# pedro-morgado/spatialaudiogen

Hardware: AMD Instinct MI355X
Metric: ambisonic seconds generated/sec (0.1 s windows, 224x448 video) (higher is better)
Workload: dtype f32 (fp32 in / out / accumulate; products on the 16-bit matrix cores with fp32-equivalent operand splits: two fp16 planes (3 products per multiply) for the ResNet trunk's 3x3 convs, whose operand ranges batch-norm bounds, three bf16 planes (6 products) elsewhere - measured against the fp64 oracle as

## Files before the change

spatialaudiogen_amd/csrc/kernels.h:

```cpp
#pragma once
#include "common.h"
#include "wave_reduce.h"
#include "igemm_tiles.h"

namespace sagen {

struct BnRef {
    const double* acc = nullptr;
    const float* gamma = nullptr;
    const float* beta = nullptr;
    double inv_count = 0.0;
    float eps = 1e-3f;
};

constexpr int H2_AMAX_SLOTS = 64, H2_AMAX_STRIDE = 32, H2_AMAX_FLOATS = H2_AMAX_SLOTS * H2_AMAX_STRIDE;

struct IgemmDesc {
    const float* x = nullptr;
    const float* w = nullptr;
    int w_split = 0;
    float* y = nullptr;
    const float* bias = nullptr;
    const float* in_scale = nullptr;
    const float* in_shift = nullptr;
    BnRef bn_in;
    double* stats = nullptr;
    float* amax_out = nullptr;
    float* splitk_ws = nullptr;
    int* sk_ticket = nullptr;
    int sk_rep = 1;
    int M = 0, N = 0, K = 0, Kpad = 0;
    int Hg = 1, Wg = 1, g_h0 = 0, g_w0 = 0;
    int Hin = 1, Win = 1, Cin = 0, ldx = 0;
    long x_bstride = 0;
    int in_sh = 1, in_sw = 1;
    int ntaps = 1, TW = 1, tap_sh = 1, tap_sw = 1, tap_h0 = 0, tap_w0 = 0;
    int log2Cin = -1;
    int dsh = 1, dsw = 1, Cout = 0;
    int Hlim = 1, Wlim = 1;
    long y_bstride = 0;
    long y_rstride = 0;
    int ldy = 0;
    int relu_out = 0;
    int splitk = 1;
    unsigned x_bytes = 0, w_bytes = 0;
    unsigned y_bytes = 0;
    int no_bounds = 0;
    int uniform_taps = 0;
    const void* xp3 = nullptr;
    unsigned xp3_bytes = 0, xp3_cstride = 0;
    int p3_np = 0;
    int xp3_fmt = 0;
    int xp3_row0 = 0, xp3_rows = 0;
    const void* xs2d = nullptr;
    unsigned xs2d_bytes = 0;
    int xs2d_np = 0;
    const void* wh2 = nullptr;
    unsigned wh2_bytes = 0;
    const float* h2_a_inv = nullptr;
    const float* h2_w_inv = nullptr;
    unsigned p3_magic_wp = 0, p3_magic_h = 0;
    const float* mm_coeffs = nullptr;
    float* mm_out = nullptr;
    int mm_row0 = 0, mm_nf = 0;
    int mm_f_lo = 1;
    void* trace = nullptr;
    int trace_block = 0;
    GroupInfo grp;
};
__device__ __forceinline__ void igemm_relocate(IgemmDesc& d, int g) {
    const GroupInfo gi = d.grp;
    d.x = grp_ptr(d.x, gi, g); d.y = grp_ptr(d.y, gi, g);
    d.in_scale = grp_ptr(d.in_scale, gi, g); d.in_shift = grp_ptr(d.in_shift, gi, g);
    d.bn_in.acc = grp_ptr(d.bn_in.acc, gi, g);
    d.stats = grp_ptr(d.stats, gi, g); d.amax_out = grp_ptr(d.amax_out, gi, g);
    d.splitk_ws = grp_ptr(d.splitk_ws, gi, g); d.sk_ticket = grp_ptr(d.sk_ticket, gi, g);
    d.xp3 = grp_ptr(d.xp3, gi, g); d.xs2d = grp_ptr(d.xs2d, gi, g);
    d.h2_a_inv = grp_ptr(d.h2_a_inv, gi, g); d.h2_w_inv = grp_ptr(d.h2_w_inv, gi, g);
    d.mm_coeffs = grp_ptr(d.mm_coeffs, gi, g); d.mm_out = grp_ptr(d.mm_out, gi, g);
}

inline void igemm_set_p3_planes(IgemmDesc& d, const void* planes, int B, int H, int W, int C) {
    d.xp3 = planes;
    d.p3_np = planes ? B * H * (W + 1) : 0;
    d.xp3_cstride = (unsigned)((size_t)d.p3_np * 96);
    d.xp3_bytes = (unsigned)((size_t)d.xp3_cstride * (C / 16));
}
inline void igemm_set_h2_planes(IgemmDesc& d, const void* planes, int B, int rows, int W, int C, const void* wh2, const float* a_inv,
                                const float* w_inv, int row0 = 0, int band = 0) {
    d.xp3 = planes; d.xp3_fmt = 1; d.xp3_row0 = row0; d.xp3_rows = band;
    d.p3_np = planes ? B * rows * (W + 1) : 0;
    d.xp3_cstride = (unsigned)((size_t)d.p3_np * 64);
    d.xp3_bytes = (unsigned)((size_t)d.xp3_cstride * (C / 16));
    d.wh2 = wh2; d.wh2_bytes = (unsigned)((size_t)d.N * d.Kpad * 4);
    d.h2_a_inv = a_inv; d.h2_w_inv = w_inv;
}
inline void igemm_set_s2d_planes(IgemmDesc& d, const void* planes, int B, int H, int W, int C) {
    d.xs2d = planes;
    d.xs2d_np = B * (H / 2) * (W / 2 + 1);
    d.xs2d_bytes = (unsigned)((size_t)4 * d.xs2d_np * 64 * (C / 16));
}

#define SAGEN_TILE_ENUM(id, ...) TILE_##id,
enum IgemmTile { SAGEN_TILES(SAGEN_TILE_ENUM) TILE_AUTO };

int igemm_launch(const IgemmDesc& d, IgemmTile tile, hipStream_t s);
int igemm_grid_m(const IgemmDesc& d, IgemmTile tile);
IgemmTile igemm_pick_tile(const IgemmDesc& d);
const char* igemm_tile_name(IgemmTile t);
unsigned igemm_tile_traits(IgemmTile t);
int igemm_tile_bm(IgemmTile t);
int igemm_tile_bn(IgemmTile t);
int igemm_tile_bk(IgemmTile t);
bool igemm_tile_split(IgemmTile t);
int igemm_auto_splitk(const IgemmDesc& d, IgemmTile tile);
int igemm3_dispatch(const IgemmDesc& d, IgemmTile tile, hipStream_t s);
int igemm3dw_dispatch(const IgemmDesc& d, IgemmTile tile, hipStream_t s);
int igemm3s2_dispatch(const IgemmDesc& d, IgemmTile tile, hipStream_t s);
int conv3p_dispatch(const IgemmDesc& d, IgemmTile tile, hipStream_t s);
int conv3g_dispatch(const IgemmDesc& d, IgemmTile tile, hipStream_t s);
int conv3h_dispatch(const IgemmDesc& d, IgemmTile tile, hipStream_t s);
int conv3s_dispatch(const IgemmDesc& d, IgemmTile tile, hipStream_t s);
bool conv3s_ok(const IgemmDesc& d);
int h2_filter_pack_launch(const float* wp, int N, int Kpad, void* w2, unsigned* scratch, float* w_inv, hipStream_t s);
struct H2Job {
    const float* wp = nullptr;
    void* w2 = nullptr;
    float* w_inv = nullptr;
    int N = 0, Kpad = 0, first_block = 0, pad_ = 0;
};
int h2_filter_pack_multi_launch(const H2Job* jobs_dev, int njobs, int nblocks, unsigned* amax, hipStream_t s);
bool conv3g_ok(const IgemmDesc& d);
constexpr int SK_TICKETS = 8192;
bool igemm_tile_p3(IgemmTile t);
bool igemm_tile_grouped(IgemmTile t);
bool igemm_tile_s2d(IgemmTile t);
bool igemm_tile_dh_split(IgemmTile t);
bool igemm_p3_eligible(const IgemmDesc& d);
bool igemm_tile_ok(const IgemmDesc& d, IgemmTile t);
constexpr int SPLITK_RB = 16;
int splitk_reduce_launch(const float* ws, int splitk, int M, int N, const float* bias, int relu,
                         float* y, int ldy, int rep, double* stats, hipStream_t s, float* amax_out = nullptr);

struct DeconvGather {
    int B = 0, Hin = 0, Win = 0, kh = 1, kw = 1, sh = 1, sw = 1, Cout = 0;
    int in_row0 = 0, R = 0;
    int y0 = 0, y1 = 0;
    int relu = 0, ldy = 0;
    const float* bias = nullptr;
    float* y = nullptr;
    float* amax_out = nullptr;
};
int deconv_gather_launch(const float* ws, int splitk, const DeconvGather& g, hipStream_t s);

int pack_conv_launch(const float* w_hwio, int ntaps, int cin_src, int cin_pad, int cout,
                     float* wp, int Npad, int Kpad, hipStream_t s, int tw_src = 0, int tw_pad = 0);
int pack_split_launch(float* wp, int N, int Kpad, hipStream_t s);
inline size_t packed_split_floats(size_t n_fp32) { return n_fp32 + (3 * n_fp32 + 1) / 2; }
enum PackKind { PACK_CONV = 0, PACK_DECONV, PACK_FLIPT, PACK_ROWS, PACK_DECONV_PHASE };
struct PackJob {
    const float* src = nullptr;
    float* dst = nullptr;
    int kind = 0, N = 0, Kpad = 0;
    int p[7] = {0, 0, 0, 0, 0, 0, 0};
    int first_block = 0;
};
inline int pack_job_blocks(int kind, long N, long Kpad) {
    return kind == PACK_CONV ? (int)(((N + 31) / 32) * ((Kpad + 31) / 32)) : (int)((N * Kpad + 1023) / 1024);
}
int pack_multi_launch(const PackJob* jobs_dev, int njobs, int nblocks, hipStream_t s, int block0 = 0);
int pack_deconv_launch(const float* w_hwoi, int kh, int kw, int cout, int cin, int sh, int sw,
                       float* wp, int Npad, int Kpad, hipStream_t s);

int bn_finalize_launch(const double* stats, long count, int C, const float* gamma,
                       const float* beta, float eps, float* scale, float* shift, hipStream_t s);
int bn_apply_relu_launch(const float* x, const float* scale, const float* shift, const BnRef& bn, const float* residual,
                         float* y, long n_pixels, int C, hipStream_t s);
int maxpool3x3s2_launch(const float* x, const float* scale, const float* shift, const BnRef& bn, float* y,
                        int B, int H, int W, int C, hipStream_t s);
int pad_nhwc3to4_launch(const float* x, float* y, int B, int H, int W, int pt, int pb, int pl, int pr,
                        hipStream_t s);
int pad_u8_nhwc3to4_launch(const unsigned char* x, float* y, int B, int H, int W, int pt, int pb, int pl, int pr, hipStream_t s);
int stempool_launch(const float* xpad, const float* wp, const float* gamma, float* pooled, double* stats, int B, hipStream_t s);
size_t stem8_plane_bytes(int B);
int stem8_prep_launch(const unsigned char* x, void* plane, int B, hipStream_t s, float* zero_ptr = nullptr, long zero_n = 0, int half = 0);
int stem8pool_h2_launch(const void* plane, const float* wp, const void* wh2, const float* w_inv, const float* gamma, float* pooled, double* stats, int B,
                        hipStream_t s);
int stem8pool_launch(const void* plane, const float* wp, const float* gamma, float* pooled, double* stats, int B, hipStream_t s);
int stem16_prep_launch(const float* x, void* planes, float* part, float* a_inv, int B, hipStream_t s, float* zero_ptr = nullptr, long zero_n = 0);
int stem16pool_launch(const void* planes, const void* wh2, const float* gamma, float* pooled, double* stats, const float* a_inv, const float* w_inv,
                      int B, hipStream_t s);
constexpr int STEM16_PARTS = 1024;
int stem8raw_launch(const void* plane, const float* wp, float* y0, double* stats, int B, hipStream_t s);
int stem8rawpool_launch(const void* plane, const float* wp, const float* gamma, float* y0, float* pooled, double* stats, int B, hipStream_t s);
int assemble_wyzx_launch(const float* audio, const float* yzx, float* out, int B, int snd_size,
                         int snd_contx, int snd_dur, hipStream_t s);
int power_map_launch(const float* ambi, long T, const float* sh, int P, float* rms, hipStream_t s);
int power_map_batched_launch(const float* ambi, int nchunks, long T, const float* sh, int P, float* rms, double* moments, hipStream_t s);
int nosep_mix_launch(const float* audio, const float* coeffs, float* out, int B, int snd_size,
                     int snd_contx, int snd_dur, int num_out, hipStream_t s);
int nosep_mix_multi_launch(const float* audio, const float* coeffs, float* out, int B, int snd_size, int snd_contx,
                           int snd_dur, int nin, int num_out, hipStream_t s);

size_t p3_bytes(int B, int H, int W, int C);
constexpr int H2S_SAT_COUNT = 7;
constexpr int H2S_FILTER_FIRST = 8;
constexpr int H2S_FIXED_FIRST = 232;
constexpr int H2S_A_INV_X = 232;
constexpr int H2S_A_INV_B = 236;
constexpr int H2S_S16_A_INV = 238;
constexpr int H2_RIG_OFF = 240;
struct P3hScale {
    float* a_inv = nullptr;
    const float* res_bound = nullptr;
    const double* res_acc = nullptr;
    double res_inv_count = 0.0;
    float* bound_out = nullptr;
    unsigned* sat_count = nullptr;
    unsigned char* relu_bits = nullptr;
    const void* res_planes = nullptr;
    const float* res_a_inv = nullptr;
};
int p3_pack_launch(const float* x, const float* scale, const float* shift, const BnRef& bn, const float* residual, int relu,
                   float* y, void* p3, int B, int H, int W, int C, hipStream_t s, int fmt = 0, const P3hScale* h2 = nullptr,
                   int s2d = 0);
size_t p3h_bytes(int B, int H, int W, int C);
size_t p3s_bytes(int B, int H, int W, int C);
int h2_pack_rows_launch(const float* x, long x_bstride, long x_rstride, int ldx, int row0, int B, int R, int W, int C, const float* amax0,
                        const float* amax1, void* planes, float* a_inv, unsigned* sat_count, hipStream_t s);
int p3_maxpool_launch(const float* x, const float* scale, const float* shift, const BnRef& bn, float* y, void* p3, int B, int H,
                      int W, int C, hipStream_t s, int fmt = 0, const P3hScale* h2 = nullptr);

int fft_tables_ensure(hipStream_t s);
int stft_launch(const float* audio, int B, int n_samples, int f0, int f1, float* mag,
                int c0, int c1, float* spec, hipStream_t s, float* zero_ptr = nullptr, int zero_n = 0);
size_t mask_istft_scratch_bytes(int B);
int mask_istft_mix_launch(const float* dmask, long dmask_bstride, int dmask_f0, const float* spec,
                          const float* coeffs, int B, int ntracks, float* out, float* scratch,
                          hipStream_t s, const float* ebuf = nullptr);
int stft_multi_launch(const float* audio, int B, int n_samples, int nin, int f0, int f1, float* mag, int c0, int c1, float* spec,
                      hipStream_t s, float* zero_ptr = nullptr, int zero_n = 0);
size_t mask_istft_hoa_scratch_bytes(int B, int nout);
int mask_istft_hoa_launch(const float* dmask, long dmask_bstride, int dmask_f0, const float* spec, const float* coeffs, int B,
                          int ntracks, int nin, int nout, float* out, float* scratch, hipStream_t s);

size_t eval_scratch_floats(int B);
int eval_init_launch(float* scratch, hipStream_t s);
int eval_metrics_launch(const float* pred, const float* gt, int B, float* ps, double* pw, float* scratch, hipStream_t s);
size_t eval_scratch_floats_c(int B, int C);
int eval_metrics_c_launch(const float* pred, const float* gt, int B, int C, float* ps, double* pw, float* scratch, hipStream_t s);
size_t evalx_scratch_floats(int B, int C);
int evalx_mel_env_launch(const float* pred, const float* gt, int B, int C, float* mel_lsd, float* env_mse, float* scratch,
                         hipStream_t s);
int evalx_emd_launch(const float* p, const float* q, int n_maps, int nodes, const double* cost, double* out, unsigned int* not_converged,
                     hipStream_t s);

int render_fir_launch(const float* x, long long n_hist, long long n, int channels, const float* taps, int outputs, int ntaps,
                      const float* rot, int n_rot, int rot_hop, long long pos0, long long zero_before, float* y, hipStream_t s);

int power_map_windows_launch(const float* ambi, int channels, int stride, long long window, int n_maps, const float* sh, int P, float* rms,
                             double* moments, hipStream_t s);
size_t overlay_blend_grid_bytes(int mh, int mw, int n_frames);
int overlay_blend_launch(const float* maps, long long map0, int mh, int mw, const double* lut, const uint8_t* frames, int n_frames,
                         long long frame0, int h, int w, int frames_per_map, uint8_t* out, void* scratch, hipStream_t s);

struct ProjArgs;
int reproject_launch(const uint8_t* src, uint8_t* dst, const double* rot, const ProjArgs& a, hipStream_t s);

struct FlowArgs;
int flow_auto_fuse();
int optical_flow_launch(const uint8_t* frames, const FlowArgs& a, float* flow, void* scratch, hipStream_t s);
int flow_encode_launch(const float* flow, int n, int h, int w, uint8_t* rgb, float* limits, void* scratch, hipStream_t s);

struct ResampleArgs;
int resample_fir_launch(const float* x, const double* taps, const double* mix, float* y, const ResampleArgs& a, const char** why, hipStream_t s);
int window_rms_launch(const float* x, int channels, int channel, long long first, long long hop, long long length, long long count,
                      double* rms, hipStream_t s);

int stft_loss_grad_launch(const float* pred, const float* gt, const float* mask, int B, float* grad, double* loss, hipStream_t s);
int adam_update_launch(float* p, const float* g, float* m, float* v, long n, float lr_t, float beta1, float beta2, float eps,
                       float gscale, hipStream_t s);

struct WgradDesc {
    const float* g = nullptr;
    const float* d = nullptr;
    float* out = nullptr;
    float* ws = nullptr;
    int B = 1, Hd = 1, Wd = 1;
    int HG = 1, WG = 1, ldg = 0, Cg = 0;
    int ldd = 0, Cd = 0;
    unsigned g_bstride = 0, g_rstride = 0, d_bstride = 0, d_rstride = 0;
    int sh = 1, sw = 1, TH = 1, TW = 1, h0 = 0, w0 = 0;
    int tsh = 1, tsw = 1;
    int splitk = 1;
    int defer_reduce = 0;
    const void* gp = nullptr;
    const void* dp = nullptr;
    const float* gp_a_inv = nullptr;
    const float* dp_a_inv = nullptr;
    unsigned gp_bytes = 0, dp_bytes = 0;
    int P = 0, fold = 1;
    unsigned g_bytes = 0, d_bytes = 0, magic_w = 0, magic_h = 0;
};
int wgrad_launch(const WgradDesc& d, hipStream_t s);
int wgrad_pick_splitk(const WgradDesc& d, size_t ws_capacity_floats);
int wgrad_reduce_launch(const WgradDesc& d, hipStream_t s);
const char* wgrad_kernel_name(const WgradDesc& d);
void wgrad_describe(const WgradDesc& d, char* buf, size_t n);
bool wgrad_reads_fp32_operands();
bool wgrad_planes_enabled();

size_t reduce_scratch_floats(int C);
int relu_bwd_launch(const float* ga, int lda, const float* gb, int ldb, const float* act, int ldact, float* dy, int lddy, long R,
                    int C, double* colsum, float* scratch, hipStream_t s, float* colsum_f32 = nullptr,
                    long band_rows = 0, long batch_rows = 0, long row0 = 0);
int bn_bwd_reduce_launch(const float* ga, const float* gb, const float* act, const float* y, const BnRef& bn, long n_pixels, int C,
                         double* acc, float* scratch, hipStream_t s, int self_mask = 0, float* mx_part = nullptr, int* mx_blocks = nullptr,
                         const unsigned char* relu_bits = nullptr);
int bn_bwd_apply_launch(const float* ga, const float* gb, const float* act, const float* y, const BnRef& bn, const double* acc,
                        long n_pixels, int C, float* dy, float* dz_out, float* dgamma, float* dbeta, hipStream_t s, int self_mask = 0);
int bn_bwd_apply_h2_launch(const float* ga, const float* gb, const float* act, const float* y, const BnRef& bn, const double* acc,
                           int B, int H, int W, int C, float* dy, float* dz_out, float* dgamma, float* dbeta, hipStream_t s, int self_mask,
                           void* planes, const float* mx_part, int mx_blocks, float* a_inv, unsigned* sat_count,
                           const unsigned char* relu_bits = nullptr);
int maxpool_bwd_launch(const float* y0, const BnRef& bn, const float* pooled, const float* ga, const float* gb, float* dz,
                       int B, int H, int W, int C, hipStream_t s);
int maxpool_bn_bwd_launch(const float* y0, const BnRef& bn, const float* pooled, const float* ga, const float* gb, float* dy0, int B,
                          int H, int W, int C, double* acc, float* scratch, float* dgamma, float* dbeta, hipStream_t s,
                          const float* pooled_raw = nullptr);
int sum_rows_launch(const float* ina, int lda, const float* inb, int ldb, int rep, long M, int C, float* out, int ldo, hipStream_t s);
int acc_to_f32_launch(const double* acc, float* dst, int n, hipStream_t s);
int bn_moving_update_launch(const BnRef& bn, float* moving_mean, float* moving_var, int C, float decay, hipStream_t s);
constexpr int BN_MOVING_MAX_JOBS = 40;
struct BnMovingJob { const double* acc = nullptr; double inv_count = 0.0; float* mm = nullptr; float* mv = nullptr; int C = 0; };
int bn_moving_update_multi_launch(const BnMovingJob* jobs, int n, float decay, hipStream_t s);
int pack_conv_flipT_launch(const float* w_hwio, int ntaps, int cin, int cout, float* wp, int Kpad, hipStream_t s);
int pack_rows_launch(const float* w, int rows, int cols, float* wp, int Kpad, hipStream_t s);
int stem_wgrad_unpack_launch(const float* tmp, float* dw, hipStream_t s);

size_t mask_istft_bwd_scratch_floats(int B, int ntracks);
int mask_istft_mix_bwd_launch(const float* dmask, long dmask_bstride, int dmask_f0, const float* spec, const float* coeffs,
                              const float* dpred, int B, int ntracks, float* d_dmask, long dd_bstride, int dd_f0, float* dcoeffs,
                              int ldc, float* scratch, hipStream_t s);

}
```

spatialaudiogen_amd/csrc/model.h:

```cpp
#pragma once
#include "kernels.h"
#include "fcm.h"
#include <algorithm>
#include <cstdlib>
#include <functional>
#include <map>
#include <string>
#include <vector>

namespace sagen {

struct VarSpec {
    std::string name;
    int ndim;
    int64_t shape[4];
    long numel() const {
        long n = 1;
        for (int i = 0; i < ndim; ++i) n *= shape[i];
        return n;
    }
};

struct Buf {
    size_t off = 0, n = 0;
};

struct Named {
    Buf buf;
    size_t extra_off = 0;
    int ndim = 0;
    int64_t shape[4] = {0, 0, 0, 0};
    int64_t pixel_stride = 0;
};

static const int AENC_F[5] = {32, 64, 128, 256, 512};
static const int AENC_K[5][2] = {{7, 16}, {3, 7}, {3, 5}, {3, 5}, {3, 5}};
static const int AENC_S[5][2] = {{4, 8}, {2, 4}, {2, 2}, {1, 1}, {1, 1}};

static inline bool is_weights(const std::string& n) { return n.size() >= 8 && n.compare(n.size() - 8, 8, "/weights") == 0; }

struct PkSpec {
    int kind = PACK_CONV;
    int N = 0, K = 0, Kpad = 0;
    int p[7] = {0, 0, 0, 0, 0, 0, 0};
    bool stem = false;
    int dec_l = -1, sh = 1, sw = 1;
    int Ns = 0, Ks = 0;
    bool h2 = false;
};
static inline PkSpec pk_spec(const VarSpec& vs) {
    PkSpec k;
    const int64_t* sp = vs.shape;
    const size_t dec = vs.name.find("/deconv");
    if (dec != std::string::npos) {
        k.kind = PACK_DECONV;
        k.dec_l = vs.name[dec + 7] - '1'; k.sh = AENC_S[k.dec_l][0]; k.sw = AENC_S[k.dec_l][1];
        const int ntw = cdiv((int)sp[1], k.sw);
        k.N = k.sh * k.sw * (int)sp[2]; k.K = cdiv((int)sp[0], k.sh) * ntw * (int)sp[3];
        for (int i = 0; i < 4; ++i) k.p[i] = (int)sp[i];
        k.p[4] = k.sh; k.p[5] = k.sw; k.p[6] = ntw;
        if (k.dec_l >= 1 && sp[3] % 16 == 0) { k.Ns = (int)(sp[0] * sp[1] * sp[2]); k.Ks = (int)sp[3]; }
        k.h2 = k.dec_l == 0;
    } else if (vs.ndim == 4) {
        int cin = (int)sp[2], cinp = cin, taps = (int)(sp[0] * sp[1]);
        k.stem = cin == 3;
        if (k.stem) { cinp = 4; taps = (int)(sp[0] * (sp[1] + 1)); k.p[4] = (int)sp[1]; k.p[5] = (int)sp[1] + 1; }
        if (cin == 1) { cin = cinp = (int)sp[1]; taps = (int)sp[0]; }
        k.N = (int)sp[3]; k.K = taps * cinp;
        k.p[0] = taps; k.p[1] = cin; k.p[2] = cinp; k.p[3] = k.N;
        const bool trunk = vs.name.find("_encoder/conv") != std::string::npos && ((sp[0] == 3 && sp[1] == 3) || (sp[0] == 1 && sp[1] == 1));
        k.h2 = k.stem || (sp[2] % 16 == 0 && (trunk || vs.name.compare(0, 18, "audio_encoder/conv") == 0));
    } else {
        k.N = (int)sp[1]; k.K = (int)sp[0];
        k.p[0] = 1; k.p[1] = k.K; k.p[2] = k.K; k.p[3] = k.N;
    }
    k.Kpad = (k.K + 15) / 16 * 16;
    return k;
}

}

using namespace sagen;

constexpr int SAGEN_MAX_GROUPS = 32;

struct ProfRec {
    std::string kernel, layer;
    double flops = 0.0;
    hipEvent_t e0 = nullptr, e1 = nullptr;
};

struct Choice {
    int tile = -1;
    int splitk = 0;
    float us = 0.f;
};

struct sagen_ctx {
    sagen_config cfg;
    std::map<std::string, Choice> plan;
    std::map<std::string, bool> materialize;
    bool tuning = false;
    bool fp32_only = false;
    bool use_p3 = true;
    int p3_from_stage = 3;
    hipEvent_t tune_e0 = nullptr, tune_e1 = nullptr;
    hipStream_t aux = nullptr;
    hipEvent_t ev_fork = nullptr, ev_join = nullptr, ev_stft = nullptr, ev_pack = nullptr;
    int pack_early_jobs = 0, pack_early_blocks = 0;
    bool late_repack = false;
    bool profiling = false;
    std::vector<ProfRec> prof;
    std::vector<hipEvent_t> event_pool;
    size_t events_used = 0;
    int B = 0;
    int snd_size = 52799, snd_contx = 48000, snd_dur = 4800;
    int enc_h[6], enc_w[6], enc_c[6];
    int Cb = 0;
    int nsep = 32;
    int nin = 1, nout = 3;
    bool has_video = false, has_flow = false, freq_mask = true;

    std::vector<VarSpec> vars;
    std::map<std::string, int> var_index;
    std::vector<const float*> var_ptr;
    bool bound = false;

    int G = 1;
    int tune_groups = 0;
    int inter_group = 0;
    size_t grp_off = 0, grp_floats = 0;
    static bool off_grouped(const sagen_ctx* c) {
        return c->use_fcm || c->sk_fused || c->fp32_only || !c->use_h2 || !c->use_p3 || !c->use_p3g || c->p3_from_stage > 2 || c->no_lean_trunk;
    }
    GroupInfo group_info() const {
        GroupInfo gi;
        if (G > 1 && ws) {
            gi.lo = reinterpret_cast<const char*>(ws + grp_off);
            gi.span = (unsigned long long)grp_floats * sizeof(float);
            gi.stride = gi.span;
            gi.G = G;
        }
        return gi;
    }
    size_t ws_floats = 0;
    float* ws = nullptr;
    std::map<std::string, Buf> bufs;
    std::map<std::string, Named> named;
    std::vector<PackJob> pack_jobs, pack_jobs_bwd;
    int pack_blocks = 0, pack_blocks_bwd = 0;
    bool train_mode = false;
    bool train_ready = false;
    bool stem_fused = true;
    bool materialize_mask = false;
    bool mask_fused_last = false;
    bool video_u8 = false;
    bool train_h2 = true;
    bool use_h2 = true;
    bool train_h2d = true;
    bool no_aud_planes = false;
    bool no_dh_split = false;
    bool sk_fused = false;
    bool train_h2w = true;
    std::map<std::string, int> h2d_slot;
    std::vector<H2Job> h2d_jobs;
    int h2d_blocks = 0;
    std::map<std::string, int> h2_slot;
    std::vector<H2Job> h2_jobs;
    int h2_blocks = 0;
    bool use_p3g = true;
    bool rawpool_last = false;
    bool train_rawpool = true;
    bool train_bands = true;
    int dec_lo[7] = {0, 0, 0, 0, 0, 0, 0}, dec_hi[7] = {0, 0, 0, 0, 0, 0, 0};
    bool use_s2d = true;
    bool no_scatter = false, no_d1_planes = false, no_lean_trunk = false;
    int dec_planes_min_batch = 16;
    bool use_fcm = false;
    std::map<std::string, int> fcm_slices;
    bool stem8h = true;
    bool stem16 = true;
    bool stem8 = true;
    size_t tws_floats = 0;
    float* tws = nullptr;
    std::map<std::string, Buf> tbufs;
    std::vector<float*> grad_ptr;
    std::vector<int> ms_bucket;
    std::vector<int> ms_count, ms_left;
    std::vector<hipEvent_t> ms_event;
    std::vector<char> ms_done;
    std::vector<int> ms_touched;
    hipEvent_t ms_tmp = nullptr;
    std::vector<float*> mov_ptr;
    Buf talloc(const std::string& name, size_t n) {
        Buf b;
        b.off = tws_floats;
        b.n = n;
        tws_floats += (n + 63) / 64 * 64;
        tbufs[name] = b;
        return b;
    }
    size_t cap(const std::string& name) const { auto it = bufs.find(name); return it != bufs.end() ? it->second.n : tbufs.at(name).n; }

    Buf alloc(const std::string& name, size_t n) {
        Buf b;
        b.off = ws_floats;
        b.n = n;
        ws_floats += (n + 63) / 64 * 64;
        bufs[name] = b;
        return b;
    }
    float* p(const std::string& name) const {
        auto it = bufs.find(name);
        if (it != bufs.end()) return ws + it->second.off;
        return tws + tbufs.at(name).off;
    }
    const float* v(const std::string& name) const { return var_ptr[var_index.at(name)]; }
    void add_var(const std::string& name, std::initializer_list<int64_t> shape) {
        VarSpec s;
        s.name = name;
        s.ndim = (int)shape.size();
        int i = 0;
        for (auto d : shape) s.shape[i++] = d;
        for (; i < 4; ++i) s.shape[i] = 1;
        var_index[name] = (int)vars.size();
        vars.push_back(s);
    }
    void expose(const std::string& name, const std::string& buf, size_t extra, std::initializer_list<int64_t> shape,
                int64_t pixel_stride) {
        Named nm;
        nm.buf = bufs.at(buf);
        nm.extra_off = extra;
        nm.ndim = (int)shape.size();
        int i = 0;
        for (auto d : shape) nm.shape[i++] = d;
        nm.pixel_stride = pixel_stride;
        named[name] = nm;
    }
};

namespace sagen {

static inline void add_resnet_vars(sagen_ctx* c, const std::string& scope) {
    auto bn = [&](const std::string& p, int ch) {
        for (const char* leaf : {"beta", "gamma", "moving_mean", "moving_variance"}) c->add_var(p + "/bn/" + leaf, {ch});
    };
    c->add_var(scope + "/conv1/conv/weights", {7, 7, 3, 64});
    bn(scope + "/conv1/conv", 64);
    int cin = 64;
    const int couts[4] = {64, 128, 256, 512};
    for (int st = 0; st < 4; ++st) {
        const int cout = couts[st];
        for (int unit = 1; unit <= 2; ++unit) {
            const std::string pfx = scope + "/conv" + std::to_string(st + 2) + "_" + std::to_string(unit);
            if (unit == 1 && cin != cout) c->add_var(pfx + "/shortcut/weights", {1, 1, cin, cout});
            c->add_var(pfx + "/conv_1/weights", {3, 3, cin, cout});
            bn(pfx + "/conv_1", cout);
            c->add_var(pfx + "/conv_2/weights", {3, 3, cout, cout});
            bn(pfx + "/conv_2", cout);
            cin = cout;
        }
    }
}

static inline bool conv3g_ok_desc(const IgemmDesc& d, int cin) {
    return cin % 16 == 0 && d.Kpad == d.K && d.in_scale == nullptr && d.bn_in.acc == nullptr && d.dsh * d.dsw == 1;
}

static inline size_t packed_floats(long N, long K) { return (size_t)N * ((K + 15) / 16 * 16); }

}


int sagen_repack_impl(sagen_ctx* c, hipStream_t s);
int sagen_repack_part(sagen_ctx* c, hipStream_t s, int part);
bool sagen_forward_forks(const sagen_ctx* c);
int sagen_upload_pack_jobs(std::vector<PackJob>& jobs, void* dev, hipStream_t s);
int sagen_forward_impl(sagen_ctx* c, const float* audio, const float* video, const float* flow, float* out, hipStream_t s);

namespace sagen {

struct Fwd {
    sagen_ctx* c;
    hipStream_t s;
    int rc = SAGEN_OK;
    std::string layer;
    std::string wsname = "splitk";
    std::string sfx;
    hipEvent_t wait_before_mfma = nullptr;
    hipEvent_t wait_packs = nullptr;
    std::function<int(const float* ws, int sk, hipStream_t s)> custom_reduce;
    const char* custom_reduce_name = "";

    hipEvent_t next_event() {
        if (c->events_used == c->event_pool.size()) {
            hipEvent_t e = nullptr;
            if (hipEventCreate(&e) != hipSuccess) return nullptr;
            c->event_pool.push_back(e);
        }
        return c->event_pool[c->events_used++];
    }
    template <class F>
    void timed(const char* kernel, double flops, F&& launch) {
        if (rc) return;
        if (!c->profiling) { rc = launch(); return; }
        ProfRec r;
        r.kernel = kernel; r.layer = layer; r.flops = flops;
        r.e0 = next_event(); r.e1 = next_event();
        if (!r.e0 || !r.e1) { rc = fail(SAGEN_ERR_HIP, "hipEventCreate failed"); return; }
        hipError_t he = hipEventRecord(r.e0, s);
        rc = launch();
        if (he == hipSuccess) he = hipEventRecord(r.e1, s);
        if (he != hipSuccess && !rc) rc = fail(SAGEN_ERR_HIP, "hipEventRecord: %s", hipGetErrorString(he));
        c->prof.push_back(r);
    }

    bool dense_out(const IgemmDesc& d) const {
        return d.dsh * d.dsw == 1 && d.g_h0 == 0 && d.g_w0 == 0 && d.y_rstride == (long)d.Wg * d.ldy &&
               (d.M <= d.Hg * d.Wg || d.y_bstride == (long)d.Hg * d.Wg * d.ldy);
    }
    size_t ws_capacity() const { return c->bufs.at(wsname).n; }
    hipError_t memset_groups(void* p, size_t bytes) {
        for (int g = 0; g < c->G; ++g) {
            const hipError_t e = hipMemsetAsync(reinterpret_cast<char*>(p) + (size_t)g * c->grp_floats * sizeof(float), 0, bytes, s);
            if (e != hipSuccess) return e;
        }
        return hipSuccess;
    }

    int run_choice(const IgemmDesc& d, int rep, IgemmTile tile, int sk) {
        if (rc) return 0;
        if (sk > 1 || rep > 1 || custom_reduce) {
            IgemmDesc e = d;
            e.splitk = sk;
            e.splitk_ws = c->ws + c->bufs.at(wsname).off;
            e.amax_out = nullptr;
            if (custom_reduce) {
                e.bias = nullptr; e.relu_out = 0; e.stats = nullptr;
                if (igemm_tile_p3(tile)) e.y = e.splitk_ws;
                timed(igemm_tile_name(tile), 2.0 * d.M * d.N * d.K, [&] { return igemm_launch(e, tile, s); });
                timed(custom_reduce_name, 0.0, [&] { return custom_reduce(e.splitk_ws, sk, s); });
                return 0;
            }
            const long tiles = (long)cdiv(d.M, igemm_tile_bm(tile)) * cdiv(d.N, igemm_tile_bn(tile));
            if (c->sk_fused && sk > 1 && !d.stats && !d.amax_out && d.N % 4 == 0 && d.ldy % 4 == 0 && ((uintptr_t)d.y % 16) == 0 && (!d.bias || ((uintptr_t)d.bias % 16) == 0) &&
                tiles <= SK_TICKETS && c->bufs.count(wsname + ":tk")) {
                e.sk_ticket = reinterpret_cast<int*>(c->ws + c->bufs.at(wsname + ":tk").off);
                e.sk_rep = rep;
                e.stats = nullptr;
                timed(igemm_tile_name(tile), 2.0 * d.M * d.N * d.K, [&] { return igemm_launch(e, tile, s); });
                return 0;
            }
            e.bias = nullptr; e.relu_out = 0; e.stats = nullptr;
            timed(igemm_tile_name(tile), 2.0 * d.M * d.N * d.K, [&] { return igemm_launch(e, tile, s); });
            timed("splitk_reduce_kernel", 0.0, [&] {
                return splitk_reduce_launch(e.splitk_ws, sk, d.M, d.N, d.bias, d.relu_out, d.y, d.ldy, rep, d.stats, s, d.amax_out); });
            return 0;
        }
        timed(igemm_tile_name(tile), 2.0 * d.M * d.N * d.K, [&] { return igemm_launch(d, tile, s); });
        return 0;
    }

    Choice heuristic(const IgemmDesc& d, int rep, bool allow_split) const {
        Choice ch;
        const IgemmTile tile = igemm_pick_tile(d);
        ch.tile = (int)tile;
        const bool can_split = allow_split && dense_out(d) && !d.stats && !igemm_tile_p3(tile);
        ch.splitk = can_split ? igemm_auto_splitk(d, tile) : 1;
        while (ch.splitk > 1 && (size_t)ch.splitk * d.M * d.N > ws_capacity()) --ch.splitk;
        return ch;
    }

    float time_once(const IgemmDesc& d, int rep, IgemmTile tile, int sk) {
        const Buf& fl = c->bufs.at("dmask_or_scratch_flush");
        (void)hipMemsetAsync(c->ws + fl.off, 0, std::min<size_t>(fl.n * sizeof(float), (size_t)48 << 20), s);
        (void)hipEventRecord(c->tune_e0, s);
        run_choice(d, rep, tile, sk);
        (void)hipEventRecord(c->tune_e1, s);
        if (hipEventSynchronize(c->tune_e1) != hipSuccess) { rc = fail(SAGEN_ERR_HIP, "autotune: event sync failed"); return 1e30f; }
        float ms = 0.f;
        (void)hipEventElapsedTime(&ms, c->tune_e0, c->tune_e1);
        return ms * 1e3f;
    }

    Choice tune(const IgemmDesc& d, int rep, bool allow_split) {
        struct FewerGroups {
            GroupInfo& g; int saved;
            explicit FewerGroups(int n) : g(cur_group()), saved(g.G) { if (n > 0 && g.G > n) g.G = n; }
            ~FewerGroups() { g.G = saved; }
        } fewer(c->tune_groups);
        Choice top[3];
        for (auto& t : top) { t = heuristic(d, rep, allow_split); t.us = 1e30f; }
        const bool dense = dense_out(d);
        static const int SKS[] = {1, 2, 3, 4, 5, 6, 8, 10, 12, 16, 24, 32, 48, 64};
        for (int t = 0; t < (int)TILE_AUTO && !rc; ++t) {
            const IgemmTile tile = (IgemmTile)t;
            const int bm = igemm_tile_bm(tile), bn = igemm_tile_bn(tile);
            if (!igemm_tile_ok(d, tile)) continue;
            static const bool p3pp = getenv("SAGEN_P3PP") != nullptr;
            if (!p3pp && !c->train_mode && (igemm_tile_traits(tile) & TF_TWO_TEAM)) continue;
            static const bool p3hr = getenv("SAGEN_P3HR") != nullptr;
            if (!p3hr && c->G == 1 && (igemm_tile_traits(tile) & TF_RING3)) continue;
            const int nk = d.Kpad / igemm_tile_bk(tile);
            if (bn > 32 && bn >= 2 * d.N) continue;
            if (bm > 32 && bm >= 4 * d.M) continue;
            for (int sk : SKS) {
                if (sk > 1 && (!allow_split || !dense)) break;
                if (sk > 1 && igemm_tile_p3(tile)) {
                    if (!igemm_tile_dh_split(tile) || sk > 3 || c->no_dh_split) break;
                    if (sk != 3) continue;
                }
                if (sk > 1 && ((nk / sk < 4 && !igemm_tile_p3(tile)) || (size_t)sk * d.M * d.N > ws_capacity())) break;
                if (sk == 1 && (rep > 1 || custom_reduce) && (size_t)d.M * d.N > ws_capacity()) continue;
                const long blocks = (long)cdiv(d.M, bm) * cdiv(d.N, bn) * sk;
                if (sk > 1 && blocks > 8192) break;
                float t_best = 1e30f;
                for (int it = 0; it < 5 && !rc; ++it) {
                    const float us = time_once(d, rep, tile, sk);
                    if (it > 0) t_best = std::min(t_best, us);
                }
                Choice ch; ch.tile = t; ch.splitk = sk; ch.us = t_best;
                for (int k = 0; k < 3; ++k)
                    if (ch.us < top[k].us) { std::swap(ch, top[k]); }
            }
        }
        if (rc || top[1].us > 1e29f) return top[0];
        std::vector<float> runs[3];
        const int nc = top[2].us > 1e29f ? 2 : 3;
        for (int it = 0; it < 8 && !rc; ++it)
            for (int k = 0; k < nc; ++k) runs[k].push_back(time_once(d, rep, (IgemmTile)top[k].tile, top[k].splitk));
        int best = 0;
        for (int k = 0; k < nc; ++k) {
            std::sort(runs[k].begin(), runs[k].end());
            top[k].us = runs[k][runs[k].size() / 2];
            if (top[k].us < top[best].us) best = k;
        }
        return top[best];
    }

    int contract(const IgemmDesc& d_in, int rep = 1, bool allow_split = true) {
        if (rc) return 0;
        IgemmDesc d = d_in;
        d.w_split = c->fp32_only ? 0 : 1;
        if (rep > 1 && !dense_out(d)) { rc = fail(SAGEN_ERR_UNSUPPORTED, "replicated store needs a dense plain epilogue"); return 0; }
        Choice ch;
        auto it = c->plan.find(layer);
        if (c->tuning) {
            const bool was_prof = c->profiling;
            c->profiling = false;
            ch = tune(d, rep, allow_split);
            c->profiling = was_prof;
            c->plan[layer] = ch;
            if (d.stats && !rc && memset_groups(d.stats, (size_t)2 * d.N * sizeof(double)) != hipSuccess)
                rc = fail(SAGEN_ERR_HIP, "autotune: memset failed");
        } else if (it != c->plan.end()) {
            ch = it->second;
            if (!igemm_tile_ok(d, (IgemmTile)ch.tile)) ch = heuristic(d, rep, allow_split);
            const bool dh3 = ch.splitk == 3 && igemm_tile_dh_split((IgemmTile)ch.tile);
            if (ch.splitk > 1 && (!allow_split || !dense_out(d) || (igemm_tile_p3((IgemmTile)ch.tile) && !dh3) || d.Kpad / igemm_tile_bk((IgemmTile)ch.tile) / ch.splitk < 1)) ch.splitk = 1;
        } else {
            ch = heuristic(d, rep, allow_split);
        }
        if ((ch.splitk > 1 || rep > 1 || custom_reduce) && (size_t)std::max(ch.splitk, 1) * d.M * d.N > ws_capacity()) {
            rc = fail(SAGEN_ERR_WORKSPACE, "split-K scratch too small for %s", layer.c_str());
            return 0;
        }
        return run_choice(d, rep, (IgemmTile)ch.tile, std::max(ch.splitk, 1));
    }
    void gemm(const IgemmDesc& d, int rep = 1, bool allow_split = true) { contract(d, rep, allow_split); }

    IgemmDesc conv_desc(const float* x, int Hin, int Win, int Cin, int ldx, const float* wp, int kh, int kw, int sh, int sw,
                        bool same, int Cout, float* y, int ldy, int& Hout, int& Wout) {
        IgemmDesc d;
        int pt = 0, pl = 0;
        if (same) {
            Hout = cdiv(Hin, sh); Wout = cdiv(Win, sw);
            pt = std::max((Hout - 1) * sh + kh - Hin, 0) / 2;
            pl = std::max((Wout - 1) * sw + kw - Win, 0) / 2;
        } else {
            Hout = (Hin - kh) / sh + 1; Wout = (Win - kw) / sw + 1;
        }
        d.x = x; d.w = wp; d.y = y;
        d.M = c->B * Hout * Wout; d.N = Cout; d.K = kh * kw * Cin; d.Kpad = (d.K + 15) / 16 * 16;
        d.Hg = Hout; d.Wg = Wout;
        d.Hin = Hin; d.Win = Win; d.Cin = Cin; d.ldx = ldx; d.x_bstride = (long)Hin * Win * ldx;
        d.in_sh = sh; d.in_sw = sw;
        d.ntaps = kh * kw; d.TW = kw; d.tap_sh = 1; d.tap_sw = 1; d.tap_h0 = -pt; d.tap_w0 = -pl;
        d.log2Cin = ilog2_exact(Cin);
        d.Cout = Cout; d.Hlim = Hout; d.Wlim = Wout;
        d.ldy = ldy; d.y_rstride = (long)Wout * ldy; d.y_bstride = (long)Hout * Wout * ldy;
        return d;
    }

    void fc(const float* x, int M, int K, int ldx, const std::string& name, int N, bool relu, float* y, int ldy, int rep = 1, float* amax_out = nullptr) {
        layer = name;
        IgemmDesc d;
        d.x = x; d.w = c->p("pk:" + name + "/weights"); d.y = y; d.bias = c->v(name + "/biases");
        d.M = M; d.N = N; d.K = K; d.Kpad = (K + 15) / 16 * 16;
        d.Hg = 1; d.Wg = 1; d.Hin = 1; d.Win = 1; d.Cin = K; d.ldx = ldx; d.x_bstride = ldx;
        d.ntaps = 1; d.Cout = N; d.Hlim = 1; d.Wlim = 1; d.ldy = ldy; d.y_rstride = ldy; d.y_bstride = ldy;
        d.relu_out = relu;
        d.amax_out = amax_out;
        gemm(d, rep);
    }

    void deconv(const float* x, int Hin, int Win, int Cin, int l, float* y, int ldy, bool relu, int a0, int a1, int Ylim,
                long y_bstride, long y_row0, const float* mm_coeffs = nullptr, float* mm_out = nullptr, int mm_nf = 0,
                const std::function<void(IgemmDesc&)>& tweak = nullptr) {
        const std::string name = "separation/deconv" + std::to_string(l + 1);
        layer = name;
        const int kh = AENC_K[l][0], kw = AENC_K[l][1], sh = AENC_S[l][0], sw = AENC_S[l][1];
        const int Cout = l == 0 ? c->nsep * c->nin : AENC_F[l - 1];
        const int Hout = Hin * sh + kh - sh, Wout = Win * sw + kw - sw;
        const int nth = cdiv(kh, sh), ntw = cdiv(kw, sw);
        IgemmDesc d;
        d.x = x; d.w = c->p("pk:" + name + "/weights"); d.bias = c->v(name + "/biases");
        d.Hg = (a1 > a0 ? a1 - a0 : cdiv(Hout, sh)); d.g_h0 = a0; d.Wg = cdiv(Wout, sw);
        d.M = c->B * d.Hg * d.Wg; d.N = sh * sw * Cout; d.K = nth * ntw * Cin; d.Kpad = (d.K + 15) / 16 * 16;
        d.Hin = Hin; d.Win = Win; d.Cin = Cin; d.ldx = Cin; d.x_bstride = (long)Hin * Win * Cin;
        d.ntaps = nth * ntw; d.TW = ntw; d.tap_sh = -1; d.tap_sw = -1; d.log2Cin = ilog2_exact(Cin);
        d.dsh = sh; d.dsw = sw; d.Cout = Cout;
        d.Hlim = Ylim > 0 ? Ylim : Hout; d.Wlim = Wout;
        d.ldy = ldy; d.y_rstride = (long)Wout * ldy;
        d.y_bstride = y_bstride > 0 ? y_bstride : (long)Hout * Wout * ldy;
        d.y = y - y_row0 * d.y_rstride;
        d.relu_out = relu;
        if (mm_out) { d.mm_coeffs = mm_coeffs; d.mm_out = mm_out; d.mm_row0 = (int)y_row0; d.mm_nf = mm_nf; d.mm_f_lo = 1; }
        if (tweak) tweak(d);
        gemm(d);
    }

    float* cat_amax(int l, int half) { return c->p("amax") + (size_t)((l - 1) * 2 + half) * H2_AMAX_FLOATS; }
    float* cat_a_inv(int l) { return c->p("amax") + (size_t)10 * H2_AMAX_FLOATS + l; }
    void deconv_scatter(const float* x, int Hin, int Win, int Cin, int l, float* y, int ldy, bool relu, int in_row0, int R, int y0, int y1,
                        float* amax_out = nullptr, bool x_planes = false) {
        const std::string name = "separation/deconv" + std::to_string(l + 1);
        layer = name;
        DeconvGather gd;
        gd.B = c->B; gd.Hin = Hin; gd.Win = Win; gd.kh = AENC_K[l][0]; gd.kw = AENC_K[l][1]; gd.sh = AENC_S[l][0]; gd.sw = AENC_S[l][1];
        gd.Cout = l == 0 ? c->nsep : AENC_F[l - 1];
        gd.in_row0 = in_row0; gd.R = R; gd.y0 = y0; gd.y1 = y1; gd.relu = relu ? 1 : 0; gd.ldy = ldy;
        gd.bias = c->v(name + "/biases"); gd.y = y; gd.amax_out = amax_out;
        IgemmDesc d;
        d.x = x + (long)in_row0 * Win * Cin; d.w = c->p("pks:" + name + "/weights");
        d.M = c->B * R * Win; d.N = gd.kh * gd.kw * gd.Cout; d.K = Cin; d.Kpad = Cin;
        d.Hg = R; d.Wg = Win; d.Hin = Hin - in_row0; d.Win = Win; d.Cin = Cin; d.ldx = Cin; d.x_bstride = (long)Hin * Win * Cin;
        d.ntaps = 1; d.Cout = d.N; d.Hlim = R; d.Wlim = Win; d.ldy = d.N; d.y_rstride = (long)Win * d.N; d.y_bstride = (long)R * Win * d.N;
        d.y = c->ws + c->bufs.at(wsname).off;
        if (x_planes && !c->tuning) {
            auto it = c->plan.find(name);
            if (it != c->plan.end() && !igemm_tile_p3((IgemmTile)it->second.tile)) x_planes = false;
        }
        if (x_planes) {
            const int lx = l + 1;
            void* planes = c->p("catp");
            timed("h2_pack_rows_kernel", 0.0, [&] {
                return h2_pack_rows_launch(x, (long)Hin * Win * Cin, (long)Win * Cin, Cin, in_row0, c->B, R, Win, Cin, cat_amax(lx, 0), cat_amax(lx, 1), planes,
                                           cat_a_inv(lx), h2_sat_count(), s); });
            const H2Filter w = h2_filter(name, true);
            igemm_set_h2_planes(d, planes, c->B, R, Win, Cin, w.w2, cat_a_inv(lx), w.w_inv, 0, R);
        }
        custom_reduce_name = "deconv_gather_kernel";
        custom_reduce = [gd](const float* ws, int sk, hipStream_t st) { return deconv_gather_launch(ws, sk, gd, st); };
        gemm(d);
        custom_reduce = nullptr;
    }

    bool h2() const { return c->use_h2 && c->use_p3 && !c->fp32_only && (!c->train_mode || c->train_h2); }
    struct H2Filter { const void* w2; const float* w_inv; };
    bool has_h2_filter(const std::string& name) const { return c->h2_slot.count(name) != 0; }
    H2Filter h2_filter(const std::string& name, bool scatter = false) const {
        return {c->p((scatter ? "pkhs:" : "pkh:") + name + "/weights"), c->p("h2s") + c->h2_slot.at((scatter ? "pks:" : "") + name)};
    }
    unsigned* h2_sat_count() const { return reinterpret_cast<unsigned*>(c->p("h2s") + H2S_SAT_COUNT); }
    int p3_fmt() const { return h2() ? 1 : 0; }
    float* h2_a_inv() { return c->p("h2s") + (sfx.empty() ? 0 : 1); }
    float* h2_a_inv_x(int parity) { return c->p("h2s") + H2S_A_INV_X + 2 * (parity & 1) + (sfx.empty() ? 0 : 1); }
    float* h2_a_inv_b() { return c->p("h2s") + H2S_A_INV_B + (sfx.empty() ? 0 : 1); }
    float* h2_xbound(int parity) { return c->p("h2s") + 2 + 2 * (parity & 1) + (sfx.empty() ? 0 : 1); }
    P3hScale h2_scale(float* bound_out = nullptr, const float* res_bound = nullptr, const double* res_acc = nullptr, double res_inv_count = 0.0) {
        P3hScale h;
        h.a_inv = h2_a_inv(); h.bound_out = bound_out; h.res_bound = res_bound; h.res_acc = res_acc; h.res_inv_count = res_inv_count;
        h.sat_count = h2_sat_count();
        return h;
    }

    double* bn_acc(int layer_index) { return reinterpret_cast<double*>(c->p("bnacc" + sfx)) + (size_t)layer_index * 2 * 512; }
    BnRef bn_ref(int layer_index, const std::string& bn_name, long count) {
        BnRef r;
        r.acc = bn_acc(layer_index);
        r.gamma = c->v(bn_name + "/bn/gamma");
        r.beta = c->v(bn_name + "/bn/beta");
        r.inv_count = 1.0 / (double)count;
        r.eps = 1e-3f;
        return r;
    }

    void conv_bn(const float* x, int Hin, int Win, int Cin, const std::string& name, int k, int stride, int Cout,
                 const BnRef& bn_in, float* y, int& Hout, int& Wout, int bn_index, const std::string& plan_key = "",
                 const void* planes = nullptr, const float* planes_a_inv = nullptr, const void* s2d_planes = nullptr) {
        if (rc) return;
        IgemmDesc d = conv_desc(x, Hin, Win, Cin, Cin, c->p("pk:" + name + "/weights"), k, k, stride, stride, true, Cout, y,
                                Cout, Hout, Wout);
        if (planes || s2d_planes) {
            if (h2() && (stride == 1 || c->use_p3g) && k == 3 && has_h2_filter(name)) {
                const H2Filter w = h2_filter(name);
                igemm_set_h2_planes(d, planes, c->B, Hin, Win, Cin, w.w2, planes_a_inv ? planes_a_inv : h2_a_inv(), w.w_inv);
                if (s2d_planes) igemm_set_s2d_planes(d, s2d_planes, c->B, Hin, Win, Cin);
            } else {
                igemm_set_p3_planes(d, planes, c->B, Hin, Win, Cin);
            }
        }
        d.bn_in = bn_in;
        d.stats = bn_acc(bn_index);
        layer = plan_key.empty() ? name : plan_key;
        contract(d);
    }

    void projection(const std::string& pfx, int st, const float* x, bool x_fp32, int H, int W, int cin, int cout, const void* planes,
                    const float* planes_a_inv, bool stats, int& Ho, int& Wo) {
        IgemmDesc d = conv_desc(x_fp32 ? x : nullptr, H, W, cin, cin, c->p("pk:" + pfx + "/shortcut/weights"), 1, 1, 2, 2, true, cout,
                                c->p("rsc" + sfx), cout, Ho, Wo);
        if (planes && planes_a_inv) {
            const H2Filter w = h2_filter(pfx + "/shortcut");
            igemm_set_h2_planes(d, planes, c->B, H, W, cin, w.w2, planes_a_inv, w.w_inv);
        } else if (planes) {
            igemm_set_p3_planes(d, planes, c->B, H, W, cin);
        }
        if (stats) d.stats = bn_acc(20 + st);
        layer = pfx + "/shortcut";
        gemm(d, 1, false);
    }

    const float* resnet(const float* img, const std::string& scope) {
        const int B = c->B;
        int li = 0;
        const bool tune_general = c->tuning && c->G == 1;
        const bool fast8 = c->video_u8 && scope == "video_encoder" && c->stem8 && !tune_general && !c->fp32_only && !c->train_mode;
        const bool fast8h = fast8 && c->stem8h && h2() && has_h2_filter(scope + "/conv1/conv");
        const bool fast16 = !fast8 && !(c->video_u8 && scope == "video_encoder") && c->stem16 && !tune_general && !c->fp32_only && !c->train_mode && h2() &&
                            c->use_p3 && c->p3_from_stage <= 2 && c->bufs.count("s16:part" + sfx) != 0 && has_h2_filter(scope + "/conv1/conv");
        if (!fast8 && !fast16 && !rc && hipMemsetAsync(c->p("bnacc" + sfx), 0, c->bufs.at("bnacc" + sfx).n * sizeof(float), s) != hipSuccess)
            rc = fail(SAGEN_ERR_HIP, "hipMemsetAsync(bn accumulators) failed");
        layer = scope + "/pad";
        const bool pool_planes = c->use_p3 && c->p3_from_stage <= 2;
        const bool no_lean = c->no_lean_trunk;
        const bool lean = !no_lean && h2() && pool_planes && c->use_p3g && c->bufs.count("p3b" + sfx) != 0 && !c->train_mode;
        float* const s16_a_inv = c->p("h2s") + H2S_S16_A_INV + (sfx.empty() ? 0 : 1);
        if (fast16)
            timed("stem16_amax_kernel+stem16_prep_kernel", 0.0, [&] { return stem16_prep_launch(img, c->p("xpad" + sfx), c->p("s16:part" + sfx), s16_a_inv, B, s,
                                                                                               c->p("bnacc" + sfx), (long)c->bufs.at("bnacc" + sfx).n); });
        else if (fast8)
            timed("stem8_prep_kernel", 0.0, [&] { return stem8_prep_launch(reinterpret_cast<const unsigned char*>(img), c->p("xpad" + sfx), B, s,
                                                                          c->p("bnacc" + sfx), (long)c->bufs.at("bnacc" + sfx).n, fast8h ? 1 : 0); });
        else if (c->video_u8 && scope == "video_encoder")
            timed("pad_u8_nhwc3to4_kernel", 0.0, [&] { return pad_u8_nhwc3to4_launch(reinterpret_cast<const unsigned char*>(img), c->p("xpad" + sfx), B, 224, 448, 2, 3, 2, 4, s); });
        else
            timed("pad_nhwc3to4_kernel", 0.0, [&] { return pad_nhwc3to4_launch(img, c->p("xpad" + sfx), B, 224, 448, 2, 3, 2, 4, s); });
        int H = 0, W = 0;
        if (!rc && wait_before_mfma) {
            if (hipStreamWaitEvent(s, wait_before_mfma, 0) != hipSuccess) rc = fail(SAGEN_ERR_HIP, "hipStreamWaitEvent failed");
            wait_before_mfma = nullptr;
        }
        {
            const std::string name = scope + "/conv1/conv";
            const bool fused = c->stem_fused && !c->tuning && !c->fp32_only && !(c->use_p3 && c->p3_from_stage <= 2);
            if (fast8 || fast16) {
                H = 112; W = 224;
                layer = name + "+pool";
                if (fast16)
                    timed("stem8pool_kernel<f16>", 2.0 * B * H * W * 64 * 224, [&] {
                        return stem16pool_launch(c->p("xpad" + sfx), h2_filter(name).w2, c->v(name + "/bn/gamma"), c->p("rx0" + sfx), bn_acc(li),
                                                 s16_a_inv, h2_filter(name).w_inv, B, s); });
                else if (fast8h)
                    timed("stem8pool_kernel<h2>", 2.0 * B * H * W * 64 * 224, [&] {
                        return stem8pool_h2_launch(c->p("xpad" + sfx), c->p("pk:" + name + "/weights"), h2_filter(name).w2, h2_filter(name).w_inv,
                                                   c->v(name + "/bn/gamma"), c->p("rx0" + sfx), bn_acc(li), B, s); });
                else
                timed("stem8pool_kernel", 2.0 * B * H * W * 64 * 224, [&] {
                    return stem8pool_launch(c->p("xpad" + sfx), c->p("pk:" + name + "/weights"), c->v(name + "/bn/gamma"), c->p("rx0" + sfx), bn_acc(li), B, s); });
                const BnRef bnf = bn_ref(li, name, (long)B * H * W);
                layer = name + "/bn-relu";
                P3hScale hs0 = h2_scale(h2_xbound(0));
                if (lean) hs0.a_inv = h2_a_inv_x(0);
                if (pool_planes)
                    timed("p3_pack_kernel", 0.0, [&] { return p3_pack_launch(c->p("rx0" + sfx), nullptr, nullptr, bnf, nullptr, 1, lean ? nullptr : c->p("rx0" + sfx), c->p("p3" + sfx), B, 56, 112, 64, s, p3_fmt(), &hs0); });
                else
                    timed("bn_apply_relu_kernel", 0.0, [&] { return bn_apply_relu_launch(c->p("rx0" + sfx), nullptr, nullptr, bnf, nullptr, c->p("rx0" + sfx), (long)B * 56 * 112, 64, s); });
            } else if (fused) {
                H = 112; W = 224;
                layer = name + "+pool";
                timed("stempool_kernel", 2.0 * B * H * W * 64 * 224, [&] {
                    return stempool_launch(c->p("xpad" + sfx), c->p("pk:" + name + "/weights"), c->v(name + "/bn/gamma"), c->p("rx0" + sfx), bn_acc(li), B, s); });
                const BnRef bnf = bn_ref(li, name, (long)B * H * W);
                layer = name + "/bn-relu";
                timed("bn_apply_relu_kernel", 0.0, [&] { return bn_apply_relu_launch(c->p("rx0" + sfx), nullptr, nullptr, bnf, nullptr, c->p("rx0" + sfx), (long)B * 56 * 112, 64, s); });
            } else {
            IgemmDesc d = conv_desc(c->p("xpad" + sfx), 229, 454, 4, 4, c->p("pk:" + name + "/weights"), 7, 8, 2, 2, false, 64,
                                    c->p("y0" + sfx), 64, H, W);
            d.stats = bn_acc(li);
            layer = name;
            contract(d);
            const BnRef bn = bn_ref(li, name, (long)B * H * W);
            if (c->use_p3 && c->p3_from_stage <= 2)
            {
                P3hScale hs0 = h2_scale(h2_xbound(0));
                if (lean) hs0.a_inv = h2_a_inv_x(0);
                timed("p3_maxpool_kernel", 0.0, [&] { return p3_maxpool_launch(c->p("y0" + sfx), nullptr, nullptr, bn, lean ? nullptr : c->p("rx0" + sfx), c->p("p3" + sfx), B, H, W, 64, s, p3_fmt(), &hs0); });
            }
            else
                timed("maxpool3x3s2_kernel", 0.0, [&] { return maxpool3x3s2_launch(c->p("y0" + sfx), nullptr, nullptr, bn, c->p("rx0" + sfx), B, H, W, 64, s); });
            }
            ++li;
            H = (H + 1) / 2; W = (W + 1) / 2;
        }
        float* xin = c->p("rx0" + sfx);
        float* xout = c->p("rx1" + sfx);
        int cin = 64;
        const int couts[4] = {64, 128, 256, 512};
        bool x_in_planes = pool_planes;
        int xb_par = 0;
        bool x_in_s2d = false, x_in_rows = true;
        bool x_fp32_valid = !lean;
        for (int st = 0; st < 4; ++st) {
            const int cout = couts[st];
            for (int unit = 1; unit <= 2; ++unit) {
                const std::string pfx = scope + "/conv" + std::to_string(st + 2) + "_" + std::to_string(unit);
                const bool first = unit == 1 && cin != cout;
                const int stride = first ? 2 : 1;
                int Ho = 0, Wo = 0;
                const float* shortcut = xin;
                const bool p3_here = c->use_p3 && st + 2 >= c->p3_from_stage;
                void* planes = p3_here ? (void*)c->p((lean ? "p3b" : "p3") + sfx) : nullptr;
                void* const xplanes = p3_here ? (void*)c->p("p3" + sfx) : nullptr;
                const float* const x_ai = lean ? h2_a_inv_x(xb_par) : nullptr;
                const void* in_planes = (p3_here && x_in_planes && x_in_rows) ? xplanes : nullptr;
                const void* const in_s2d = (first && p3_here && x_in_planes && x_in_s2d) ? (void*)c->p("p3b" + sfx) : nullptr;
                auto shortcut_s2d = [&] {
                    IgemmDesc d = conv_desc(nullptr, H / 2, W / 2, cin, cin, c->p("pk:" + pfx + "/shortcut/weights"), 1, 1, 1, 1, true,
                                            cout, c->p("rsc" + sfx), cout, Ho, Wo);
                    const H2Filter w = h2_filter(pfx + "/shortcut");
                    igemm_set_h2_planes(d, in_s2d, B, H / 2, W / 2, cin, w.w2, x_ai, w.w_inv);
                    d.stats = bn_acc(20 + st);
                    layer = pfx + "/shortcut#s2d";
                    gemm(d, 1, false);
                };
                if (first && in_s2d && !in_planes) {
                    shortcut_s2d();
                    shortcut = c->p("rsc" + sfx);
                } else if (first) {
                    const bool proj_h2 = h2() && has_h2_filter(pfx + "/shortcut");
                    projection(pfx, st, xin, x_fp32_valid, H, W, cin, cout, in_planes, proj_h2 ? (x_ai ? x_ai : h2_a_inv()) : nullptr, h2() && p3_here, Ho, Wo);
                    if (in_s2d && !rc) {
                        if (memset_groups(bn_acc(20 + st), (size_t)2 * cout * sizeof(double)) != hipSuccess) rc = fail(SAGEN_ERR_HIP, "autotune: memset failed");
                        shortcut_s2d();
                    }
                    shortcut = c->p("rsc" + sfx);
                }
                conv_bn(x_fp32_valid ? xin : nullptr, H, W, cin, pfx + "/conv_1", 3, stride, cout, BnRef(), c->p("ry1" + sfx), Ho, Wo, li, "", in_planes, x_ai, in_s2d);
                const BnRef bn1 = bn_ref(li, pfx + "/conv_1", (long)B * Ho * Wo);
                ++li;
                int H2, W2;
                if (p3_here) {
                    layer = pfx + "/bn1-relu";
                    P3hScale hs1 = h2_scale();
                    if (lean) hs1.a_inv = h2_a_inv_b();
                    timed("p3_pack_kernel", 0.0, [&] { return p3_pack_launch(c->p("ry1" + sfx), nullptr, nullptr, bn1, nullptr, 1, nullptr, planes, B, Ho, Wo, cout, s, p3_fmt(), &hs1); });
                    conv_bn(nullptr, Ho, Wo, cout, pfx + "/conv_2", 3, 1, cout, BnRef(), c->p("ry2" + sfx), H2, W2, li, "", planes, lean ? h2_a_inv_b() : nullptr);
                    const BnRef bn2 = bn_ref(li, pfx + "/conv_2", (long)B * Ho * Wo);
                    layer = pfx + "/merge";
                    const bool to_next_stage = unit == 2 && c->use_p3g && st < 3;
                    const bool next_p3 = unit == 1 || to_next_stage;
                    P3hScale hs2 = first ? h2_scale(h2_xbound(xb_par ^ 1), nullptr, bn_acc(20 + st), 1.0 / ((double)B * Ho * Wo))
                                         : h2_scale(h2_xbound(xb_par ^ 1), h2_xbound(xb_par));
                    const bool res_planes = lean && !first;
                    const bool y_fp32 = lean ? !next_p3 : !to_next_stage;
                    if (lean) {
                        hs2.a_inv = h2_a_inv_x(xb_par ^ 1);
                        if (res_planes) { hs2.res_planes = xplanes; hs2.res_a_inv = h2_a_inv_x(xb_par); }
                    }
                    xb_par ^= 1;
                    bool s2d_out = false, rows_out = true;
                    const std::string next_c1 = scope + "/conv" + std::to_string(st + 3) + "_1/conv_1";
                    if (lean && to_next_stage && c->use_s2d && !(Ho & 1) && !(Wo & 1) && c->h2_slot.count(next_c1) != 0 &&
                        c->h2_slot.count(scope + "/conv" + std::to_string(st + 3) + "_1/shortcut") != 0) {
                        auto it = c->plan.find(next_c1);
                        s2d_out = c->tuning || (it != c->plan.end() && igemm_tile_s2d((IgemmTile)it->second.tile));
                        rows_out = c->tuning || !s2d_out;
                    }
                    if (s2d_out)
                        timed("p3_pack_kernel", 0.0, [&] { return p3_pack_launch(c->p("ry2" + sfx), nullptr, nullptr, bn2, res_planes ? nullptr : shortcut, 1, nullptr, c->p("p3b" + sfx), B, Ho, Wo, cout, s, p3_fmt(), &hs2, 1); });
                    if (rows_out)
                        timed("p3_pack_kernel", 0.0, [&] { return p3_pack_launch(c->p("ry2" + sfx), nullptr, nullptr, bn2, res_planes ? nullptr : shortcut, 1, y_fp32 ? xout : nullptr, next_p3 ? xplanes : nullptr, B, Ho, Wo, cout, s, p3_fmt(), &hs2); });
                    x_in_s2d = s2d_out; x_in_rows = rows_out;
                    x_in_planes = next_p3;
                    x_fp32_valid = y_fp32;
                    ++li;
                    std::swap(xin, xout);
                    H = Ho; W = Wo; cin = cout;
                    continue;
                }
                const std::string l2 = pfx + "/conv_2";
                auto run_prologue = [&] { conv_bn(c->p("ry1" + sfx), Ho, Wo, cout, l2, 3, 1, cout, bn1, c->p("ry2" + sfx), H2, W2, li); };
                auto run_materialized = [&](const std::string& key) {
                    layer = pfx + "/bn1-relu";
                    timed("bn_apply_relu_kernel", 0.0, [&] { return bn_apply_relu_launch(c->p("ry1" + sfx), nullptr, nullptr, bn1, nullptr, c->p("ry1n" + sfx), (long)B * Ho * Wo, cout, s); });
                    conv_bn(c->p("ry1n" + sfx), Ho, Wo, cout, l2, 3, 1, cout, BnRef(), c->p("ry2" + sfx), H2, W2, li, key);
                };
                if (c->tuning && !rc) {
                    run_prologue();
                    const float t_pro = c->plan[l2].us;
                    (void)hipEventRecord(c->tune_e0, s);
                    (void)bn_apply_relu_launch(c->p("ry1" + sfx), nullptr, nullptr, bn1, nullptr, c->p("ry1n" + sfx), (long)B * Ho * Wo, cout, s);
                    (void)hipEventRecord(c->tune_e1, s);
                    (void)hipEventSynchronize(c->tune_e1);
                    float ms = 0.f;
                    (void)hipEventElapsedTime(&ms, c->tune_e0, c->tune_e1);
                    if (!rc && hipMemsetAsync(bn_acc(li), 0, (size_t)2 * cout * sizeof(double), s) != hipSuccess) rc = fail(SAGEN_ERR_HIP, "memset failed");
                    run_materialized(l2 + "#mat");
                    const float t_mat = c->plan[l2 + "#mat"].us + ms * 1e3f;
                    c->materialize[l2] = t_mat < t_pro;
                    if (!c->materialize[l2] && !rc) {
                        if (hipMemsetAsync(bn_acc(li), 0, (size_t)2 * cout * sizeof(double), s) != hipSuccess) rc = fail(SAGEN_ERR_HIP, "memset failed");
                        c->tuning = false; run_prologue(); c->tuning = true;
                    }
                } else if (c->materialize.count(l2) && c->materialize[l2]) {
                    run_materialized(l2 + "#mat");
                } else {
                    run_prologue();
                }
                const BnRef bn2 = bn_ref(li, pfx + "/conv_2", (long)B * Ho * Wo);
                layer = pfx + "/merge";
                const bool planes_out = unit == 2 && st < 3 && c->use_p3g && c->use_p3 && st + 3 >= c->p3_from_stage;
                if (planes_out)
                    timed("p3_pack_kernel", 0.0, [&] { return p3_pack_launch(c->p("ry2" + sfx), nullptr, nullptr, bn2, shortcut, 1, nullptr, c->p("p3" + sfx), B, Ho, Wo, cout, s); });
                else
                    timed("bn_apply_relu_kernel", 0.0, [&] { return bn_apply_relu_launch(c->p("ry2" + sfx), nullptr, nullptr, bn2, shortcut, xout, (long)B * Ho * Wo, cout, s); });
                x_in_planes = planes_out;
                x_fp32_valid = !planes_out;
                ++li;
                std::swap(xin, xout);
                H = Ho; W = Wo; cin = cout;
            }
        }
        return xin;
    }

    bool h2w() const { return c->train_mode && c->train_h2w && c->train_h2d && h2() && c->p3_from_stage <= 2 && wgrad_planes_enabled() && c->tbufs.count("t:h2a" + sfx) != 0; }
    void* pl_buf(const char* what, int k) { return c->p(std::string("t:pl:") + what + ":" + std::to_string(k) + sfx); }
    float* pl_a_inv(int slot) { return c->p("t:h2a" + sfx) + slot; }
    const float* resnet_train(const float* img, const std::string& scope) {
        const int B = c->B;
        const bool keep = h2w();
        int li = 0;
        if (!rc && hipMemsetAsync(c->p("bnacc" + sfx), 0, c->bufs.at("bnacc" + sfx).n * sizeof(float), s) != hipSuccess)
            rc = fail(SAGEN_ERR_HIP, "hipMemsetAsync(bn accumulators) failed");
        layer = scope + "/pad";
        if (c->video_u8 && scope == "video_encoder")
            timed("pad_u8_nhwc3to4_kernel", 0.0, [&] { return pad_u8_nhwc3to4_launch(reinterpret_cast<const unsigned char*>(img), c->p("xpad" + sfx), B, 224, 448, 2, 3, 2, 4, s); });
        else
            timed("pad_nhwc3to4_kernel", 0.0, [&] { return pad_nhwc3to4_launch(img, c->p("xpad" + sfx), B, 224, 448, 2, 3, 2, 4, s); });
        int H = 0, W = 0;
        const bool fast8 = c->video_u8 && scope == "video_encoder" && c->stem8 && !c->tuning && !c->fp32_only && c->tbufs.count("t:s8plane" + sfx) != 0;
        if (fast8) {
            layer = scope + "/plane";
            timed("stem8_prep_kernel", 0.0, [&] { return stem8_prep_launch(reinterpret_cast<const unsigned char*>(img), c->p("t:s8plane" + sfx), B, s); });
        }
        if (!rc && wait_before_mfma) {
            if (hipStreamWaitEvent(s, wait_before_mfma, 0) != hipSuccess) rc = fail(SAGEN_ERR_HIP, "hipStreamWaitEvent failed");
            wait_before_mfma = nullptr;
        }
        {
            const std::string name = scope + "/conv1/conv";
            const bool rawpool = fast8 && keep && c->train_rawpool && c->bufs.count("rx0" + sfx) != 0;
            if (scope == "video_encoder") c->rawpool_last = rawpool;
            if (rawpool) {
                H = 112; W = 224;
                layer = name;
                timed("stem8pool_kernel<raw+pool>", 2.0 * B * H * W * 64 * 224, [&] {
                    return stem8rawpool_launch(c->p("t:s8plane" + sfx), c->p("pk:" + name + "/weights"), c->v(name + "/bn/gamma"), c->p("y0" + sfx), c->p("rx0" + sfx),
                                               bn_acc(li), B, s); });
            } else if (fast8) {
                H = 112; W = 224;
                layer = name;
                timed("stem8pool_kernel<raw>", 2.0 * B * H * W * 64 * 224, [&] {
                    return stem8raw_launch(c->p("t:s8plane" + sfx), c->p("pk:" + name + "/weights"), c->p("y0" + sfx), bn_acc(li), B, s); });
            } else {
                IgemmDesc d = conv_desc(c->p("xpad" + sfx), 229, 454, 4, 4, c->p("pk:" + name + "/weights"), 7, 8, 2, 2, false, 64,
                                        c->p("y0" + sfx), 64, H, W);
                d.stats = bn_acc(li);
                layer = name;
                contract(d);
            }
            const BnRef bn = bn_ref(li, name, (long)B * H * W);
            if (rawpool) {
                P3hScale hs0 = h2_scale(h2_xbound(0));
                hs0.a_inv = pl_a_inv(8);
                layer = name + "/bn-relu";
                timed("p3_pack_kernel", 0.0, [&] { return p3_pack_launch(c->p("rx0" + sfx), nullptr, nullptr, bn, nullptr, 1, c->p("t:x0" + sfx), pl_buf("x", 0), B, 56, 112, 64, s, 1, &hs0); });
            } else if (keep) {
                P3hScale hs0 = h2_scale(h2_xbound(0));
                hs0.a_inv = pl_a_inv(8);
                timed("p3_maxpool_kernel", 0.0, [&] { return p3_maxpool_launch(c->p("y0" + sfx), nullptr, nullptr, bn, c->p("t:x0" + sfx), pl_buf("x", 0), B, H, W, 64, s, 1, &hs0); });
            } else {
                timed("maxpool3x3s2_kernel", 0.0, [&] { return maxpool3x3s2_launch(c->p("y0" + sfx), nullptr, nullptr, bn, c->p("t:x0" + sfx), B, H, W, 64, s); });
            }
            ++li;
            H = (H + 1) / 2; W = (W + 1) / 2;
        }
        if (!rc && wait_packs) {
            if (hipStreamWaitEvent(s, wait_packs, 0) != hipSuccess) rc = fail(SAGEN_ERR_HIP, "hipStreamWaitEvent failed");
            wait_packs = nullptr;
        }
        const float* xin = c->p("t:x0" + sfx);
        int cin = 64;
        int xb_par = 0;
        const int couts[4] = {64, 128, 256, 512};
        for (int st = 0; st < 4; ++st) {
            const int cout = couts[st];
            for (int unit = 1; unit <= 2; ++unit) {
                const std::string pfx = scope + "/conv" + std::to_string(st + 2) + "_" + std::to_string(unit);
                const std::string k = std::to_string(2 * st + unit - 1) + sfx;
                const bool first = unit == 1 && cin != cout;
                const int stride = first ? 2 : 1;
                int Ho = 0, Wo = 0, H2, W2;
                const float* shortcut = xin;
                const int kidx = 2 * st + unit - 1;
                const bool p3_here = c->use_p3 && st + 2 >= c->p3_from_stage && (st + 2 >= 3 || keep);
                void* planes = p3_here ? (keep ? pl_buf("a1", kidx) : (void*)c->p("p3" + sfx)) : nullptr;
                const float* planes_ai = keep && p3_here ? pl_a_inv(kidx) : nullptr;
                void* xplanes = p3_here ? (keep ? pl_buf("x", kidx) : (void*)c->p("p3" + sfx)) : nullptr;
                const float* xplanes_ai = keep && p3_here ? pl_a_inv(8 + kidx) : nullptr;
                const bool to_next_stage = keep && unit == 2 && st < 3 && c->use_p3g;
                void* nplanes = p3_here && (unit == 1 || to_next_stage) ? (keep ? pl_buf("x", kidx + 1) : (void*)c->p("p3" + sfx)) : nullptr;
                const bool x_planes = p3_here && (stride == 1 ? (unit == 2 || (keep && st == 0)) : (keep && c->use_p3g));
                if (first) {
                    projection(pfx, st, xin, true, H, W, cin, cout, x_planes && has_h2_filter(pfx + "/shortcut") ? xplanes : nullptr, xplanes_ai,
                               h2() && p3_here, Ho, Wo);
                    shortcut = c->p("rsc" + sfx);
                }
                float* y1 = c->p("t:y1:" + k); float* a1 = c->p("t:a1:" + k); float* y2 = c->p("t:y2:" + k); float* xout = c->p("t:out:" + k);
                conv_bn(xin, H, W, cin, pfx + "/conv_1", 3, stride, cout, BnRef(), y1, Ho, Wo, li, "",
                        x_planes ? xplanes : nullptr, x_planes ? xplanes_ai : nullptr);
                const BnRef bn1 = bn_ref(li, pfx + "/conv_1", (long)B * Ho * Wo);
                ++li;
                layer = pfx + "/bn1-relu";
                P3hScale hs1 = h2_scale();
                if (planes_ai) hs1.a_inv = const_cast<float*>(planes_ai);
                static const bool a1_wanted = getenv("SAGEN_BN_READ_ACT") != nullptr || getenv("SAGEN_TRAIN_KEEP_A1") != nullptr;
                float* a1w = (keep && p3_here && !a1_wanted && !wgrad_reads_fp32_operands()) ? nullptr : a1;
                if (p3_here) timed("p3_pack_kernel", 0.0, [&] { return p3_pack_launch(y1, nullptr, nullptr, bn1, nullptr, 1, a1w, planes, B, Ho, Wo, cout, s, p3_fmt(), &hs1); });
                else timed("bn_apply_relu_kernel", 0.0, [&] { return bn_apply_relu_launch(y1, nullptr, nullptr, bn1, nullptr, a1, (long)B * Ho * Wo, cout, s); });
                conv_bn(p3_here ? a1w : a1, Ho, Wo, cout, pfx + "/conv_2", 3, 1, cout, BnRef(), y2, H2, W2, li, p3_here ? "" : pfx + "/conv_2#mat", planes, planes_ai);
                const BnRef bn2 = bn_ref(li, pfx + "/conv_2", (long)B * Ho * Wo);
                ++li;
                layer = pfx + "/merge";
                P3hScale hs2 = first ? h2_scale(h2_xbound(xb_par ^ 1), nullptr, bn_acc(20 + st), 1.0 / ((double)B * Ho * Wo))
                                     : h2_scale(h2_xbound(xb_par ^ 1), h2_xbound(xb_par));
                if (keep && p3_here) {
                    hs2.a_inv = pl_a_inv(8 + kidx + 1);
                    hs2.relu_bits = reinterpret_cast<unsigned char*>(c->p("t:mb:" + k));
                }
                if (p3_here) xb_par ^= 1;
                if (p3_here) timed("p3_pack_kernel", 0.0, [&] { return p3_pack_launch(y2, nullptr, nullptr, bn2, shortcut, 1, xout, nplanes, B, Ho, Wo, cout, s, p3_fmt(), &hs2); });
                else timed("bn_apply_relu_kernel", 0.0, [&] { return bn_apply_relu_launch(y2, nullptr, nullptr, bn2, shortcut, xout, (long)B * Ho * Wo, cout, s); });
                xin = xout;
                H = Ho; W = Wo; cin = cout;
            }
        }
        return xin;
    }
};

}
```

spatialaudiogen_amd/csrc/model.hip:

```cpp
#include "model.h"

void sagen_destroy_impl(sagen_ctx* c);
int sagen_groups_impl(const sagen_ctx* c) { return c->G; }
int sagen_create_impl(sagen_ctx** out, const sagen_config* cfg, int groups) {
    if (!out || !cfg) return fail(SAGEN_ERR_NULL, "sagen_create: null argument");
    if (groups < 1 || groups > SAGEN_MAX_GROUPS) return fail(SAGEN_ERR_SHAPE, "sagen_create_grouped: groups=%d (1..%d)", groups, SAGEN_MAX_GROUPS);
    if (groups > 1 && cfg->separation != SAGEN_SEP_FREQ_MASK)
        return fail(SAGEN_ERR_UNSUPPORTED, "sagen_create_grouped: the grouped launch covers the FREQ_MASK path only");
    if (cfg->batch <= 0) return fail(SAGEN_ERR_SHAPE, "sagen_create: batch=%d", cfg->batch);
    if (!(cfg->encoders & SAGEN_ENC_AUDIO))
        return fail(SAGEN_ERR_UNSUPPORTED, "the audio encoder is mandatory (reference model.py:207)");
    if (cfg->audio_rate != 48000 || cfg->video_rate != 10 || cfg->context != 1.0f || cfg->sample_duration != 0.1f ||
        cfg->fft_window != 0.025f)
        return fail(SAGEN_ERR_UNSUPPORTED,
                    "HIP path implements audio_rate=48000 video_rate=10 context=1.0 sample_duration=0.1 "
                    "fft_window=0.025 (the geometry of every BASELINE config)");
    if (cfg->ambi_order != 1 && cfg->ambi_order != 2)
        return fail(SAGEN_ERR_UNSUPPORTED, "ambi_order=%d (supported: 1, 2; order 3 would need audio_encoder/conv1 with cin = 9, "
                    "which the contraction kernels do not take)", cfg->ambi_order);
    if (cfg->separation != SAGEN_SEP_NONE && cfg->separation != SAGEN_SEP_FREQ_MASK)
        return fail(SAGEN_ERR_UNSUPPORTED, "unknown separation mode %d", cfg->separation);
    if (cfg->separation == SAGEN_SEP_NONE && cfg->num_sep_tracks > 1)
        return fail(SAGEN_ERR_UNSUPPORTED, "separation 'none' decodes the mono track only: num_sep_tracks must be 1 (got %d); the reference's fc3 "
                    "would be [.., 3*(num_sep_tracks+1)] (model.py:254) against a single separated track (model.py:274-280)", cfg->num_sep_tracks);
    if (cfg->separation == SAGEN_SEP_FREQ_MASK && cfg->num_sep_tracks != 16 && cfg->num_sep_tracks != 32 &&
        cfg->num_sep_tracks != 64)
        return fail(SAGEN_ERR_UNSUPPORTED, "num_sep_tracks=%d (supported 16/32/64)", cfg->num_sep_tracks);
    if (cfg->n_loc_units < 0 || cfg->n_loc_units > 4) return fail(SAGEN_ERR_SHAPE, "n_loc_units=%d", cfg->n_loc_units);
    for (int i = 0; i < cfg->n_loc_units; ++i)
        if (cfg->loc_units[i] <= 0 || cfg->loc_units[i] % 4) return fail(SAGEN_ERR_UNSUPPORTED, "loc_units[%d]=%d must be a positive multiple of 4", i, cfg->loc_units[i]);

    sagen_ctx* c = new sagen_ctx();
    c->G = groups;

    c->fp32_only = getenv("SAGEN_FP32_ONLY") != nullptr;
    c->use_p3 = !c->fp32_only && getenv("SAGEN_NO_P3") == nullptr;
    if (const char* e = getenv("SAGEN_P3_FROM_STAGE")) c->p3_from_stage = atoi(e);
    c->stem_fused = getenv("SAGEN_NO_STEMPOOL") == nullptr && (getenv("SAGEN_ONE_STREAM") == nullptr || getenv("SAGEN_STEMPOOL") != nullptr);
    c->stem8 = getenv("SAGEN_NO_STEM8") == nullptr;
    c->stem16 = getenv("SAGEN_NO_STEM16") == nullptr;
    c->stem8h = getenv("SAGEN_NO_STEM8_H2") == nullptr;
    c->use_h2 = getenv("SAGEN_NO_H2") == nullptr;
    c->train_h2 = getenv("SAGEN_TRAIN_NO_H2") == nullptr;
    c->train_h2d = getenv("SAGEN_TRAIN_NO_H2D") == nullptr;
    c->train_h2w = getenv("SAGEN_TRAIN_NO_H2W") == nullptr;
    c->sk_fused = getenv("SAGEN_SK_FUSED") != nullptr;
    c->no_dh_split = getenv("SAGEN_NO_DH_SPLIT") != nullptr;
    c->no_aud_planes = getenv("SAGEN_NO_AUDIO_PLANES") != nullptr;
    if (const char* e = getenv("SAGEN_TUNE_GROUPS")) c->tune_groups = atoi(e);
    c->no_scatter = getenv("SAGEN_NO_DECONV_SCATTER") != nullptr;
    c->train_bands = getenv("SAGEN_TRAIN_NO_BANDS") == nullptr;
    c->train_rawpool = getenv("SAGEN_TRAIN_NO_RAWPOOL") == nullptr;
    c->no_d1_planes = getenv("SAGEN_NO_DECONV1_PLANES") != nullptr;
    c->no_lean_trunk = getenv("SAGEN_NO_LEAN_TRUNK") != nullptr;
    c->use_s2d = getenv("SAGEN_NO_S2D") == nullptr;
    if (getenv("SAGEN_NO_DECODER_PLANES") != nullptr) c->dec_planes_min_batch = 1 << 30;
    if (getenv("SAGEN_P3_FROM_STAGE") == nullptr) c->p3_from_stage = (c->use_h2 && c->use_p3) ? 2 : 3;
    c->use_p3g = c->use_p3 && (getenv("SAGEN_P3G") != nullptr || (c->use_h2 && getenv("SAGEN_NO_P3G") == nullptr));
    c->cfg = *cfg;
    c->B = cfg->batch;
    c->has_video = cfg->encoders & SAGEN_ENC_VIDEO;
    c->has_flow = cfg->encoders & SAGEN_ENC_FLOW;
    c->freq_mask = cfg->separation == SAGEN_SEP_FREQ_MASK;
    c->nsep = c->freq_mask ? cfg->num_sep_tracks : 1;
    c->nin = cfg->ambi_order * cfg->ambi_order;
    c->nout = (cfg->ambi_order + 1) * (cfg->ambi_order + 1) - cfg->ambi_order * cfg->ambi_order;
    const int B = c->B;

    c->enc_h[0] = 127; c->enc_w[0] = 1024; c->enc_c[0] = c->nin;
    for (int l = 0; l < 5; ++l) {
        c->enc_h[l + 1] = (c->enc_h[l] - AENC_K[l][0]) / AENC_S[l][0] + 1;
        c->enc_w[l + 1] = (c->enc_w[l] - AENC_K[l][1]) / AENC_S[l][1] + 1;
        c->enc_c[l + 1] = AENC_F[l];
    }
    c->Cb = 1024 + (c->has_video ? 512 : 0) + (c->has_flow ? 512 : 0);

    {
        int cin = c->nin;
        for (int l = 0; l < 5; ++l) {
            const std::string n = "audio_encoder/conv" + std::to_string(l + 1);
            c->add_var(n + "/weights", {AENC_K[l][0], AENC_K[l][1], cin, AENC_F[l]});
            c->add_var(n + "/biases", {AENC_F[l]});
            cin = AENC_F[l];
        }
        if (c->has_video) add_resnet_vars(c, "video_encoder");
        if (c->has_flow) add_resnet_vars(c, "flow_encoder");
        c->add_var("bottleneck/audio-fc/weights", {c->enc_w[5] * c->enc_c[5], 1024});
        c->add_var("bottleneck/audio-fc/biases", {1024});
        for (const char* e : {"video", "flow"}) {
            if ((std::string(e) == "video" && !c->has_video) || (std::string(e) == "flow" && !c->has_flow)) continue;
            c->add_var(std::string("bottleneck/") + e + "-fc-red/weights", {512, 128});
            c->add_var(std::string("bottleneck/") + e + "-fc-red/biases", {128});
            c->add_var(std::string("bottleneck/") + e + "-fc/weights", {7 * 14 * 128, 512});
            c->add_var(std::string("bottleneck/") + e + "-fc/biases", {512});
        }
        int fin = c->Cb;
        for (int i = 0; i < cfg->n_loc_units; ++i) {
            const std::string n = "localization/fc" + std::to_string(i + 1);
            c->add_var(n + "/weights", {fin, cfg->loc_units[i]});
            c->add_var(n + "/biases", {cfg->loc_units[i]});
            fin = cfg->loc_units[i];
        }
        const int nlast = c->nout * c->nin * (c->nsep + 1);
        const std::string n = "localization/fc" + std::to_string(cfg->n_loc_units + 1);
        c->add_var(n + "/weights", {fin, nlast});
        c->add_var(n + "/biases", {nlast});
        if (c->freq_mask) {
            c->add_var("separation/fc-feats/weights", {c->Cb, 512});
            c->add_var("separation/fc-feats/biases", {512});
            const int nfs[5] = {c->nsep * c->nin, 32, 64, 128, 256};
            int dcin = 1024;
            for (int l = 4; l >= 0; --l) {
                const std::string dn = "separation/deconv" + std::to_string(l + 1);
                c->add_var(dn + "/weights", {AENC_K[l][0], AENC_K[l][1], nfs[l], dcin});
                c->add_var(dn + "/biases", {nfs[l]});
                dcin = nfs[l] + (l > 0 ? AENC_F[l - 1] : 0);
            }
        }
    }
    c->var_ptr.assign(c->vars.size(), nullptr);

    size_t h2_pack_blocks = 0;
    for (const auto& vs : c->vars) {
        if (!is_weights(vs.name)) continue;
        const PkSpec k = pk_spec(vs);
        const std::string lname = vs.name.substr(0, vs.name.size() - 8);
        const size_t n = (size_t)k.N * k.Kpad;
        c->alloc("pk:" + vs.name, packed_split_floats(n));
        if (k.Ns) {
            const size_t ns = (size_t)k.Ns * k.Ks;
            c->alloc("pks:" + vs.name, packed_split_floats(ns));
            c->alloc("pkhs:" + vs.name, ns);
            h2_pack_blocks += ns / 1024 + 1;
            c->h2_slot["pks:" + lname] = -1;
        }
        if (k.h2) {
            c->alloc("pkh:" + vs.name, n);
            h2_pack_blocks += n / 1024 + 1;
            c->h2_slot[lname] = -1;
        }
    }
    {
        int slot = H2S_FILTER_FIRST;
        for (auto& kv : c->h2_slot) kv.second = slot++;
        static_assert(H2S_A_INV_X + 4 <= H2S_A_INV_B && H2S_A_INV_B + 2 <= H2S_S16_A_INV && H2S_S16_A_INV + 2 <= H2_RIG_OFF &&
                      2 + H2_RIG_OFF + 4 <= 256, "h2s: the fixed slots overlap");
        if (slot > H2S_FIXED_FIRST) return fail(SAGEN_ERR_UNSUPPORTED, "too many fp16x2 layers for the scale table");
    }
    c->alloc("h2:jobs", (c->h2_slot.size() + 1) * sizeof(H2Job) / sizeof(float) + 64);
    c->alloc("h2:amax", c->h2_slot.size() + h2_pack_blocks + 64);
    c->alloc("pk:jobs", (c->vars.size() + 1) * sizeof(PackJob) / sizeof(float) + 64);
    c->grp_off = c->ws_floats;
    c->alloc("h2s", 256);
    c->alloc("mag", (size_t)B * 127 * 1024 * c->nin);
    c->alloc("spec", (size_t)B * c->nin * 28 * 513 * 2);
    for (int l = 1; l <= 5; ++l)
        c->alloc("cat" + std::to_string(l), (size_t)B * c->enc_h[l] * c->enc_w[l] * 2 * c->enc_c[l]);
    c->alloc("bott", (size_t)B * 3 * c->Cb);
    for (int i = 0; i < cfg->n_loc_units; ++i) c->alloc("loc" + std::to_string(i + 1), (size_t)B * 3 * cfg->loc_units[i]);
    c->alloc("coeffs", (size_t)B * 3 * c->nout * c->nin * (c->nsep + 1));
    {
        struct L { std::string name; int rows, K, N; };
        std::vector<L> ls;
        ls.push_back({"bottleneck/audio-fc", 3 * B, c->enc_w[5] * c->enc_c[5], 1024});
        if (c->has_video) ls.push_back({"bottleneck/video-fc", B, 7 * 14 * 128, 512});
        if (c->has_flow) ls.push_back({"bottleneck/flow-fc", B, 7 * 14 * 128, 512});
        int fin = c->Cb;
        for (int i = 0; i < cfg->n_loc_units; ++i) { ls.push_back({"localization/fc" + std::to_string(i + 1), 3 * B, fin, cfg->loc_units[i]}); fin = cfg->loc_units[i]; }
        ls.push_back({"localization/fc" + std::to_string(cfg->n_loc_units + 1), 3 * B, fin, c->nout * c->nin * (c->nsep + 1)});
        if (c->freq_mask) ls.push_back({"separation/fc-feats", 3 * B, c->Cb, 512});
        bool ok = getenv("SAGEN_FCM") != nullptr && !c->sk_fused && 3 * B <= FCM_MAX_M;
        for (const L& l : ls) ok = ok && fcm_pick_slices(l.K, (long)l.K * l.N) > 0;
        c->use_fcm = ok;
        if (ok)
            for (const L& l : ls) {
                int ns = fcm_pick_slices(l.K, (long)l.K * l.N);
                if (l.name == "separation/fc-feats") ns = c->fcm_slices.at("localization/fc1");
                c->fcm_slices[l.name] = ns;
                c->alloc("fcm:" + l.name, (size_t)ns * l.rows * l.N);
            }
    }
    c->alloc("splitk", std::max<size_t>((size_t)16 << 20, (size_t)B * 56 * 112 * 64 * 2));
    if (c->freq_mask) {
        c->alloc("cat1p", (p3h_bytes(B, 7, c->enc_w[1], 2 * c->enc_c[1]) + 3) / 4 + 64);
        {
            size_t mx = 0;
            for (int l = 2; l <= 5; ++l) mx = std::max(mx, p3h_bytes(B, c->enc_h[l], c->enc_w[l], 2 * c->enc_c[l]));
            c->alloc("catp", (mx + 3) / 4 + 64);
        }
        {
            size_t mx = 0;
            for (int l = 1; l <= 4; ++l) mx = std::max(mx, p3h_bytes(B, c->enc_h[l], c->enc_w[l], c->enc_c[l]));
            c->alloc("aencp", (mx + 3) / 4 + 64);
        }
        c->alloc("amax", 10 * H2_AMAX_FLOATS + 64);
        c->alloc("dmask", (size_t)B * 23 * 1024 * c->nsep * c->nin);
        c->alloc("frames", (c->nin == 1 ? mask_istft_scratch_bytes(B) : mask_istft_hoa_scratch_bytes(B, c->nout)) / sizeof(float));
    }
    c->alloc("splitk_aux", (size_t)8 << 20);
    c->alloc("splitk:tk", SK_TICKETS);
    c->alloc("splitk_aux:tk", SK_TICKETS);
    for (int set = 0; set < 2; ++set) {
        const std::string x = set ? "_b" : "";
        if (set == 0 ? !(c->has_video || c->has_flow) : !(c->has_video && c->has_flow)) continue;
        c->alloc("xpad" + x, (size_t)B * 229 * 456 * 4);
        c->alloc("s16:part" + x, STEM16_PARTS + 64);
        c->alloc("y0" + x, (size_t)B * 112 * 224 * 64);
        const size_t stage = (size_t)B * 56 * 112 * 64;
        for (const char* nm : {"rx0", "rx1", "ry1", "ry2", "rsc", "ry1n"}) c->alloc(nm + x, stage);
        c->alloc("p3" + x, (p3_bytes(B, 56, 112, 64) + 3) / 4 + 64);
        c->alloc("p3b" + x, (std::max(p3h_bytes(B, 56, 112, 64), p3s_bytes(B, 56, 112, 64)) + 3) / 4 + 64);
        c->alloc("bnacc" + x, (size_t)24 * 2 * 512 * 2);
        c->alloc("fcred" + x, (size_t)B * 98 * 128);
        const std::string enc = (set == 1 || !c->has_video) ? "flow_encoder" : "video_encoder";
        c->expose(enc + "/conv5_2", "rx0" + x, 0, {B, 7, 14, 512}, 512);
    }
    c->bufs["dmask_or_scratch_flush"] = c->freq_mask ? c->bufs.at("dmask") : c->bufs.at("splitk_aux");
    c->expose("mag", "mag", 0, {B, 127, 1024, c->nin}, c->nin);
    c->expose("stft", "spec", 0, {B, c->nin * 28, 513, 2}, 2);
    for (int l = 1; l <= 5; ++l) {
        const int ce = c->enc_c[l];
        c->expose("audio_encoder/conv" + std::to_string(l), "cat" + std::to_string(l), l == 5 ? 0 : ce,
                  {B, c->enc_h[l], c->enc_w[l], ce}, 2 * ce);
    }
    c->expose("bottleneck", "bott", 0, {B, 3, c->Cb}, c->Cb);
    c->expose("localization/coeffs", "coeffs", 0, {B, 3, c->nout * c->nin, c->nsep + 1}, c->nsep + 1);
    if (c->freq_mask) c->expose("separation/deconv1", "dmask", 0, {B, 23, 1024, c->nsep * c->nin}, c->nsep * c->nin);
    int prio_lo = 0, prio_hi = 0;
    (void)hipDeviceGetStreamPriorityRange(&prio_lo, &prio_hi);
    const char* aux_prio = getenv("SAGEN_AUX_PRIO");
    const int prio = aux_prio && aux_prio[0] == 'l' ? prio_lo : (aux_prio && aux_prio[0] == 'h' ? prio_hi : 0);
    if ((aux_prio ? hipStreamCreateWithPriority(&c->aux, hipStreamNonBlocking, prio) : hipStreamCreateWithFlags(&c->aux, hipStreamNonBlocking)) != hipSuccess ||
        hipEventCreateWithFlags(&c->ev_fork, hipEventDisableTiming) != hipSuccess ||
        hipEventCreateWithFlags(&c->ev_stft, hipEventDisableTiming) != hipSuccess ||
        hipEventCreateWithFlags(&c->ev_pack, hipEventDisableTiming) != hipSuccess ||
        hipEventCreateWithFlags(&c->ev_join, hipEventDisableTiming) != hipSuccess) {
        (void)hipGetLastError();
        c->aux = nullptr;
    }
    c->grp_floats = c->ws_floats - c->grp_off;
    c->ws_floats = c->grp_off + (size_t)c->G * c->grp_floats;
    if (c->G > 1 && sagen_ctx::off_grouped(c)) {
        sagen_destroy_impl(c);
        return fail(SAGEN_ERR_UNSUPPORTED, "sagen_create_grouped: the grouped launch runs the default kernels only (an environment switch selected others)");
    }
    *out = c;
    return SAGEN_OK;
}

int sagen_bind_impl(sagen_ctx* c, const sagen_tensor* tensors, int n, void* workspace, size_t workspace_bytes,
                    hipStream_t s) {
    if (!c || !tensors || !workspace) return fail(SAGEN_ERR_NULL, "sagen_bind_weights: null argument");
    if (workspace_bytes < c->ws_floats * sizeof(float))
        return fail(SAGEN_ERR_WORKSPACE, "workspace has %zu bytes, need %zu", workspace_bytes, c->ws_floats * sizeof(float));
    if (((uintptr_t)workspace) % 256) return fail(SAGEN_ERR_WORKSPACE, "workspace must be 256-byte aligned");
    c->ws = (float*)workspace;
    std::vector<const float*> ptr(c->vars.size(), nullptr);
    for (int i = 0; i < n; ++i) {
        const sagen_tensor& t = tensors[i];
        if (!t.name || !t.data) return fail(SAGEN_ERR_NULL, "tensor %d has a null name or data pointer", i);
        auto it = c->var_index.find(t.name);
        if (it == c->var_index.end()) continue;
        const VarSpec& vs = c->vars[it->second];
        bool ok = t.ndim == vs.ndim;
        for (int k = 0; ok && k < vs.ndim; ++k) ok = t.shape[k] == vs.shape[k];
        if (!ok) return fail(SAGEN_ERR_WEIGHTS, "variable %s has the wrong shape", t.name);
        if (((uintptr_t)t.data) % 16) return fail(SAGEN_ERR_WEIGHTS, "variable %s is not 16-byte aligned", t.name);
        ptr[it->second] = t.data;
    }
    for (size_t i = 0; i < c->vars.size(); ++i) {
        const std::string& nm = c->vars[i].name;
        const bool moving = nm.find("/moving_") != std::string::npos;
        if (!ptr[i] && !moving) return fail(SAGEN_ERR_WEIGHTS, "variable %s was not provided", nm.c_str());
    }
    c->var_ptr = ptr;
    c->pack_jobs.clear();
    c->h2_jobs.clear();
    for (int g = 0; g < c->G; ++g) {
        const size_t go = (size_t)g * c->grp_floats;
        SAGEN_HIP_CHECK(hipMemsetAsync(c->p("h2s") + go, 0, 256 * sizeof(float), s));
        SAGEN_HIP_CHECK(hipMemsetAsync(c->p("splitk:tk") + go, 0, SK_TICKETS * sizeof(int), s));
        SAGEN_HIP_CHECK(hipMemsetAsync(c->p("splitk_aux:tk") + go, 0, SK_TICKETS * sizeof(int), s));
    }
    int rc = fft_tables_ensure(s);
    if (rc) return rc;
    rc = sagen_repack_impl(c, s);
    if (rc) return rc;
    for (int g = 1; g < c->G; ++g)
        SAGEN_HIP_CHECK(hipMemcpyAsync(c->p("h2s") + (size_t)g * c->grp_floats + H2S_FILTER_FIRST, c->p("h2s") + H2S_FILTER_FIRST,
                                       (H2S_FIXED_FIRST - H2S_FILTER_FIRST) * sizeof(float), hipMemcpyDeviceToDevice, s));
    c->bound = true;
    return SAGEN_OK;
}

static PackJob forward_pack_job(const sagen_ctx* c, const VarSpec& vs, const PkSpec& k, bool scatter = false) {
    PackJob j;
    j.src = c->v(vs.name);
    j.dst = c->p((scatter ? "pks:" : "pk:") + vs.name);
    if (scatter) {
        j.kind = PACK_ROWS; j.N = k.Ns; j.Kpad = k.Ks;
        j.p[0] = k.Ns; j.p[1] = k.Ks;
    } else {
        j.kind = k.kind; j.N = k.N; j.Kpad = k.Kpad;
        std::copy(k.p, k.p + 7, j.p);
    }
    return j;
}

int sagen_upload_pack_jobs(std::vector<PackJob>& jobs, void* dev, hipStream_t s) {
    int nb = 0;
    for (auto& j : jobs) { j.first_block = nb; nb += pack_job_blocks(j.kind, j.N, j.Kpad); }
    if (!jobs.empty() && hipMemcpyAsync(dev, jobs.data(), jobs.size() * sizeof(PackJob), hipMemcpyHostToDevice, s) != hipSuccess) return -1;
    return nb;
}

int sagen_repack_part(sagen_ctx* c, hipStream_t s, int part) {
    if (c->pack_jobs.empty()) {
        for (int pass = 0; pass < 2; ++pass) {
            for (const auto& vs : c->vars) {
                if (!is_weights(vs.name)) continue;
                const PkSpec k = pk_spec(vs);
                if (k.stem == (pass == 0)) c->pack_jobs.push_back(forward_pack_job(c, vs, k));
                if (pass == 1 && k.Ns) c->pack_jobs.push_back(forward_pack_job(c, vs, k, true));
            }
            if (pass == 0) c->pack_early_jobs = (int)c->pack_jobs.size();
        }
        if (c->pack_jobs.size() * sizeof(PackJob) > c->bufs.at("pk:jobs").n * sizeof(float)) return fail(SAGEN_ERR_WORKSPACE, "pack job table too small");
        c->pack_blocks = sagen_upload_pack_jobs(c->pack_jobs, c->p("pk:jobs"), s);
        if (c->pack_blocks < 0) return fail(SAGEN_ERR_HIP, "pack job upload failed");
        c->pack_early_blocks = c->pack_early_jobs < (int)c->pack_jobs.size() ? c->pack_jobs[c->pack_early_jobs].first_block : c->pack_blocks;
    }
    const PackJob* jobs = reinterpret_cast<const PackJob*>(c->p("pk:jobs"));
    const int ne = c->pack_early_jobs, be = c->pack_early_blocks, n = (int)c->pack_jobs.size();
    int rc = SAGEN_OK;
    if (part == 1) return ne > 0 ? pack_multi_launch(jobs, ne, be, s) : SAGEN_OK;
    if (part == 2) rc = n > ne ? pack_multi_launch(jobs + ne, n - ne, c->pack_blocks - be, s, be) : SAGEN_OK;
    else rc = pack_multi_launch(jobs, n, c->pack_blocks, s);
    if (rc || c->fp32_only || !c->use_p3) return rc;
    if (c->h2_jobs.empty()) {
        c->h2_jobs.assign(c->h2_slot.size(), H2Job());
        for (const auto& vs : c->vars) {
            if (!is_weights(vs.name)) continue;
            const PkSpec k = pk_spec(vs);
            auto job = [&](const std::string& key, const char* from, const char* to, int N, int Kpad) {
                const int slot = c->h2_slot.at(key);
                H2Job& j = c->h2_jobs[slot - H2S_FILTER_FIRST];
                j.N = N; j.Kpad = Kpad;
                j.wp = c->p(from + vs.name); j.w2 = c->p(to + vs.name); j.w_inv = c->p("h2s") + slot;
            };
            const std::string lname = vs.name.substr(0, vs.name.size() - 8);
            if (k.h2) job(lname, "pk:", "pkh:", k.N, k.Kpad);
            if (k.Ns) job("pks:" + lname, "pks:", "pkhs:", k.Ns, k.Ks);
        }
        int nb = 0;
        for (H2Job& j : c->h2_jobs) { j.first_block = nb; nb += (int)(((long)j.N * j.Kpad + 1023) / 1024); }
        c->h2_blocks = nb;
        if (c->h2_jobs.size() * sizeof(H2Job) > c->bufs.at("h2:jobs").n * sizeof(float)) return fail(SAGEN_ERR_WORKSPACE, "fp16x2 job table too small");
        if (!c->h2_jobs.empty() && hipMemcpyAsync(c->p("h2:jobs"), c->h2_jobs.data(), c->h2_jobs.size() * sizeof(H2Job), hipMemcpyHostToDevice, s) != hipSuccess)
            return fail(SAGEN_ERR_HIP, "fp16x2 job upload failed");
    }
    return h2_filter_pack_multi_launch(reinterpret_cast<const H2Job*>(c->p("h2:jobs")), (int)c->h2_jobs.size(), c->h2_blocks,
                                       reinterpret_cast<unsigned*>(c->p("h2:amax")), s);
}
int sagen_repack_impl(sagen_ctx* c, hipStream_t s) { return sagen_repack_part(c, s, 0); }
bool sagen_forward_forks(const sagen_ctx* c) {
    static const bool one_stream = getenv("SAGEN_ONE_STREAM") != nullptr;
    return c->aux && !c->tuning && !one_stream && (c->has_video || c->has_flow);
}


int sagen_forward_impl(sagen_ctx* c, const float* audio, const float* video, const float* flow, float* out, hipStream_t s) {
    if (!c || !audio || !out) return fail(SAGEN_ERR_NULL, "sagen_forward: null argument");
    if (!c->bound) return fail(SAGEN_ERR_WEIGHTS, "sagen_forward: weights are not bound");
    if (c->has_video && !video) return fail(SAGEN_ERR_NULL, "sagen_forward: video encoder enabled but video is NULL");
    if (c->has_flow && !flow) return fail(SAGEN_ERR_NULL, "sagen_forward: flow encoder enabled but flow is NULL");
    const int B = c->B;
    c->events_used = 0;
    c->prof.clear();
    struct GroupScope {
        GroupInfo saved;
        explicit GroupScope(const GroupInfo& gi) : saved(cur_group()) { cur_group() = gi; }
        ~GroupScope() { cur_group() = saved; }
    } group_scope(c->group_info());
    if (c->G > 1) {
        if (c->train_mode) return fail(SAGEN_ERR_UNSUPPORTED, "the training step has no grouped launch");
        if (!c->freq_mask || sagen_ctx::off_grouped(c) ||
            (c->has_video && !c->video_u8 && !c->stem16) || (c->has_video && c->video_u8 && !c->stem8) || (c->has_flow && !c->stem16))
            return fail(SAGEN_ERR_UNSUPPORTED, "grouped forward: an option moved the path off the kernels that take a group dimension "
                        "(fp16x2 / planes_from_stage / plane_gather / u8_fast_stem / f16_fast_stem must keep their defaults)");
    }

    const bool forked = sagen_forward_forks(c);
    Fwd f{c, s};
    Fwd g{c, forked ? c->aux : s};
    auto bail = [&](int rc) {
        if (forked) {
            if (hipEventRecord(c->ev_join, c->aux) == hipSuccess) (void)hipStreamWaitEvent(s, c->ev_join, 0);
            else (void)hipStreamSynchronize(c->aux);
        }
        return rc;
    };
    if (forked) {
        g.wsname = "splitk_aux";
        SAGEN_HIP_CHECK(hipEventRecord(c->ev_fork, s));
        SAGEN_HIP_CHECK(hipStreamWaitEvent(c->aux, c->ev_fork, 0));
    }

    const bool no_d1p = c->no_d1_planes;
    bool d1_planes = !no_d1p && !c->sk_fused && c->freq_mask && !c->train_mode && !c->materialize_mask && !c->fp32_only && c->nsep == 32 && c->nin == 1 && f.h2() &&
                     c->bufs.count("cat1p") != 0 && c->h2_slot.count("separation/deconv1") != 0 && getenv("SAGEN_NO_MASKFUSE") == nullptr;
    if (d1_planes && !c->tuning) {
        auto it = c->plan.find("separation/deconv1");
        if (it != c->plan.end() && !igemm_tile_p3((IgemmTile)it->second.tile)) d1_planes = false;
    }
    const bool no_decp = c->dec_planes_min_batch > (1 << 29);
    static const bool train_no_decp = getenv("SAGEN_TRAIN_NO_DEC_PLANES") != nullptr;
    const bool dec_planes = !no_decp && c->B >= c->dec_planes_min_batch && !c->sk_fused && c->freq_mask && !(c->train_mode && (train_no_decp || !c->train_bands)) &&
                            !c->fp32_only && f.h2() && c->bufs.count("catp") != 0 && !c->no_scatter;
    const bool want_amax = d1_planes || dec_planes;

    g.layer = "stft";
    if (c->nin == 1)
        g.timed("stft_kernel", 0.0, [&] { return stft_launch(audio, B, c->snd_size, 46, 173, c->p("mag"), 89, 117, c->p("spec"), g.s,
                                                             want_amax ? c->p("amax") : nullptr, 10 * H2_AMAX_FLOATS + 64); });
    else
        g.timed("stft_multi_kernel", 0.0, [&] { return stft_multi_launch(audio, B, c->snd_size, c->nin, 46, 173, c->p("mag"), 89, 117, c->p("spec"), g.s,
                                                                         want_amax ? c->p("amax") : nullptr, 10 * H2_AMAX_FLOATS + 64); });
    if (forked) {
        SAGEN_HIP_CHECK(hipEventRecord(c->ev_stft, c->aux));
        f.wait_before_mfma = c->ev_stft;
    }
    if (c->late_repack) {
        c->late_repack = false;
        if (!forked) return bail(fail(SAGEN_ERR_UNSUPPORTED, "late repack without a second stream"));
        const int rc = sagen_repack_part(c, c->aux, 2);
        if (rc) return bail(rc);
        SAGEN_HIP_CHECK(hipEventRecord(c->ev_pack, c->aux));
        f.wait_packs = c->ev_pack;
    }

    for (int l = 0; l < 5 && !g.rc; ++l) {
        const std::string name = "audio_encoder/conv" + std::to_string(l + 1);
        const int ce = c->enc_c[l + 1];
        float* y = c->p("cat" + std::to_string(l + 1)) + (l == 4 ? 0 : ce);
        int Ho, Wo;
        IgemmDesc d;
        if (l == 0 && c->nin > 1) {
            d = g.conv_desc(c->p("mag"), 127, 1024, c->nin, c->nin, c->p("pk:" + name + "/weights"), 7, 16, 4, 8, false, ce, y, 2 * ce, Ho, Wo);
        } else if (l == 0) {
            d = g.conv_desc(c->p("mag"), 127, 1024, 16, 1, c->p("pk:" + name + "/weights"), 7, 1, 4, 8, false, ce, y, 2 * ce, Ho, Wo);
            Wo = c->enc_w[1];
            d.M = B * Ho * Wo; d.Wg = Wo; d.Wlim = Wo;
            d.y_rstride = (long)Wo * 2 * ce; d.y_bstride = (long)Ho * Wo * 2 * ce;
        } else {
            const int cp = c->enc_c[l];
            const float* x = c->p("cat" + std::to_string(l)) + (l == 5 ? 0 : cp);
            d = g.conv_desc(x, c->enc_h[l], c->enc_w[l], cp, 2 * cp, c->p("pk:" + name + "/weights"), AENC_K[l][0], AENC_K[l][1],
                            AENC_S[l][0], AENC_S[l][1], false, ce, y, 2 * ce, Ho, Wo);
        }
        d.bias = c->v(name + "/biases");
        d.relu_out = 1;
        if (want_amax) d.amax_out = g.cat_amax(l + 1, 1);
        g.layer = name;
        bool aud_planes = l >= 1 && want_amax && !c->no_aud_planes && f.h2() && c->bufs.count("aencp") != 0 && g.has_h2_filter(name) &&
                          conv3g_ok_desc(d, c->enc_c[l]);
        if (aud_planes && !c->tuning) {
            auto it = c->plan.find(name);
            if (it != c->plan.end() ? !igemm_tile_p3((IgemmTile)it->second.tile)
                                    : B < 128)
                aud_planes = false;
        }
        if (aud_planes) {
            const int cp = c->enc_c[l], Hl = c->enc_h[l], Wl = c->enc_w[l];
            float* const a_inv = c->p("amax") + (size_t)10 * H2_AMAX_FLOATS + 8 + l;
            g.layer = name + "/planes";
            g.timed("h2_pack_rows_kernel", 0.0, [&] {
                return h2_pack_rows_launch(c->p("cat" + std::to_string(l)) + cp, (long)Hl * Wl * 2 * cp, (long)Wl * 2 * cp, 2 * cp, 0, B, Hl, Wl, cp,
                                           g.cat_amax(l, 1), nullptr, c->p("aencp"), a_inv, g.h2_sat_count(), g.s); });
            g.layer = name;
            const Fwd::H2Filter w = g.h2_filter(name);
            igemm_set_h2_planes(d, c->p("aencp"), B, Hl, Wl, cp, w.w2, a_inv, w.w_inv);
        }
        g.gemm(d);
    }

    float* bott = c->p("bott");
    const bool fcm = c->use_fcm && !c->train_mode && !c->tuning;
    auto fcm_layer = [&](Fwd& w, const std::string& label, int M, int K, const std::vector<FcmSeg>& segs, const std::vector<std::string>& names, const std::vector<int>& Ns) {
        FcmDesc fd;
        fd.M = M; fd.K = K; fd.nseg = (int)segs.size(); fd.njobs = (int)names.size(); fd.nslices = c->fcm_slices.at(names[0]);
        for (size_t q = 0; q < segs.size(); ++q) fd.seg[q] = segs[q];
        double fl = 0.0;
        for (size_t j = 0; j < names.size(); ++j) {
            fd.job[j].w = c->v(names[j] + "/weights"); fd.job[j].N = Ns[j]; fd.job[j].out = c->p("fcm:" + names[j]);
            fl += 2.0 * M * K * Ns[j];
        }
        w.layer = label;
        w.timed(M <= 32 ? "fcm_kernel<1>" : (M <= 64 ? "fcm_kernel<2>" : "fcm_kernel<3>"), fl, [&] { return fcm_launch(fd, w.s); });
    };
    auto fcm_finish = [&](Fwd& w, const std::string& name, int rows, int N, bool relu, float* y, int ldy, int rep, float* amax_out = nullptr) {
        w.layer = name;
        w.timed("splitk_reduce_kernel", 0.0, [&] {
            return splitk_reduce_launch(c->p("fcm:" + name), c->fcm_slices.at(name), rows, N, c->v(name + "/biases"), relu ? 1 : 0, y, ldy, rep, nullptr, w.s, amax_out); });
    };
    if (fcm) {
        std::vector<FcmSeg> segs(6);
        for (int wq = 0; wq < 6; ++wq) {
            segs[wq].p = c->p("cat5") + (size_t)wq * 1024; segs[wq].k0 = wq * 512; segs[wq].k1 = (wq + 1) * 512; segs[wq].ld = 6 * 1024;
        }
        fcm_layer(g, "bottleneck/audio-fc", B * 3, 6 * 512, segs, {"bottleneck/audio-fc"}, {1024});
        fcm_finish(g, "bottleneck/audio-fc", B * 3, 1024, true, bott, c->Cb, 1);
    } else {
        IgemmDesc d;
        d.x = c->p("cat5"); d.w = c->p("pk:bottleneck/audio-fc/weights"); d.y = bott; d.bias = c->v("bottleneck/audio-fc/biases");
        d.M = B * 3; d.N = 1024; d.K = 6 * 512; d.Kpad = d.K;
        d.Hg = 3; d.Wg = 1; d.Hin = 3; d.Win = 6; d.Cin = 512; d.ldx = 1024; d.x_bstride = 3L * 6 * 1024;
        d.ntaps = 6; d.TW = 6; d.log2Cin = 9;
        d.Cout = 1024; d.Hlim = 3; d.Wlim = 1; d.ldy = c->Cb; d.y_rstride = c->Cb; d.y_bstride = 3L * c->Cb;
        d.relu_out = 1;
        g.layer = "bottleneck/audio-fc";
        g.gemm(d);
    }
    int choff = 1024;
    for (int e = 0; e < 2; ++e) {
        const bool on = e == 0 ? c->has_video : c->has_flow;
        if (!on) continue;
        const std::string enc = e == 0 ? "video" : "flow";
        Fwd& w = (e == 1 && c->has_video) ? g : f;
        w.sfx = (e == 1 && c->has_video) ? "_b" : "";
        const float* feat = c->train_mode ? w.resnet_train(e == 0 ? video : flow, enc + "_encoder")
                                          : w.resnet(e == 0 ? video : flow, enc + "_encoder");
        w.fc(feat, B * 98, 512, 512, "bottleneck/" + enc + "-fc-red", 128, true, c->p("fcred" + w.sfx), 128);
        if (fcm) {
            FcmSeg sg;
            sg.p = c->p("fcred" + w.sfx); sg.k0 = 0; sg.k1 = 98 * 128; sg.ld = 98 * 128;
            fcm_layer(w, "bottleneck/" + enc + "-fc", B, 98 * 128, {sg}, {"bottleneck/" + enc + "-fc"}, {512});
            fcm_finish(w, "bottleneck/" + enc + "-fc", B, 512, true, bott + choff, c->Cb, 3);
        } else {
            w.fc(c->p("fcred" + w.sfx), B, 98 * 128, 98 * 128, "bottleneck/" + enc + "-fc", 512, true, bott + choff, c->Cb, 3);
        }
        choff += 512;
    }
    if (f.rc || g.rc) return bail(f.rc ? f.rc : g.rc);
    if (forked) {
        SAGEN_HIP_CHECK(hipEventRecord(c->ev_join, c->aux));
        SAGEN_HIP_CHECK(hipStreamWaitEvent(s, c->ev_join, 0));
    }

    static const bool no_fork2 = getenv("SAGEN_NO_FORK2") != nullptr;
    const bool fork2 = forked && c->freq_mask && !no_fork2;
    const int nlast_fcm = c->nout * c->nin * (c->nsep + 1);
    if (fcm) {
        const int M3 = B * 3, nl = c->cfg.n_loc_units;
        auto plain = [&](const float* x, int K) { FcmSeg sg; sg.p = x; sg.k0 = 0; sg.k1 = K; sg.ld = K; return sg; };
        std::vector<std::string> names{"localization/fc1"};
        std::vector<int> Ns{nl > 0 ? c->cfg.loc_units[0] : nlast_fcm};
        if (c->freq_mask) { names.push_back("separation/fc-feats"); Ns.push_back(512); }
        fcm_layer(f, c->freq_mask ? "localization/fc1+separation/fc-feats" : "localization/fc1", M3, c->Cb, {plain(bott, c->Cb)}, names, Ns);
        if (c->freq_mask) fcm_finish(f, "separation/fc-feats", M3, 512, true, c->p("cat5") + 512, 1024, 6, want_amax ? f.cat_amax(5, 0) : nullptr);
        if (fork2) {
            SAGEN_HIP_CHECK(hipEventRecord(c->ev_fork, s));
            SAGEN_HIP_CHECK(hipStreamWaitEvent(c->aux, c->ev_fork, 0));
        }
        Fwd& w = fork2 ? g : f;
        int K = Ns[0];
        for (int i = 1; i <= nl; ++i) {
            const std::string prev = "localization/fc" + std::to_string(i), cur = "localization/fc" + std::to_string(i + 1);
            const int N = i < nl ? c->cfg.loc_units[i] : nlast_fcm;
            float* y = c->p("loc" + std::to_string(i));
            fcm_finish(w, prev, M3, K, true, y, K, 1);
            fcm_layer(w, cur, M3, K, {plain(y, K)}, {cur}, {N});
            K = N;
        }
        fcm_finish(w, "localization/fc" + std::to_string(nl + 1), M3, nlast_fcm, false, c->p("coeffs"), nlast_fcm, 1);
        if (f.rc || g.rc) return bail(f.rc ? f.rc : g.rc);
    } else {
    if (fork2) {
        SAGEN_HIP_CHECK(hipEventRecord(c->ev_fork, s));
        SAGEN_HIP_CHECK(hipStreamWaitEvent(c->aux, c->ev_fork, 0));
    }
    {
        Fwd& w = fork2 ? g : f;
        const float* x = bott;
        int K = c->Cb;
        for (int i = 0; i < c->cfg.n_loc_units; ++i) {
            float* y = c->p("loc" + std::to_string(i + 1));
            w.fc(x, B * 3, K, K, "localization/fc" + std::to_string(i + 1), c->cfg.loc_units[i], true, y, c->cfg.loc_units[i]);
            x = y; K = c->cfg.loc_units[i];
        }
        const int nlast = c->nout * c->nin * (c->nsep + 1);
        w.fc(x, B * 3, K, K, "localization/fc" + std::to_string(c->cfg.n_loc_units + 1), nlast, false, c->p("coeffs"), nlast);
        if (f.rc || g.rc) return bail(f.rc ? f.rc : g.rc);
    }
    }

    if (!c->freq_mask) {
        f.layer = "decoder";
        if (c->nin == 1)
            f.timed("nosep_mix_kernel", 0.0, [&] { return nosep_mix_launch(audio, c->p("coeffs"), out, B, c->snd_size, c->snd_contx, c->snd_dur, 3, s); });
        else
            f.timed("nosep_mix_multi_kernel", 0.0, [&] {
                return nosep_mix_multi_launch(audio, c->p("coeffs"), out, B, c->snd_size, c->snd_contx, c->snd_dur, c->nin, c->nout, s); });
        return f.rc;
    }

    if (!fcm)
        f.fc(bott, B * 3, c->Cb, c->Cb, "separation/fc-feats", 512, true, c->p("cat5") + 512, 1024, 6,
             want_amax ? f.cat_amax(5, 0) : nullptr);
    const bool no_scatter = c->no_scatter;
    const bool lean = (!c->train_mode || c->train_bands) && !c->fp32_only && !no_scatter;
    int need_lo[7], need_hi[7];
    for (int l = 1; l <= 5; ++l) { need_lo[l] = 0; need_hi[l] = c->enc_h[l]; }
    if (lean) {
        need_lo[1] = 10; need_hi[1] = 17;
        for (int l = 1; l <= 4; ++l) {
            const int sh = AENC_S[l][0], kh = AENC_K[l][0];
            need_lo[l + 1] = std::max((need_lo[l] - (kh - 1) + sh - 1) / sh, 0);
            need_hi[l + 1] = std::min((need_hi[l] - 1) / sh + 1, c->enc_h[l + 1]);
        }
    }
    for (int l = 1; l <= 5; ++l) { c->dec_lo[l] = need_lo[l]; c->dec_hi[l] = need_hi[l]; }
    for (int l = 4; l >= 1; --l) {
        const int Cin = 2 * c->enc_c[l + 1];
        float* const am = want_amax ? f.cat_amax(l, 0) : nullptr;
        if (lean && c->bufs.count("pks:separation/deconv" + std::to_string(l + 1) + "/weights")) {
            f.deconv_scatter(c->p("cat" + std::to_string(l + 1)), c->enc_h[l + 1], c->enc_w[l + 1], Cin, l, c->p("cat" + std::to_string(l)),
                             2 * c->enc_c[l], true, need_lo[l + 1], need_hi[l + 1] - need_lo[l + 1], need_lo[l], need_hi[l], am, dec_planes);
            continue;
        }
        f.deconv(c->p("cat" + std::to_string(l + 1)), c->enc_h[l + 1], c->enc_w[l + 1], Cin, l, c->p("cat" + std::to_string(l)),
                 2 * c->enc_c[l], true, 0, 0, 0, 0, 0, nullptr, nullptr, 0, [am](IgemmDesc& d) { d.amax_out = am; });
    }
    static const bool no_maskfuse = getenv("SAGEN_NO_MASKFUSE") != nullptr;
    const bool fused_tail = !no_maskfuse && !c->train_mode && !c->materialize_mask && !c->fp32_only && c->nsep == 32 && c->nin == 1;
    c->mask_fused_last = fused_tail;
    if (fork2 && fused_tail) {
        SAGEN_HIP_CHECK(hipEventRecord(c->ev_join, c->aux));
        SAGEN_HIP_CHECK(hipStreamWaitEvent(s, c->ev_join, 0));
    }
    float* const ebuf = fused_tail ? c->p("dmask") : nullptr;
    std::function<void(IgemmDesc&)> d1_tweak = nullptr;
    if (d1_planes && fused_tail) {
        const int W1 = c->enc_w[1], C1 = 2 * c->enc_c[1];
        f.layer = "separation/cat1-planes";
        f.timed("h2_pack_rows_kernel", 0.0, [&] {
            return h2_pack_rows_launch(c->p("cat1"), (long)c->enc_h[1] * W1 * C1, (long)W1 * C1, C1, 10, B, 7, W1, C1, f.cat_amax(1, 0), f.cat_amax(1, 1), c->p("cat1p"),
                                       f.cat_a_inv(1), f.h2_sat_count(), s); });
        const Fwd::H2Filter w = f.h2_filter("separation/deconv1");
        const void* planes = c->p("cat1p");
        const float* a_inv = f.cat_a_inv(1);
        d1_tweak = [=](IgemmDesc& d) { igemm_set_h2_planes(d, planes, B, 7, W1, C1, w.w2, a_inv, w.w_inv, 10, 7); };
    }
    const int nmask = c->nsep * c->nin;
    f.deconv(c->p("cat1"), 31, 127, 64, 0, c->p("dmask"), nmask, false, 11, 17, 67, 23L * 1024 * nmask, 44, c->p("coeffs"), ebuf, 23, d1_tweak);
    if (fork2 && !fused_tail) {
        SAGEN_HIP_CHECK(hipEventRecord(c->ev_join, c->aux));
        SAGEN_HIP_CHECK(hipStreamWaitEvent(s, c->ev_join, 0));
    }
    f.layer = "separation/mask-istft-mix";
    if (c->nin > 1) {
        f.timed("mask_istft_hoa_kernel+ola_mix_hoa_kernel", 0.0, [&] {
            return mask_istft_hoa_launch(c->p("dmask"), 23L * 1024 * nmask, 1, c->p("spec"), c->p("coeffs"), B, c->nsep, c->nin, c->nout, out,
                                         c->p("frames"), s); });
        return f.rc;
    }
    f.timed("mask_istft_kernel+ola_mix_kernel", 0.0, [&] {
        return mask_istft_mix_launch(c->p("dmask"), 23L * 1024 * c->nsep, 1, c->p("spec"), c->p("coeffs"), B, c->nsep, out,
                                     c->p("frames"), s, ebuf); });
    return f.rc;
}
int sagen_forward_u8_impl(sagen_ctx* c, const float* audio, const uint8_t* video_u8, const float* flow, float* out, hipStream_t s) {
    if (!c) return fail(SAGEN_ERR_NULL, "sagen_forward_u8: null ctx");
    if (!c->has_video) return fail(SAGEN_ERR_UNSUPPORTED, "sagen_forward_u8: the video encoder is not enabled");
    c->video_u8 = true;
    const int rc = sagen_forward_impl(c, audio, reinterpret_cast<const float*>(video_u8), flow, out, s);
    c->video_u8 = false;
    return rc;
}
void sagen_destroy_impl(sagen_ctx* c) {
    if (!c) return;
    for (hipEvent_t e : c->event_pool) (void)hipEventDestroy(e);
    if (c->tune_e0) { (void)hipEventDestroy(c->tune_e0); (void)hipEventDestroy(c->tune_e1); }
    if (c->ev_fork) (void)hipEventDestroy(c->ev_fork);
    if (c->ev_join) (void)hipEventDestroy(c->ev_join);
    if (c->ev_stft) (void)hipEventDestroy(c->ev_stft);
    if (c->ev_pack) (void)hipEventDestroy(c->ev_pack);
    if (c->aux) (void)hipStreamDestroy(c->aux);
    delete c;
}


int sagen_autotune_impl(sagen_ctx* c, const float* audio, const float* video, const float* flow, float* out, hipStream_t s) {
    if (!c) return fail(SAGEN_ERR_NULL, "sagen_autotune: null ctx");
    if (getenv("SAGEN_NO_AUTOTUNE")) return SAGEN_OK;
    if (!c->tune_e0) {
        SAGEN_HIP_CHECK(hipEventCreate(&c->tune_e0));
        SAGEN_HIP_CHECK(hipEventCreate(&c->tune_e1));
    }
    c->plan.clear();
    c->materialize.clear();
    c->tuning = true;
    const int rc = sagen_forward_impl(c, audio, video, flow, out, s);
    c->tuning = false;
    if (rc) { c->plan.clear(); return rc; }
    SAGEN_HIP_CHECK(hipStreamSynchronize(s));
    return SAGEN_OK;
}

int sagen_plan_set_impl(sagen_ctx* c, const char* layer, int tile, int splitk) {
    const std::string name(layer);
    const std::string sfx = "#materialize";
    if (name.size() > sfx.size() && name.compare(name.size() - sfx.size(), sfx.size(), sfx) == 0) {
        c->materialize[name.substr(0, name.size() - sfx.size())] = splitk != 0;
        return SAGEN_OK;
    }
    if (tile < 0 || tile >= (int)TILE_AUTO || splitk < 1 || splitk > 64) return fail(SAGEN_ERR_SHAPE, "sagen_plan_set: tile=%d splitk=%d", tile, splitk);
    Choice ch;
    ch.tile = tile; ch.splitk = splitk;
    c->plan[layer] = ch;
    return SAGEN_OK;
}

int sagen_plan_describe_impl(sagen_ctx* c, char* buf, size_t buflen) {
    std::string out;
    for (const auto& kv : c->plan) {
        char line[512];
        snprintf(line, sizeof line, "%s\t%s\t%d\t%.2f\n", kv.first.c_str(), igemm_tile_name((IgemmTile)kv.second.tile),
                 kv.second.splitk, kv.second.us);
        out += line;
    }
    int n = (int)c->plan.size();
    for (const auto& kv : c->materialize) {
        out += kv.first + "#materialize\t-\t" + (kv.second ? "1" : "0") + "\t0\n";
        ++n;
    }
    if (out.size() + 1 > buflen) return fail(SAGEN_ERR_WORKSPACE, "plan description needs %zu bytes", out.size() + 1);
    memcpy(buf, out.c_str(), out.size() + 1);
    return n;
}

int sagen_profile_enable_impl(sagen_ctx* c, int on) {
    c->profiling = on != 0;
    c->prof.clear();
    c->events_used = 0;
    return SAGEN_OK;
}

int sagen_profile_report_impl(sagen_ctx* c, char* buf, size_t buflen) {
    std::string out;
    for (const ProfRec& r : c->prof) {
        float ms = 0.f;
        hipError_t e = hipEventSynchronize(r.e1);
        if (e == hipSuccess) e = hipEventElapsedTime(&ms, r.e0, r.e1);
        if (e != hipSuccess) return fail(SAGEN_ERR_HIP, "profile: %s", hipGetErrorString(e));
        char line[512];
        snprintf(line, sizeof line, "%s\t%s\t%.3f\t%.6g\n", r.kernel.c_str(), r.layer.c_str(), ms * 1e3, r.flops);
        out += line;
    }
    if (out.size() + 1 > buflen) return fail(SAGEN_ERR_WORKSPACE, "profile report needs %zu bytes", out.size() + 1);
    memcpy(buf, out.c_str(), out.size() + 1);
    return (int)c->prof.size();
}
size_t sagen_workspace_bytes_impl(const sagen_ctx* c) { return c->ws_floats * sizeof(float); }
int sagen_num_variables_impl(const sagen_ctx* c) { return (int)c->vars.size(); }
int sagen_variable_spec_impl(const sagen_ctx* c, int i, const char** name, int32_t* ndim, int64_t shape[4]) {
    if (i < 0 || i >= (int)c->vars.size()) return fail(SAGEN_ERR_SHAPE, "variable index %d out of range", i);
    *name = c->vars[i].name.c_str();
    *ndim = c->vars[i].ndim;
    for (int k = 0; k < 4; ++k) shape[k] = c->vars[i].shape[k];
    return SAGEN_OK;
}
int sagen_set_option_impl(sagen_ctx* c, const char* name, int value) {
    const std::string n = name;
    if (n == "materialize_mask") { c->materialize_mask = value != 0; return SAGEN_OK; }
    if (n == "intermediate_group") {
        if (value < 0 || value >= c->G) return fail(SAGEN_ERR_SHAPE, "intermediate_group=%d of %d groups", value, c->G);
        c->inter_group = value;
        return SAGEN_OK;
    }
    if (n == "u8_fast_stem") { c->stem8 = value != 0; return SAGEN_OK; }
    if (n == "f16_fast_stem") { c->stem16 = value != 0; return SAGEN_OK; }
    if (n == "u8_stem_h2") { c->stem8h = value != 0; return SAGEN_OK; }
    if (n == "train_bands") { c->train_bands = value != 0; return SAGEN_OK; }
    if (n == "train_rawpool") { c->train_rawpool = value != 0; return SAGEN_OK; }
    if (n == "fp16x2") { c->use_h2 = value != 0; return SAGEN_OK; }
    if (n == "planes_from_stage") { if (value < 2 || value > 6) return fail(SAGEN_ERR_SHAPE, "planes_from_stage in 2..6"); c->p3_from_stage = value; return SAGEN_OK; }
    if (n == "decoder_planes") { c->dec_planes_min_batch = value ? 1 : (1 << 30); return SAGEN_OK; }
    if (n == "plane_gather") { c->use_p3g = c->use_p3 && value != 0; return SAGEN_OK; }
    if (n == "plane_s2d") { c->use_s2d = value != 0; return SAGEN_OK; }
    return fail(SAGEN_ERR_UNSUPPORTED, "sagen_set_option: unknown option %s", name);
}

int sagen_counter_impl(sagen_ctx* c, const char* name, uint64_t* value, hipStream_t s) {
    if (!c->ws) return fail(SAGEN_ERR_WORKSPACE, "no workspace bound");
    if (std::string(name) != "fp16x2_saturations") return fail(SAGEN_ERR_UNSUPPORTED, "sagen_counter: unknown counter %s", name);
    unsigned v[SAGEN_MAX_GROUPS] = {0};
    for (int g = 0; g < c->G; ++g)
        SAGEN_HIP_CHECK(hipMemcpyAsync(&v[g], c->p("h2s") + (size_t)g * c->grp_floats + H2S_SAT_COUNT, sizeof(unsigned), hipMemcpyDeviceToHost, s));
    SAGEN_HIP_CHECK(hipStreamSynchronize(s));
    uint64_t tot = 0;
    for (int g = 0; g < c->G; ++g) tot += v[g];
    *value = tot;
    return SAGEN_OK;
}

int sagen_get_intermediate_impl(const sagen_ctx* c, const char* name, const float** data, int32_t* ndim, int64_t shape[4],
                                int64_t* pixel_stride) {
    if (!c->ws) return fail(SAGEN_ERR_WORKSPACE, "no workspace bound");
    auto it = c->named.find(name);
    if (it == c->named.end()) return fail(SAGEN_ERR_SHAPE, "unknown intermediate %s", name);
    const Named& nm = it->second;
    if (c->mask_fused_last && std::string(name) == "separation/deconv1")
        return fail(SAGEN_ERR_UNSUPPORTED, "separation/deconv1: the last forward fused the mask into the deconvolution's epilogue - "
                    "sagen_set_option(ctx, \"materialize_mask\", 1) keeps the logits");
    *data = c->ws + nm.buf.off + nm.extra_off + (size_t)c->inter_group * c->grp_floats;
    *ndim = nm.ndim;
    for (int k = 0; k < 4; ++k) shape[k] = nm.shape[k];
    *pixel_stride = nm.pixel_stride;
    return SAGEN_OK;
}
```

spatialaudiogen_amd/csrc/stem8.hip:

```cpp
#include "igemm3_common.h"
#include "h2_planes.h"

namespace sagen {

constexpr int S8_PH = 8, S8_PW = 7;
constexpr int S8_RH = 2 * S8_PH + 1;
constexpr int S8_RW = 2 * S8_PW + 1;
constexpr int S8_M = S8_RH * S8_RW;
__device__ __forceinline__ int s8_slot(int m) { return m ^ ((m >> 1) & 1); }
constexpr int S8_UH = 229, S8_UW = 456;
constexpr int S8_NH = 32;
constexpr int S8_W_BYTES = 14 * 3 * S8_NH * 32;
constexpr int S8_CT_BYTES = 256 * S8_NH * 4;
constexpr int S8_THREADS = 512;
constexpr int S8_LDS = S8_W_BYTES + S8_CT_BYTES + 2 * 8 * S8_NH * 4 + S8_NH * 4;
typedef _Float16 f16x8s __attribute__((ext_vector_type(8)));

size_t stem8_plane_bytes(int B) { return (size_t)B * S8_UH * S8_UW * 8; }

template <bool HALF>
__global__ __launch_bounds__(256) void stem8_prep_kernel(const unsigned char* __restrict__ x_, u32x2* __restrict__ plane_, int B,
                                                         float* __restrict__ zero_ptr_, long zero_n, const GroupInfo gi) {
    const unsigned char* __restrict__ x = x_ + (size_t)blockIdx.z * ((size_t)B * 224 * 448 * 3);
    u32x2* __restrict__ plane = SAGEN_GRP(plane_);
    float* __restrict__ zero_ptr = SAGEN_GRP(zero_ptr_);
    const long total = (long)B * S8_UH * S8_UW;
    for (long i = (long)blockIdx.x * 256 + threadIdx.x; i < zero_n; i += (long)gridDim.x * 256) zero_ptr[i] = 0.f;
    auto conv = [](unsigned u) -> unsigned {
        return HALF ? (unsigned)__builtin_bit_cast(unsigned short, (_Float16)(float)((int)u - 128))
                    : __builtin_bit_cast(unsigned, (float)((int)u - 128)) >> 16;
    };
    constexpr int QW = S8_UW / 4;
    static_assert(S8_UW % 4 == 0, "plane rows are whole quads");
    const long nquad = (long)B * S8_UH * QW;
    const unsigned border = HALF ? 0xB800u : 0xBF00u;
    for (long iq = (long)blockIdx.x * 256 + threadIdx.x; iq < nquad; iq += (long)gridDim.x * 256) {
        long p = iq;
        const int q = (int)(p % QW); p /= QW;
        const int h = (int)(p % S8_UH) - 2;
        const int b = (int)(p / S8_UH);
        const int w0 = 4 * q - 2;
        u32x2 o[4];
        if ((unsigned)h < 224u && w0 >= 0 && w0 + 3 < 448) {
            const long ob = (((long)b * 224 + h) * 448 + w0) * 3;
            constexpr unsigned sh = 2;
            const unsigned* src = reinterpret_cast<const unsigned*>(x + (ob - sh));
            const unsigned d[4] = {src[0], src[1], src[2], src[3]};
            unsigned by[12];
#pragma unroll
            for (int k = 0; k < 12; ++k) by[k] = (d[(sh + k) >> 2] >> (8 * ((sh + k) & 3))) & 0xffu;
#pragma unroll
            for (int k = 0; k < 4; ++k) o[k] = u32x2{conv(by[3 * k]) | (conv(by[3 * k + 1]) << 16), conv(by[3 * k + 2])};
        } else {
#pragma unroll
            for (int k = 0; k < 4; ++k) {
                const int w = w0 + k;
                unsigned c0 = border, c1 = border, c2 = border;
                if ((unsigned)h < 224u && (unsigned)w < 448u) {
                    const unsigned char* src = x + (((long)b * 224 + h) * 448 + w) * 3;
                    c0 = conv(src[0]); c1 = conv(src[1]); c2 = conv(src[2]);
                }
                o[k] = u32x2{c0 | (c1 << 16), c2};
            }
        }
        u32x4* dst = reinterpret_cast<u32x4*>(plane + iq * 4);
        dst[0] = u32x4{o[0][0], o[0][1], o[1][0], o[1][1]};
        dst[1] = u32x4{o[2][0], o[2][1], o[3][0], o[3][1]};
    }
    (void)total;
}

template <int OUT, int MODE = 0>
__global__ __launch_bounds__(S8_THREADS, 2) void stem8pool_kernel(const char* __restrict__ plane_, const float* __restrict__ wf32,
                                                                  const char* __restrict__ wplanes, const float* __restrict__ gamma,
                                                                  float* __restrict__ pooled_, double* __restrict__ stats_, int B,
                                                                  long plane_stride, const float* __restrict__ a_inv_, const float* __restrict__ w_inv_,
                                                                  float* __restrict__ raw2_, const GroupInfo gi) {
    const char* __restrict__ plane = SAGEN_GRP(plane_);
    float* __restrict__ pooled = SAGEN_GRP(pooled_);
    double* __restrict__ stats = SAGEN_GRP(stats_);
    const float* __restrict__ a_inv = SAGEN_GRP(a_inv_);
    const float* __restrict__ w_inv = SAGEN_GRP(w_inv_);
    float* __restrict__ raw2 = SAGEN_GRP(raw2_);
    constexpr bool F16 = MODE != 0;
    constexpr int NPLA = MODE == 1 ? 2 : 1, NPLW = MODE == 0 ? 3 : 2;
    constexpr int W_BYTES = 14 * NPLW * S8_NH * 32;
    extern __shared__ __attribute__((aligned(16))) char smem[];
    char* const wl = smem;
    char* const pa = smem + S8_W_BYTES;
    float* const ct = reinterpret_cast<float*>(smem + S8_W_BYTES);
    float* const red = reinterpret_cast<float*>(smem + S8_W_BYTES + S8_CT_BYTES);
    float* const cb = reinterpret_cast<float*>(smem + S8_W_BYTES + S8_CT_BYTES + 2 * 8 * S8_NH * 4);
    const int tid = threadIdx.x;
    const int lane = tid & 63;
    const int wave = __builtin_amdgcn_readfirstlane(tid >> 6);
    const int li = lane & 31, g = lane >> 5;
    const int nh = blockIdx.x & 1;
    const int wg = blockIdx.x >> 1, nwg = gridDim.x >> 1;

    for (int i = tid; i < W_BYTES / 16; i += S8_THREADS) {
        const int row = i >> 1, hf = i & 1;
        const int kp = row >> 5, n = row & 31;
        reinterpret_cast<f32x4*>(wl)[i] = *reinterpret_cast<const f32x4*>(wplanes + ((long)(kp * 64 + nh * 32 + n) * 32 + 16 * (hf ^ ((n >> 3) & 1))));
    }
    if (tid < S8_NH) {
        double s = 0.0;
        if (MODE != 1)
            for (int k = 0; k < 224; ++k) s += (double)wf32[(nh * S8_NH + tid) * 224 + k];
        cb[tid] = (float)(s * (0.5 / 255.0));
    }
    const float osc = MODE == 1 ? a_inv[0] * w_inv[0] : (MODE == 2 ? w_inv[0] * (1.f / 255.f) : 1.f / 255.f);
    const int pch4 = tid & 7;
    bool use_min[4];
#pragma unroll
    for (int k = 0; k < 4; ++k) use_min[k] = OUT == 1 ? false : gamma[nh * S8_NH + 4 * pch4 + k] < 0.f;
    constexpr bool SGN = OUT == 0;
    float sgn4[4];
#pragma unroll
    for (int k = 0; k < 4; ++k) sgn4[k] = (SGN && use_min[k]) ? -1.f : 1.f;
    const float sgn_l = (SGN && gamma[nh * S8_NH + li] < 0.f) ? -1.f : 1.f;
    int poff[9];
    {
        const int p = tid >> 3;
        const int pr_l = p / S8_PW, pc_l = p - pr_l * S8_PW;
#pragma unroll
        for (int dr = 0; dr < 3; ++dr)
#pragma unroll
            for (int dc = 0; dc < 3; ++dc) poff[dr * 3 + dc] = s8_slot((2 * pr_l + dr) * S8_RW + 2 * pc_l + dc) * S8_NH + 4 * pch4;
    }
    unsigned own = 0;
#pragma unroll
    for (int e = 0; e < 16; ++e) {
        const int m = wave * 32 + (e & 3) + 8 * (e >> 2) + 4 * g;
        const int r = m / S8_RW, c = m - r * S8_RW;
        if (m < S8_M && r < 2 * S8_PH && c < 2 * S8_PW) own |= 1u << e;
    }
    float ssum = 0.f, ssq = 0.f;
    __syncthreads();
    const float cbl = cb[li] * sgn_l;
    const float osc_l = osc * sgn_l;

    const int npatch = B * 7 * 16;
    constexpr int PROWS = 2 * (S8_RH - 1) + 7, PCH = (2 * (S8_RW - 1) + 8) / 2;
    constexpr int NCHUNK = PROWS * PCH;
    constexpr int PATCH_BYTES = NCHUNK * 16;
    static_assert(NCHUNK <= 2 * S8_THREADS && NPLA * PATCH_BYTES <= S8_CT_BYTES, "patch staging");
    const int ck0 = tid, ck1 = tid + S8_THREADS;
    const int cr0 = ck0 / PCH, cc0 = ck0 - cr0 * PCH, cr1 = ck1 / PCH, cc1 = ck1 - cr1 * PCH;
    auto patch_src = [&](int patch, int crow, int ccol) {
        const int b = patch / 112, rem = patch - b * 112;
        const int pr = rem >> 4, pc = rem & 15;
        const int row = min(2 * 16 * pr + crow, S8_UH - 1);
        return plane + (((long)b * S8_UH + row) * S8_UW + 2 * 14 * pc) * 8 + ccol * 16;
    };
    f32x4 ld0[NPLA], ld1[NPLA];
#pragma unroll
    for (int p = 0; p < NPLA; ++p) {
        ld0[p] = f32x4{0.f, 0.f, 0.f, 0.f}; ld1[p] = ld0[p];
        if (wg < npatch) {
            ld0[p] = *reinterpret_cast<const f32x4*>(patch_src(wg, cr0, cc0) + p * plane_stride);
            if (ck1 < NCHUNK) ld1[p] = *reinterpret_cast<const f32x4*>(patch_src(wg, cr1, cc1) + p * plane_stride);
        }
    }
    int aoff;
    {
        const int m = wave * 32 + li;
        int r = m / S8_RW, c = m - r * S8_RW;
        if (m >= S8_M) { r = 0; c = 0; }
        aoff = ((2 * r) * (2 * PCH) + 2 * c + 2 * g) * 8;
    }
    for (int patch = wg; patch < npatch; patch += nwg) {
        const int b = patch / 112, rem = patch - b * 112;
        const int pr = rem >> 4, pc = rem & 15;
        const int R0 = 16 * pr, C0 = 14 * pc;
#pragma unroll
        for (int p = 0; p < NPLA; ++p) {
            reinterpret_cast<f32x4*>(pa + p * PATCH_BYTES)[ck0] = ld0[p];
            if (ck1 < NCHUNK) reinterpret_cast<f32x4*>(pa + p * PATCH_BYTES)[ck1] = ld1[p];
        }
        __syncthreads();
        const int next_patch = patch + nwg;
        if (next_patch < npatch) {
#pragma unroll
            for (int p = 0; p < NPLA; ++p) {
                ld0[p] = *reinterpret_cast<const f32x4*>(patch_src(next_patch, cr0, cc0) + p * plane_stride);
                if (ck1 < NCHUNK) ld1[p] = *reinterpret_cast<const f32x4*>(patch_src(next_patch, cr1, cc1) + p * plane_stride);
            }
        }
        f32x16 acc[2];
#pragma unroll
        for (int j = 0; j < 2; ++j)
#pragma unroll
            for (int e = 0; e < 16; ++e) acc[j][e] = 0.f;
#pragma unroll
        for (int ks = 0; ks < 14; ++ks) {
            bf16x8 fa[NPLA], fb[NPLW];
#pragma unroll
            for (int p = 0; p < NPLA; ++p) fa[p] = *reinterpret_cast<const bf16x8*>(pa + p * PATCH_BYTES + aoff + ((ks >> 1) * (2 * PCH) + (ks & 1) * 4) * 8);
#pragma unroll
            for (int pl = 0; pl < NPLW; ++pl) fb[pl] = *reinterpret_cast<const bf16x8*>(wl + ((ks * NPLW + pl) * S8_NH + li) * 32 + 16 * (g ^ ((li >> 3) & 1)));
            const int a = ks & 1;
            if constexpr (MODE == 2) {
                acc[a] = __builtin_amdgcn_mfma_f32_32x32x16_f16(__builtin_bit_cast(f16x8s, fa[0]), __builtin_bit_cast(f16x8s, fb[1]), acc[a], 0, 0, 0);
                acc[a ^ 1] = __builtin_amdgcn_mfma_f32_32x32x16_f16(__builtin_bit_cast(f16x8s, fa[0]), __builtin_bit_cast(f16x8s, fb[0]), acc[a ^ 1], 0, 0, 0);
            } else if constexpr (F16) {
                acc[a] = __builtin_amdgcn_mfma_f32_32x32x16_f16(__builtin_bit_cast(f16x8s, fa[NPLA - 1]), __builtin_bit_cast(f16x8s, fb[0]), acc[a], 0, 0, 0);
                acc[a ^ 1] = __builtin_amdgcn_mfma_f32_32x32x16_f16(__builtin_bit_cast(f16x8s, fa[0]), __builtin_bit_cast(f16x8s, fb[NPLW - 1]), acc[a ^ 1], 0, 0, 0);
                acc[a] = __builtin_amdgcn_mfma_f32_32x32x16_f16(__builtin_bit_cast(f16x8s, fa[0]), __builtin_bit_cast(f16x8s, fb[0]), acc[a], 0, 0, 0);
            } else {
                acc[a] = __builtin_amdgcn_mfma_f32_32x32x16_bf16(fa[0], fb[NPLW - 1], acc[a], 0, 0, 0);
                acc[a ^ 1] = __builtin_amdgcn_mfma_f32_32x32x16_bf16(fa[0], fb[1], acc[a ^ 1], 0, 0, 0);
                acc[a] = __builtin_amdgcn_mfma_f32_32x32x16_bf16(fa[0], fb[0], acc[a], 0, 0, 0);
            }
        }
        __syncthreads();
#pragma unroll
        for (int e = 0; e < 16; ++e) {
            const float v = fmaf(acc[0][e] + acc[1][e], osc_l, cbl);
            ct[s8_slot(wave * 32 + (e & 3) + 8 * (e >> 2) + 4 * g) * S8_NH + li] = v;
            const float vo = ((own >> e) & 1u) ? v : 0.f;
            ssum += vo;
            ssq = fmaf(vo, vo, ssq);
        }
        __syncthreads();
        if (OUT >= 1) {
            float* const raw = OUT == 2 ? raw2 : pooled;
            for (int it = tid; it < 2 * S8_PH * 2 * S8_PW * 8; it += S8_THREADS) {
                const int p = it >> 3, q4 = it & 7;
                const int r = p / (2 * S8_PW), cc = p - r * (2 * S8_PW);
                *reinterpret_cast<float4*>(raw + (((long)b * 112 + R0 + r) * 224 + C0 + cc) * 64 + nh * S8_NH + 4 * q4) =
                    *reinterpret_cast<const float4*>(ct + s8_slot(r * S8_RW + cc) * S8_NH + 4 * q4);
            }
        }
        if (OUT != 1 && tid < S8_PH * S8_PW * 8) {
            const int p = tid >> 3;
            const int pr_l = p / S8_PW, pc_l = p - pr_l * S8_PW;
            float4 v[9];
            if (pr < 6 && pc < 15) {
#pragma unroll
                for (int k = 0; k < 9; ++k) v[k] = *reinterpret_cast<const float4*>(ct + poff[k]);
            } else {
#pragma unroll
                for (int dr = 0; dr < 3; ++dr)
#pragma unroll
                    for (int dc = 0; dc < 3; ++dc) {
                        const int rr = (R0 + 2 * pr_l + dr >= 112) ? 2 * pr_l : 2 * pr_l + dr;
                        const int cc = (C0 + 2 * pc_l + dc >= 224) ? 2 * pc_l : 2 * pc_l + dc;
                        v[dr * 3 + dc] = *reinterpret_cast<const float4*>(ct + s8_slot(rr * S8_RW + cc) * S8_NH + 4 * pch4);
                    }
            }
            float4 ext = v[0];
            if constexpr (SGN) {
#pragma unroll
                for (int k = 1; k < 9; ++k) {
                    ext.x = fmaxf(ext.x, v[k].x); ext.y = fmaxf(ext.y, v[k].y); ext.z = fmaxf(ext.z, v[k].z); ext.w = fmaxf(ext.w, v[k].w);
                }
                ext.x *= sgn4[0]; ext.y *= sgn4[1]; ext.z *= sgn4[2]; ext.w *= sgn4[3];
            } else {
#pragma unroll
                for (int k = 1; k < 9; ++k) {
                    ext.x = use_min[0] ? fminf(ext.x, v[k].x) : fmaxf(ext.x, v[k].x); ext.y = use_min[1] ? fminf(ext.y, v[k].y) : fmaxf(ext.y, v[k].y);
                    ext.z = use_min[2] ? fminf(ext.z, v[k].z) : fmaxf(ext.z, v[k].z); ext.w = use_min[3] ? fminf(ext.w, v[k].w) : fmaxf(ext.w, v[k].w);
                }
            }
            *reinterpret_cast<float4*>(pooled + (((long)b * 56 + 8 * pr + pr_l) * 112 + 7 * pc + pc_l) * 64 + nh * S8_NH + 4 * pch4) = ext;
        }
        __syncthreads();
    }
    ssum *= sgn_l;
    ssum = wave_xor_add<32>(ssum);
    ssq = wave_xor_add<32>(ssq);
    if (g == 0) {
        red[(0 * 8 + wave) * S8_NH + li] = ssum;
        red[(1 * 8 + wave) * S8_NH + li] = ssq;
    }
    __syncthreads();
    if (tid < 2 * S8_NH) {
        const int which = tid >> 5, ch = tid & 31;
        float s = 0.f;
#pragma unroll
        for (int k = 0; k < 8; ++k) s += red[(which * 8 + k) * S8_NH + ch];
        atomicAdd(&stats[which * 64 + nh * S8_NH + ch], (double)s);
    }
}

int stem8_prep_launch(const unsigned char* x, void* plane, int B, hipStream_t s, float* zero_ptr, long zero_n, int half) {
    if (!x || !plane) return fail(SAGEN_ERR_NULL, "stem8_prep: null argument");
    if (((uintptr_t)x % 4) || ((uintptr_t)plane % 16)) return fail(SAGEN_ERR_UNSUPPORTED, "stem8_prep: the frames must be 4-byte aligned, the plane 16-byte aligned");
    const long total = (long)B * S8_UH * S8_UW / 4;
    const int grid = (int)std::min<long>(cdiv(total, 256), 256L * 16);
    const GroupInfo gi = cur_group();
    if (half) hipLaunchKernelGGL(stem8_prep_kernel<true>, dim3(grid, 1, gi.G), dim3(256), 0, s, x, reinterpret_cast<u32x2*>(plane), B, zero_ptr, zero_ptr ? zero_n : 0L, gi);
    else hipLaunchKernelGGL(stem8_prep_kernel<false>, dim3(grid, 1, gi.G), dim3(256), 0, s, x, reinterpret_cast<u32x2*>(plane), B, zero_ptr, zero_ptr ? zero_n : 0L, gi);
    SAGEN_LAUNCH_CHECK();
    return SAGEN_OK;
}

int stem8pool_launch(const void* plane, const float* wp, const float* gamma, float* pooled, double* stats, int B, hipStream_t s) {
    if (!plane || !wp || !gamma || !pooled || !stats) return fail(SAGEN_ERR_NULL, "stem8pool: null argument");
    static bool attr_set = false;
    if (!attr_set) {
        SAGEN_HIP_CHECK(hipFuncSetAttribute(reinterpret_cast<const void*>(stem8pool_kernel<0>), hipFuncAttributeMaxDynamicSharedMemorySize, S8_LDS));
        attr_set = true;
    }
    const char* planes = reinterpret_cast<const char*>(wp + 64 * 224);
    const int npatch = B * 7 * 16;
    hipLaunchKernelGGL(stem8pool_kernel<0>, dim3(2 * std::min(npatch, 256), 1, cur_group().G), dim3(S8_THREADS), S8_LDS, s, reinterpret_cast<const char*>(plane), wp, planes, gamma,
                       pooled, stats, B, 0L, (const float*)nullptr, (const float*)nullptr, (float*)nullptr, cur_group());
    SAGEN_LAUNCH_CHECK();
    return SAGEN_OK;
}

int stem8pool_h2_launch(const void* plane, const float* wp, const void* wh2, const float* w_inv, const float* gamma, float* pooled, double* stats, int B,
                        hipStream_t s) {
    if (!plane || !wp || !wh2 || !w_inv || !gamma || !pooled || !stats) return fail(SAGEN_ERR_NULL, "stem8pool_h2: null argument");
    static bool attr_set = false;
    if (!attr_set) {
        SAGEN_HIP_CHECK(hipFuncSetAttribute(reinterpret_cast<const void*>(stem8pool_kernel<0, 2>), hipFuncAttributeMaxDynamicSharedMemorySize, S8_LDS));
        attr_set = true;
    }
    const int npatch = B * 7 * 16;
    hipLaunchKernelGGL((stem8pool_kernel<0, 2>), dim3(2 * std::min(npatch, 256), 1, cur_group().G), dim3(S8_THREADS), S8_LDS, s, reinterpret_cast<const char*>(plane), wp,
                       reinterpret_cast<const char*>(wh2), gamma, pooled, stats, B, 0L, (const float*)nullptr, w_inv, (float*)nullptr, cur_group());
    SAGEN_LAUNCH_CHECK();
    return SAGEN_OK;
}

int stem8raw_launch(const void* plane, const float* wp, float* y0, double* stats, int B, hipStream_t s) {
    if (!plane || !wp || !y0 || !stats) return fail(SAGEN_ERR_NULL, "stem8raw: null argument");
    static bool attr_set = false;
    if (!attr_set) {
        SAGEN_HIP_CHECK(hipFuncSetAttribute(reinterpret_cast<const void*>(stem8pool_kernel<1>), hipFuncAttributeMaxDynamicSharedMemorySize, S8_LDS));
        attr_set = true;
    }
    const char* planes = reinterpret_cast<const char*>(wp + 64 * 224);
    const int npatch = B * 7 * 16;
    hipLaunchKernelGGL(stem8pool_kernel<1>, dim3(2 * std::min(npatch, 256), 1, cur_group().G), dim3(S8_THREADS), S8_LDS, s, reinterpret_cast<const char*>(plane), wp, planes,
                       (const float*)nullptr, y0, stats, B, 0L, (const float*)nullptr, (const float*)nullptr, (float*)nullptr, cur_group());
    SAGEN_LAUNCH_CHECK();
    return SAGEN_OK;
}

int stem8rawpool_launch(const void* plane, const float* wp, const float* gamma, float* y0, float* pooled, double* stats, int B, hipStream_t s) {
    if (!plane || !wp || !gamma || !y0 || !pooled || !stats) return fail(SAGEN_ERR_NULL, "stem8rawpool: null argument");
    static bool attr_set = false;
    if (!attr_set) {
        SAGEN_HIP_CHECK(hipFuncSetAttribute(reinterpret_cast<const void*>(stem8pool_kernel<2>), hipFuncAttributeMaxDynamicSharedMemorySize, S8_LDS));
        attr_set = true;
    }
    const char* planes = reinterpret_cast<const char*>(wp + 64 * 224);
    const int npatch = B * 7 * 16;
    hipLaunchKernelGGL(stem8pool_kernel<2>, dim3(2 * std::min(npatch, 256), 1, cur_group().G), dim3(S8_THREADS), S8_LDS, s, reinterpret_cast<const char*>(plane), wp, planes,
                       gamma, pooled, stats, B, 0L, (const float*)nullptr, (const float*)nullptr, y0, cur_group());
    SAGEN_LAUNCH_CHECK();
    return SAGEN_OK;
}

constexpr int S16_PARTS = 1024;
__global__ __launch_bounds__(256) void stem16_amax_kernel(const float* __restrict__ x_, long n4, float* __restrict__ part_, float* __restrict__ zero_ptr_, long zero_n, const GroupInfo gi) {
    const float* __restrict__ x = x_ + (size_t)blockIdx.z * (size_t)n4 * 4;
    float* __restrict__ part = SAGEN_GRP(part_);
    float* __restrict__ zero_ptr = SAGEN_GRP(zero_ptr_);
    for (long i = (long)blockIdx.x * 256 + threadIdx.x; i < zero_n; i += (long)gridDim.x * 256) zero_ptr[i] = 0.f;
    float m = 0.f;
    for (long i = (long)blockIdx.x * 256 + threadIdx.x; i < n4; i += (long)gridDim.x * 256) {
        const float4 v = reinterpret_cast<const float4*>(x)[i];
        m = fmaxf(m, fmaxf(fmaxf(fabsf(v.x), fabsf(v.y)), fmaxf(fabsf(v.z), fabsf(v.w))));
    }
    m = wave_max_f(m);
    __shared__ float s_m[4];
    if ((threadIdx.x & 63) == 0) s_m[threadIdx.x >> 6] = m;
    __syncthreads();
    if (threadIdx.x == 0) part[blockIdx.x] = fmaxf(fmaxf(s_m[0], s_m[1]), fmaxf(s_m[2], s_m[3]));
}
__global__ __launch_bounds__(256) void stem16_prep_kernel(const float* __restrict__ x_, u32x2* __restrict__ hi_, u32x2* __restrict__ lo_, int B,
                                                          const float* __restrict__ part_, float* __restrict__ a_inv_, const GroupInfo gi) {
    const float* __restrict__ x = x_ + (size_t)blockIdx.z * ((size_t)B * 224 * 448 * 3);
    u32x2* __restrict__ hi = SAGEN_GRP(hi_);
    u32x2* __restrict__ lo = SAGEN_GRP(lo_);
    const float* __restrict__ part = SAGEN_GRP(part_);
    float* __restrict__ a_inv = SAGEN_GRP(a_inv_);
    float m = 0.f;
    for (int i = threadIdx.x & 63; i < S16_PARTS; i += 64) m = fmaxf(m, part[i]);
    m = wave_max_f(m);
    const float sa = h2_scale_of_bound(m);
    if (blockIdx.x == 0 && threadIdx.x == 0) a_inv[0] = 1.f / sa;
    const long total = (long)B * S8_UH * S8_UW;
    for (long i = (long)blockIdx.x * 256 + threadIdx.x; i < total; i += (long)gridDim.x * 256) {
        long p = i;
        const int w = (int)(p % S8_UW) - 2; p /= S8_UW;
        const int h = (int)(p % S8_UH) - 2;
        const int b = (int)(p / S8_UH);
        unsigned short hh[3] = {0, 0, 0}, ll[3] = {0, 0, 0};
        if ((unsigned)h < 224u && (unsigned)w < 448u) {
            const float* src = x + (((long)b * 224 + h) * 448 + w) * 3;
#pragma unroll
            for (int c = 0; c < 3; ++c) {
                const float v = src[c] * sa;
                const _Float16 a = __builtin_isfinite(v) ? (_Float16)v : __builtin_bit_cast(_Float16, (unsigned short)0x7e00);
                const _Float16 r = __builtin_isfinite(v) ? (_Float16)(v - (float)a) : (_Float16)0.f;
                hh[c] = __builtin_bit_cast(unsigned short, a); ll[c] = __builtin_bit_cast(unsigned short, r);
            }
        }
        hi[i] = u32x2{(unsigned)hh[0] | ((unsigned)hh[1] << 16), (unsigned)hh[2]};
        lo[i] = u32x2{(unsigned)ll[0] | ((unsigned)ll[1] << 16), (unsigned)ll[2]};
    }
}

int stem16_prep_launch(const float* x, void* planes, float* part, float* a_inv, int B, hipStream_t s, float* zero_ptr, long zero_n) {
    if (!x || !planes || !part || !a_inv) return fail(SAGEN_ERR_NULL, "stem16_prep: null argument");
    const long n = (long)B * 224 * 448 * 3;
    if (n % 4 || ((uintptr_t)x % 16)) return fail(SAGEN_ERR_UNSUPPORTED, "stem16_prep: the frames must be 16-byte aligned");
    const GroupInfo gi = cur_group();
    hipLaunchKernelGGL(stem16_amax_kernel, dim3(S16_PARTS, 1, gi.G), dim3(256), 0, s, x, n / 4, part, zero_ptr, zero_ptr ? zero_n : 0L, gi);
    const long total = (long)B * S8_UH * S8_UW;
    char* p = reinterpret_cast<char*>(planes);
    hipLaunchKernelGGL(stem16_prep_kernel, dim3((int)std::min<long>(cdiv(total, 256), 256L * 16), 1, gi.G), dim3(256), 0, s, x, reinterpret_cast<u32x2*>(p),
                       reinterpret_cast<u32x2*>(p + stem8_plane_bytes(B)), B, part, a_inv, gi);
    SAGEN_LAUNCH_CHECK();
    return SAGEN_OK;
}

int stem16pool_launch(const void* planes, const void* wh2, const float* gamma, float* pooled, double* stats, const float* a_inv, const float* w_inv,
                      int B, hipStream_t s) {
    if (!planes || !wh2 || !gamma || !pooled || !stats || !a_inv || !w_inv) return fail(SAGEN_ERR_NULL, "stem16pool: null argument");
    static bool attr_set = false;
    if (!attr_set) {
        SAGEN_HIP_CHECK(hipFuncSetAttribute(reinterpret_cast<const void*>(stem8pool_kernel<0, 1>), hipFuncAttributeMaxDynamicSharedMemorySize, S8_LDS));
        attr_set = true;
    }
    const int npatch = B * 7 * 16;
    hipLaunchKernelGGL((stem8pool_kernel<0, 1>), dim3(2 * std::min(npatch, 256), 1, cur_group().G), dim3(S8_THREADS), S8_LDS, s, reinterpret_cast<const char*>(planes),
                       (const float*)nullptr, reinterpret_cast<const char*>(wh2), gamma, pooled, stats, B, (long)stem8_plane_bytes(B), a_inv, w_inv, (float*)nullptr, cur_group());
    SAGEN_LAUNCH_CHECK();
    return SAGEN_OK;
}

}
```

Baseline: 3214.

## Hold stem filter in registers with 4-wave blocks and bank-rotated patch layout

Adds a REGS variant of the fused stem conv+pool kernel for the fp16x2 u8 path. In it the whole 14-step filter fragment set lives in VGPRs instead of LDS, blocks shrink to 4 waves that each process two M tiles, and the input patch moves to a separate LDS region with a rotated, padded layout. A software-pipelined A-fragment prefetch and double-buffered patch staging are also added. The aim is to cut LDS traffic and bank conflicts for the B operand and to overlap the patch load with MFMA work, at the cost of higher register pressure and fewer threads per block.

```diff
diff --git a/spatialaudiogen_amd/csrc/kernels.h b/spatialaudiogen_amd/csrc/kernels.h
--- a/spatialaudiogen_amd/csrc/kernels.h
+++ b/spatialaudiogen_amd/csrc/kernels.h
@@ -185,7 +185,7 @@
 size_t stem8_plane_bytes(int B);
 int stem8_prep_launch(const unsigned char* x, void* plane, int B, hipStream_t s, float* zero_ptr = nullptr, long zero_n = 0, int half = 0);
 int stem8pool_h2_launch(const void* plane, const float* wp, const void* wh2, const float* w_inv, const float* gamma, float* pooled, double* stats, int B,
-                        hipStream_t s);
+                        hipStream_t s, int regs = 1);
 int stem8pool_launch(const void* plane, const float* wp, const float* gamma, float* pooled, double* stats, int B, hipStream_t s);
 int stem16_prep_launch(const float* x, void* planes, float* part, float* a_inv, int B, hipStream_t s, float* zero_ptr = nullptr, long zero_n = 0);
 int stem16pool_launch(const void* planes, const void* wh2, const float* gamma, float* pooled, double* stats, const float* a_inv, const float* w_inv,
diff --git a/spatialaudiogen_amd/csrc/model.h b/spatialaudiogen_amd/csrc/model.h
--- a/spatialaudiogen_amd/csrc/model.h
+++ b/spatialaudiogen_amd/csrc/model.h
@@ -178,6 +178,7 @@
     int dec_planes_min_batch = 16;
     bool use_fcm = false;
     std::map<std::string, int> fcm_slices;
+    bool stem8regs = true;
     bool stem8h = true;
     bool stem16 = true;
     bool stem8 = true;
@@ -675,7 +676,7 @@
                 else if (fast8h)
                     timed("stem8pool_kernel<h2>", 2.0 * B * H * W * 64 * 224, [&] {
                         return stem8pool_h2_launch(c->p("xpad" + sfx), c->p("pk:" + name + "/weights"), h2_filter(name).w2, h2_filter(name).w_inv,
-                                                   c->v(name + "/bn/gamma"), c->p("rx0" + sfx), bn_acc(li), B, s); });
+                                                   c->v(name + "/bn/gamma"), c->p("rx0" + sfx), bn_acc(li), B, s, c->stem8regs ? 1 : 0); });
                 else
                 timed("stem8pool_kernel", 2.0 * B * H * W * 64 * 224, [&] {
                     return stem8pool_launch(c->p("xpad" + sfx), c->p("pk:" + name + "/weights"), c->v(name + "/bn/gamma"), c->p("rx0" + sfx), bn_acc(li), B, s); });
diff --git a/spatialaudiogen_amd/csrc/model.hip b/spatialaudiogen_amd/csrc/model.hip
--- a/spatialaudiogen_amd/csrc/model.hip
+++ b/spatialaudiogen_amd/csrc/model.hip
@@ -40,6 +40,7 @@
     c->stem8 = getenv("SAGEN_NO_STEM8") == nullptr;
     c->stem16 = getenv("SAGEN_NO_STEM16") == nullptr;
     c->stem8h = getenv("SAGEN_NO_STEM8_H2") == nullptr;
+    c->stem8regs = getenv("SAGEN_NO_STEM8_REGS") == nullptr;
     c->use_h2 = getenv("SAGEN_NO_H2") == nullptr;
     c->train_h2 = getenv("SAGEN_TRAIN_NO_H2") == nullptr;
     c->train_h2d = getenv("SAGEN_TRAIN_NO_H2D") == nullptr;
@@ -781,6 +782,7 @@
     if (n == "u8_fast_stem") { c->stem8 = value != 0; return SAGEN_OK; }
     if (n == "f16_fast_stem") { c->stem16 = value != 0; return SAGEN_OK; }
     if (n == "u8_stem_h2") { c->stem8h = value != 0; return SAGEN_OK; }
+    if (n == "u8_stem_regs") { c->stem8regs = value != 0; return SAGEN_OK; }
     if (n == "train_bands") { c->train_bands = value != 0; return SAGEN_OK; }
     if (n == "train_rawpool") { c->train_rawpool = value != 0; return SAGEN_OK; }
     if (n == "fp16x2") { c->use_h2 = value != 0; return SAGEN_OK; }
diff --git a/spatialaudiogen_amd/csrc/stem8.hip b/spatialaudiogen_amd/csrc/stem8.hip
--- a/spatialaudiogen_amd/csrc/stem8.hip
+++ b/spatialaudiogen_amd/csrc/stem8.hip
@@ -1,5 +1,6 @@
 #include "igemm3_common.h"
 #include "h2_planes.h"
+#include "stem8_layout.h"
 
 namespace sagen {
 
@@ -12,8 +13,18 @@
 constexpr int S8_NH = 32;
 constexpr int S8_W_BYTES = 14 * 3 * S8_NH * 32;
 constexpr int S8_CT_BYTES = 256 * S8_NH * 4;
-constexpr int S8_THREADS = 512;
-constexpr int S8_LDS = S8_W_BYTES + S8_CT_BYTES + 2 * 8 * S8_NH * 4 + S8_NH * 4;
+static_assert(S8_RW == S8L_RW && S8_M == S8L_M, "stem8_layout.h describes this patch");
+template <int MODE, bool REGS> struct S8Cfg {
+    static_assert(!REGS || MODE == 2, "the filter fits the register file in MODE 2 only (14 x 2 fragments = 112 VGPRs)");
+    static constexpr int NPLA = MODE == 1 ? 2 : 1, NPLW = MODE == 0 ? 3 : 2;
+    static constexpr int WAVES = REGS ? 4 : 8, THREADS = 64 * WAVES, TPW = 8 / WAVES;
+    static constexpr int W_LDS = REGS ? 0 : S8_W_BYTES;
+    static constexpr int PATCH_BYTES = s8l_plane_bytes(NPLA);
+    static constexpr int PA_LDS = REGS ? NPLA * PATCH_BYTES : 0;
+    static constexpr int LDS = W_LDS + S8_CT_BYTES + PA_LDS + 2 * 8 * S8_NH * 4 + S8_NH * 4;
+    static_assert(NPLA * PATCH_BYTES <= S8_CT_BYTES, "patch staging");
+    static_assert(2 * LDS <= 160 * 1024, "two workgroups per CU");
+};
 typedef _Float16 f16x8s __attribute__((ext_vector_type(8)));
 
 size_t stem8_plane_bytes(int B) { return (size_t)B * S8_UH * S8_UW * 8; }
@@ -70,8 +81,8 @@
     (void)total;
 }
 
-template <int OUT, int MODE = 0>
-__global__ __launch_bounds__(S8_THREADS, 2) void stem8pool_kernel(const char* __restrict__ plane_, const float* __restrict__ wf32,
+template <int OUT, int MODE = 0, bool REGS = false>
+__global__ __launch_bounds__((S8Cfg<MODE, REGS>::THREADS), 2) void stem8pool_kernel(const char* __restrict__ plane_, const float* __restrict__ wf32,
                                                                   const char* __restrict__ wplanes, const float* __restrict__ gamma,
                                                                   float* __restrict__ pooled_, double* __restrict__ stats_, int B,
                                                                   long plane_stride, const float* __restrict__ a_inv_, const float* __restrict__ w_inv_,
@@ -82,15 +93,18 @@
     const float* __restrict__ a_inv = SAGEN_GRP(a_inv_);
     const float* __restrict__ w_inv = SAGEN_GRP(w_inv_);
     float* __restrict__ raw2 = SAGEN_GRP(raw2_);
+    using Cfg = S8Cfg<MODE, REGS>;
     constexpr bool F16 = MODE != 0;
-    constexpr int NPLA = MODE == 1 ? 2 : 1, NPLW = MODE == 0 ? 3 : 2;
+    constexpr int NPLA = Cfg::NPLA, NPLW = Cfg::NPLW;
     constexpr int W_BYTES = 14 * NPLW * S8_NH * 32;
+    constexpr int WAVES = Cfg::WAVES, THREADS = Cfg::THREADS, TPW = Cfg::TPW;
+    constexpr int PATCH_BYTES = Cfg::PATCH_BYTES;
     extern __shared__ __attribute__((aligned(16))) char smem[];
     char* const wl = smem;
-    char* const pa = smem + S8_W_BYTES;
-    float* const ct = reinterpret_cast<float*>(smem + S8_W_BYTES);
-    float* const red = reinterpret_cast<float*>(smem + S8_W_BYTES + S8_CT_BYTES);
-    float* const cb = reinterpret_cast<float*>(smem + S8_W_BYTES + S8_CT_BYTES + 2 * 8 * S8_NH * 4);
+    float* const ct = reinterpret_cast<float*>(smem + Cfg::W_LDS);
+    char* const pa = smem + Cfg::W_LDS + (REGS ? S8_CT_BYTES : 0);
+    float* const red = reinterpret_cast<float*>(smem + Cfg::W_LDS + S8_CT_BYTES + Cfg::PA_LDS);
+    float* const cb = red + 2 * 8 * S8_NH;
     const int tid = threadIdx.x;
     const int lane = tid & 63;
     const int wave = __builtin_amdgcn_readfirstlane(tid >> 6);
@@ -98,10 +112,19 @@
     const int nh = blockIdx.x & 1;
     const int wg = blockIdx.x >> 1, nwg = gridDim.x >> 1;
 
-    for (int i = tid; i < W_BYTES / 16; i += S8_THREADS) {
-        const int row = i >> 1, hf = i & 1;
-        const int kp = row >> 5, n = row & 31;
-        reinterpret_cast<f32x4*>(wl)[i] = *reinterpret_cast<const f32x4*>(wplanes + ((long)(kp * 64 + nh * 32 + n) * 32 + 16 * (hf ^ ((n >> 3) & 1))));
+    bf16x8 fbr[REGS ? 14 : 1][NPLW];
+    if constexpr (REGS) {
+#pragma unroll
+        for (int ks = 0; ks < 14; ++ks)
+#pragma unroll
+            for (int pl = 0; pl < NPLW; ++pl)
+                fbr[ks][pl] = *reinterpret_cast<const bf16x8*>(wplanes + ((long)((ks * NPLW + pl) * 64 + nh * S8_NH + li) * 32 + 16 * g));
+    } else {
+        for (int i = tid; i < W_BYTES / 16; i += THREADS) {
+            const int row = i >> 1, hf = i & 1;
+            const int kp = row >> 5, n = row & 31;
+            reinterpret_cast<f32x4*>(wl)[i] = *reinterpret_cast<const f32x4*>(wplanes + ((long)(kp * 64 + nh * 32 + n) * 32 + 16 * (hf ^ ((n >> 3) & 1))));
+        }
     }
     if (tid < S8_NH) {
         double s = 0.0;
@@ -110,6 +133,9 @@
         cb[tid] = (float)(s * (0.5 / 255.0));
     }
     const float osc = MODE == 1 ? a_inv[0] * w_inv[0] : (MODE == 2 ? w_inv[0] * (1.f / 255.f) : 1.f / 255.f);
+    constexpr int NPOOL = S8_PH * S8_PW * 8, PTH = THREADS >= NPOOL ? NPOOL : NPOOL / 2, PI = NPOOL / PTH;
+    constexpr int PROUND = (PTH / 8 / S8_PW) * 2 * S8_RW;
+    static_assert(PTH <= THREADS && PTH % (8 * S8_PW) == 0 && PROUND % 4 == 0, "a round of the pool is whole pooled rows");
     const int pch4 = tid & 7;
     bool use_min[4];
 #pragma unroll
@@ -128,12 +154,16 @@
 #pragma unroll
             for (int dc = 0; dc < 3; ++dc) poff[dr * 3 + dc] = s8_slot((2 * pr_l + dr) * S8_RW + 2 * pc_l + dc) * S8_NH + 4 * pch4;
     }
-    unsigned own = 0;
-#pragma unroll
-    for (int e = 0; e < 16; ++e) {
-        const int m = wave * 32 + (e & 3) + 8 * (e >> 2) + 4 * g;
-        const int r = m / S8_RW, c = m - r * S8_RW;
-        if (m < S8_M && r < 2 * S8_PH && c < 2 * S8_PW) own |= 1u << e;
+    unsigned own[TPW];
+#pragma unroll
+    for (int t = 0; t < TPW; ++t) {
+        own[t] = 0;
+#pragma unroll
+        for (int e = 0; e < 16; ++e) {
+            const int m = (wave * TPW + t) * 32 + (e & 3) + 8 * (e >> 2) + 4 * g;
+            const int r = m / S8_RW, c = m - r * S8_RW;
+            if (m < S8_M && r < 2 * S8_PH && c < 2 * S8_PW) own[t] |= 1u << e;
+        }
     }
     float ssum = 0.f, ssq = 0.f;
     __syncthreads();
@@ -141,129 +171,167 @@
     const float osc_l = osc * sgn_l;
 
     const int npatch = B * 7 * 16;
-    constexpr int PROWS = 2 * (S8_RH - 1) + 7, PCH = (2 * (S8_RW - 1) + 8) / 2;
+    constexpr int PROWS = S8L_PROWS, PCH = S8L_PCH;
+    static_assert(PROWS == 2 * (S8_RH - 1) + 7 && PCH == (2 * (S8_RW - 1) + 8) / 2, "patch geometry");
     constexpr int NCHUNK = PROWS * PCH;
-    constexpr int PATCH_BYTES = NCHUNK * 16;
-    static_assert(NCHUNK <= 2 * S8_THREADS && NPLA * PATCH_BYTES <= S8_CT_BYTES, "patch staging");
-    const int ck0 = tid, ck1 = tid + S8_THREADS;
-    const int cr0 = ck0 / PCH, cc0 = ck0 - cr0 * PCH, cr1 = ck1 / PCH, cc1 = ck1 - cr1 * PCH;
-    auto patch_src = [&](int patch, int crow, int ccol) {
+    constexpr int NS = (NCHUNK + THREADS - 1) / THREADS;
+    static_assert((NS - 1) * THREADS < NCHUNK, "patch staging");
+    const bool last_chunk = tid + (NS - 1) * THREADS < NCHUNK;
+    auto opaque_tid = [&]() { int t = tid; asm volatile("" : "+v"(t)); return t; };
+    auto patch_src = [&](int patch, int crow_, int ccol_) {
         const int b = patch / 112, rem = patch - b * 112;
         const int pr = rem >> 4, pc = rem & 15;
-        const int row = min(2 * 16 * pr + crow, S8_UH - 1);
-        return plane + (((long)b * S8_UH + row) * S8_UW + 2 * 14 * pc) * 8 + ccol * 16;
+        const int row = min(2 * 16 * pr + crow_, S8_UH - 1);
+        return plane + (((long)b * S8_UH + row) * S8_UW + 2 * 14 * pc) * 8 + ccol_ * 16;
     };
-    f32x4 ld0[NPLA], ld1[NPLA];
-#pragma unroll
-    for (int p = 0; p < NPLA; ++p) {
-        ld0[p] = f32x4{0.f, 0.f, 0.f, 0.f}; ld1[p] = ld0[p];
-        if (wg < npatch) {
-            ld0[p] = *reinterpret_cast<const f32x4*>(patch_src(wg, cr0, cc0) + p * plane_stride);
-            if (ck1 < NCHUNK) ld1[p] = *reinterpret_cast<const f32x4*>(patch_src(wg, cr1, cc1) + p * plane_stride);
-        }
-    }
-    int aoff;
-    {
-        const int m = wave * 32 + li;
-        int r = m / S8_RW, c = m - r * S8_RW;
-        if (m >= S8_M) { r = 0; c = 0; }
-        aoff = ((2 * r) * (2 * PCH) + 2 * c + 2 * g) * 8;
+    f32x4 ld[NS][NPLA];
+    auto prefetch = [&](int patch) {
+        const int t0 = opaque_tid();
+#pragma unroll
+        for (int i = 0; i < NS; ++i) {
+            const int ck = t0 + i * THREADS, crow = ck / PCH, ccol = ck - crow * PCH;
+#pragma unroll
+            for (int p = 0; p < NPLA; ++p)
+                if (i < NS - 1 || last_chunk) ld[i][p] = *reinterpret_cast<const f32x4*>(patch_src(patch, crow, ccol) + p * plane_stride);
+        }
+    };
+    auto stage = [&]() {
+        const int t0 = opaque_tid();
+#pragma unroll
+        for (int i = 0; i < NS; ++i) {
+            const int soff = s8l_stage_off(NPLA, t0 + i * THREADS);
+#pragma unroll
+            for (int p = 0; p < NPLA; ++p)
+                if (i < NS - 1 || last_chunk) *reinterpret_cast<f32x4*>(pa + p * PATCH_BYTES + soff) = ld[i][p];
+        }
+    };
+#pragma unroll
+    for (int i = 0; i < NS; ++i)
+#pragma unroll
+        for (int p = 0; p < NPLA; ++p) ld[i][p] = f32x4{0.f, 0.f, 0.f, 0.f};
+    if (wg < npatch) prefetch(wg);
+    if constexpr (REGS) {
+        if (wg < npatch) stage();
+        __syncthreads();
+        if (wg + nwg < npatch) prefetch(wg + nwg);
     }
     for (int patch = wg; patch < npatch; patch += nwg) {
         const int b = patch / 112, rem = patch - b * 112;
         const int pr = rem >> 4, pc = rem & 15;
         const int R0 = 16 * pr, C0 = 14 * pc;
-#pragma unroll
-        for (int p = 0; p < NPLA; ++p) {
-            reinterpret_cast<f32x4*>(pa + p * PATCH_BYTES)[ck0] = ld0[p];
-            if (ck1 < NCHUNK) reinterpret_cast<f32x4*>(pa + p * PATCH_BYTES)[ck1] = ld1[p];
+        const int next_patch = patch + nwg;
+        if constexpr (!REGS) {
+            stage();
+            __syncthreads();
+            if (next_patch < npatch) prefetch(next_patch);
+        }
+#pragma unroll
+        for (int t = 0; t < TPW; ++t) {
+            const int tile = wave * TPW + t;
+            int m_l = tile * 32 + li;
+            asm volatile("" : "+v"(m_l));
+            f32x16 acc[2];
+#pragma unroll
+            for (int j = 0; j < 2; ++j)
+#pragma unroll
+                for (int e = 0; e < 16; ++e) acc[j][e] = 0.f;
+            constexpr int DEPTH = REGS ? 2 : 0;
+            bf16x8 faq[DEPTH + 1][NPLA];
+            auto load_a = [&](int ks) {
+                const int aoff = s8l_frag_off(NPLA, m_l, ks, g);
+#pragma unroll
+                for (int p = 0; p < NPLA; ++p) faq[ks % (DEPTH + 1)][p] = *reinterpret_cast<const bf16x8*>(pa + p * PATCH_BYTES + aoff);
+            };
+#pragma unroll
+            for (int ks = 0; ks < DEPTH; ++ks) load_a(ks);
+#pragma unroll
+            for (int ks = 0; ks < 14; ++ks) {
+                if (ks + DEPTH < 14) load_a(ks + DEPTH);
+                bf16x8 fa[NPLA], fb[NPLW];
+#pragma unroll
+                for (int p = 0; p < NPLA; ++p) fa[p] = faq[ks % (DEPTH + 1)][p];
+#pragma unroll
+                for (int pl = 0; pl < NPLW; ++pl) {
+                    if constexpr (REGS) fb[pl] = fbr[ks][pl];
+                    else fb[pl] = *reinterpret_cast<const bf16x8*>(wl + ((ks * NPLW + pl) * S8_NH + li) * 32 + 16 * (g ^ ((li >> 3) & 1)));
+                }
+                const int a = ks & 1;
+                if constexpr (MODE == 2) {
+                    acc[a] = __builtin_amdgcn_mfma_f32_32x32x16_f16(__builtin_bit_cast(f16x8s, fa[0]), __builtin_bit_cast(f16x8s, fb[1]), acc[a], 0, 0, 0);
+                    acc[a ^ 1] = __builtin_amdgcn_mfma_f32_32x32x16_f16(__builtin_bit_cast(f16x8s, fa[0]), __builtin_bit_cast(f16x8s, fb[0]), acc[a ^ 1], 0, 0, 0);
+                } else if constexpr (F16) {
+                    acc[a] = __builtin_amdgcn_mfma_f32_32x32x16_f16(__builtin_bit_cast(f16x8s, fa[NPLA - 1]), __builtin_bit_cast(f16x8s, fb[0]), acc[a], 0, 0, 0);
+                    acc[a ^ 1] = __builtin_amdgcn_mfma_f32_32x32x16_f16(__builtin_bit_cast(f16x8s, fa[0]), __builtin_bit_cast(f16x8s, fb[NPLW - 1]), acc[a ^ 1], 0, 0, 0);
+                    acc[a] = __builtin_amdgcn_mfma_f32_32x32x16_f16(__builtin_bit_cast(f16x8s, fa[0]), __builtin_bit_cast(f16x8s, fb[0]), acc[a], 0, 0, 0);
+                } else {
+                    acc[a] = __builtin_amdgcn_mfma_f32_32x32x16_bf16(fa[0], fb[NPLW - 1], acc[a], 0, 0, 0);
+                    acc[a ^ 1] = __builtin_amdgcn_mfma_f32_32x32x16_bf16(fa[0], fb[1], acc[a ^ 1], 0, 0, 0);
+                    acc[a] = __builtin_amdgcn_mfma_f32_32x32x16_bf16(fa[0], fb[0], acc[a], 0, 0, 0);
+                }
+            }
+            if constexpr (!REGS) __syncthreads();
+            float* const ctl = ct + (tile * 32 + 4 * g) * S8_NH + li;
+#pragma unroll
+            for (int e = 0; e < 16; ++e) {
+                const float v = fmaf(acc[0][e] + acc[1][e], osc_l, cbl);
+                ctl[(8 * (e >> 2) + s8_slot(e & 3)) * S8_NH] = v;
+                const float vo = ((own[t] >> e) & 1u) ? v : 0.f;
+                ssum += vo;
+                ssq = fmaf(vo, vo, ssq);
+            }
         }
         __syncthreads();
-        const int next_patch = patch + nwg;
-        if (next_patch < npatch) {
-#pragma unroll
-            for (int p = 0; p < NPLA; ++p) {
-                ld0[p] = *reinterpret_cast<const f32x4*>(patch_src(next_patch, cr0, cc0) + p * plane_stride);
-                if (ck1 < NCHUNK) ld1[p] = *reinterpret_cast<const f32x4*>(patch_src(next_patch, cr1, cc1) + p * plane_stride);
-            }
-        }
-        f32x16 acc[2];
-#pragma unroll
-        for (int j = 0; j < 2; ++j)
-#pragma unroll
-            for (int e = 0; e < 16; ++e) acc[j][e] = 0.f;
-#pragma unroll
-        for (int ks = 0; ks < 14; ++ks) {
-            bf16x8 fa[NPLA], fb[NPLW];
-#pragma unroll
-            for (int p = 0; p < NPLA; ++p) fa[p] = *reinterpret_cast<const bf16x8*>(pa + p * PATCH_BYTES + aoff + ((ks >> 1) * (2 * PCH) + (ks & 1) * 4) * 8);
-#pragma unroll
-            for (int pl = 0; pl < NPLW; ++pl) fb[pl] = *reinterpret_cast<const bf16x8*>(wl + ((ks * NPLW + pl) * S8_NH + li) * 32 + 16 * (g ^ ((li >> 3) & 1)));
-            const int a = ks & 1;
-            if constexpr (MODE == 2) {
-                acc[a] = __builtin_amdgcn_mfma_f32_32x32x16_f16(__builtin_bit_cast(f16x8s, fa[0]), __builtin_bit_cast(f16x8s, fb[1]), acc[a], 0, 0, 0);
-                acc[a ^ 1] = __builtin_amdgcn_mfma_f32_32x32x16_f16(__builtin_bit_cast(f16x8s, fa[0]), __builtin_bit_cast(f16x8s, fb[0]), acc[a ^ 1], 0, 0, 0);
-            } else if constexpr (F16) {
-                acc[a] = __builtin_amdgcn_mfma_f32_32x32x16_f16(__builtin_bit_cast(f16x8s, fa[NPLA - 1]), __builtin_bit_cast(f16x8s, fb[0]), acc[a], 0, 0, 0);
-                acc[a ^ 1] = __builtin_amdgcn_mfma_f32_32x32x16_f16(__builtin_bit_cast(f16x8s, fa[0]), __builtin_bit_cast(f16x8s, fb[NPLW - 1]), acc[a ^ 1], 0, 0, 0);
-                acc[a] = __builtin_amdgcn_mfma_f32_32x32x16_f16(__builtin_bit_cast(f16x8s, fa[0]), __builtin_bit_cast(f16x8s, fb[0]), acc[a], 0, 0, 0);
-            } else {
-                acc[a] = __builtin_amdgcn_mfma_f32_32x32x16_bf16(fa[0], fb[NPLW - 1], acc[a], 0, 0, 0);
-                acc[a ^ 1] = __builtin_amdgcn_mfma_f32_32x32x16_bf16(fa[0], fb[1], acc[a ^ 1], 0, 0, 0);
-                acc[a] = __builtin_amdgcn_mfma_f32_32x32x16_bf16(fa[0], fb[0], acc[a], 0, 0, 0);
-            }
-        }
-        __syncthreads();
-#pragma unroll
-        for (int e = 0; e < 16; ++e) {
-            const float v = fmaf(acc[0][e] + acc[1][e], osc_l, cbl);
-            ct[s8_slot(wave * 32 + (e & 3) + 8 * (e >> 2) + 4 * g) * S8_NH + li] = v;
-            const float vo = ((own >> e) & 1u) ? v : 0.f;
-            ssum += vo;
-            ssq = fmaf(vo, vo, ssq);
-        }
-        __syncthreads();
+        if constexpr (REGS) {
+            if (next_patch < npatch) {
+                stage();
+                if (next_patch + nwg < npatch) prefetch(next_patch + nwg);
+            }
+        }
         if (OUT >= 1) {
             float* const raw = OUT == 2 ? raw2 : pooled;
-            for (int it = tid; it < 2 * S8_PH * 2 * S8_PW * 8; it += S8_THREADS) {
+            for (int it = tid; it < 2 * S8_PH * 2 * S8_PW * 8; it += THREADS) {
                 const int p = it >> 3, q4 = it & 7;
                 const int r = p / (2 * S8_PW), cc = p - r * (2 * S8_PW);
                 *reinterpret_cast<float4*>(raw + (((long)b * 112 + R0 + r) * 224 + C0 + cc) * 64 + nh * S8_NH + 4 * q4) =
                     *reinterpret_cast<const float4*>(ct + s8_slot(r * S8_RW + cc) * S8_NH + 4 * q4);
             }
         }
-        if (OUT != 1 && tid < S8_PH * S8_PW * 8) {
-            const int p = tid >> 3;
-            const int pr_l = p / S8_PW, pc_l = p - pr_l * S8_PW;
-            float4 v[9];
-            if (pr < 6 && pc < 15) {
-#pragma unroll
-                for (int k = 0; k < 9; ++k) v[k] = *reinterpret_cast<const float4*>(ct + poff[k]);
-            } else {
-#pragma unroll
-                for (int dr = 0; dr < 3; ++dr)
-#pragma unroll
-                    for (int dc = 0; dc < 3; ++dc) {
-                        const int rr = (R0 + 2 * pr_l + dr >= 112) ? 2 * pr_l : 2 * pr_l + dr;
-                        const int cc = (C0 + 2 * pc_l + dc >= 224) ? 2 * pc_l : 2 * pc_l + dc;
-                        v[dr * 3 + dc] = *reinterpret_cast<const float4*>(ct + s8_slot(rr * S8_RW + cc) * S8_NH + 4 * pch4);
+        if (OUT != 1) {
+#pragma unroll
+            for (int i = 0; i < PI; ++i) {
+                if (tid >= PTH) continue;
+                const int p = (tid >> 3) + i * (PTH / 8);
+                const int pr_l = p / S8_PW, pc_l = p - pr_l * S8_PW;
+                float4 v[9];
+                if (pr < 6 && pc < 15) {
+#pragma unroll
+                    for (int k = 0; k < 9; ++k) v[k] = *reinterpret_cast<const float4*>(ct + poff[k] + i * PROUND * S8_NH);
+                } else {
+#pragma unroll
+                    for (int dr = 0; dr < 3; ++dr)
+#pragma unroll
+                        for (int dc = 0; dc < 3; ++dc) {
+                            const int rr = (R0 + 2 * pr_l + dr >= 112) ? 2 * pr_l : 2 * pr_l + dr;
+                            const int cc = (C0 + 2 * pc_l + dc >= 224) ? 2 * pc_l : 2 * pc_l + dc;
+                            v[dr * 3 + dc] = *reinterpret_cast<const float4*>(ct + s8_slot(rr * S8_RW + cc) * S8_NH + 4 * pch4);
+                        }
+                }
+                float4 ext = v[0];
+                if constexpr (SGN) {
+#pragma unroll
+                    for (int k = 1; k < 9; ++k) {
+                        ext.x = fmaxf(ext.x, v[k].x); ext.y = fmaxf(ext.y, v[k].y); ext.z = fmaxf(ext.z, v[k].z); ext.w = fmaxf(ext.w, v[k].w);
                     }
-            }
-            float4 ext = v[0];
-            if constexpr (SGN) {
-#pragma unroll
-                for (int k = 1; k < 9; ++k) {
-                    ext.x = fmaxf(ext.x, v[k].x); ext.y = fmaxf(ext.y, v[k].y); ext.z = fmaxf(ext.z, v[k].z); ext.w = fmaxf(ext.w, v[k].w);
+                    ext.x *= sgn4[0]; ext.y *= sgn4[1]; ext.z *= sgn4[2]; ext.w *= sgn4[3];
+                } else {
+#pragma unroll
+                    for (int k = 1; k < 9; ++k) {
+                        ext.x = use_min[0] ? fminf(ext.x, v[k].x) : fmaxf(ext.x, v[k].x); ext.y = use_min[1] ? fminf(ext.y, v[k].y) : fmaxf(ext.y, v[k].y);
+                        ext.z = use_min[2] ? fminf(ext.z, v[k].z) : fmaxf(ext.z, v[k].z); ext.w = use_min[3] ? fminf(ext.w, v[k].w) : fmaxf(ext.w, v[k].w);
+                    }
                 }
-                ext.x *= sgn4[0]; ext.y *= sgn4[1]; ext.z *= sgn4[2]; ext.w *= sgn4[3];
-            } else {
-#pragma unroll
-                for (int k = 1; k < 9; ++k) {
-                    ext.x = use_min[0] ? fminf(ext.x, v[k].x) : fmaxf(ext.x, v[k].x); ext.y = use_min[1] ? fminf(ext.y, v[k].y) : fmaxf(ext.y, v[k].y);
-                    ext.z = use_min[2] ? fminf(ext.z, v[k].z) : fmaxf(ext.z, v[k].z); ext.w = use_min[3] ? fminf(ext.w, v[k].w) : fmaxf(ext.w, v[k].w);
-                }
-            }
-            *reinterpret_cast<float4*>(pooled + (((long)b * 56 + 8 * pr + pr_l) * 112 + 7 * pc + pc_l) * 64 + nh * S8_NH + 4 * pch4) = ext;
+                *reinterpret_cast<float4*>(pooled + (((long)b * 56 + 8 * pr + pr_l) * 112 + 7 * pc + pc_l) * 64 + nh * S8_NH + 4 * pch4) = ext;
+            }
         }
         __syncthreads();
     }
@@ -279,7 +347,7 @@
         const int which = tid >> 5, ch = tid & 31;
         float s = 0.f;
 #pragma unroll
-        for (int k = 0; k < 8; ++k) s += red[(which * 8 + k) * S8_NH + ch];
+        for (int k = 0; k < WAVES; ++k) s += red[(which * 8 + k) * S8_NH + ch];
         atomicAdd(&stats[which * 64 + nh * S8_NH + ch], (double)s);
     }
 }
@@ -296,64 +364,47 @@
     return SAGEN_OK;
 }
 
+template <int OUT, int MODE, bool REGS>
+static int stem8pool_run(const char* plane, const float* wf32, const char* wplanes, const float* gamma, float* pooled, double* stats, int B, long plane_stride,
+                         const float* a_inv, const float* w_inv, float* raw2, hipStream_t s) {
+    using Cfg = S8Cfg<MODE, REGS>;
+    static bool attr_set = false;
+    if (!attr_set) {
+        SAGEN_HIP_CHECK(hipFuncSetAttribute(reinterpret_cast<const void*>(stem8pool_kernel<OUT, MODE, REGS>), hipFuncAttributeMaxDynamicSharedMemorySize, Cfg::LDS));
+        attr_set = true;
+    }
+    const int npatch = B * 7 * 16;
+    hipLaunchKernelGGL((stem8pool_kernel<OUT, MODE, REGS>), dim3(2 * std::min(npatch, 256), 1, cur_group().G), dim3(Cfg::THREADS), Cfg::LDS, s, plane, wf32, wplanes, gamma,
+                       pooled, stats, B, plane_stride, a_inv, w_inv, raw2, cur_group());
+    SAGEN_LAUNCH_CHECK();
+    return SAGEN_OK;
+}
+
 int stem8pool_launch(const void* plane, const float* wp, const float* gamma, float* pooled, double* stats, int B, hipStream_t s) {
     if (!plane || !wp || !gamma || !pooled || !stats) return fail(SAGEN_ERR_NULL, "stem8pool: null argument");
-    static bool attr_set = false;
-    if (!attr_set) {
-        SAGEN_HIP_CHECK(hipFuncSetAttribute(reinterpret_cast<const void*>(stem8pool_kernel<0>), hipFuncAttributeMaxDynamicSharedMemorySize, S8_LDS));
-        attr_set = true;
-    }
     const char* planes = reinterpret_cast<const char*>(wp + 64 * 224);
-    const int npatch = B * 7 * 16;
-    hipLaunchKernelGGL(stem8pool_kernel<0>, dim3(2 * std::min(npatch, 256), 1, cur_group().G), dim3(S8_THREADS), S8_LDS, s, reinterpret_cast<const char*>(plane), wp, planes, gamma,
-                       pooled, stats, B, 0L, (const float*)nullptr, (const float*)nullptr, (float*)nullptr, cur_group());
-    SAGEN_LAUNCH_CHECK();
-    return SAGEN_OK;
+    return stem8pool_run<0, 0, false>(reinterpret_cast<const char*>(plane), wp, planes, gamma, pooled, stats, B, 0L, nullptr, nullptr, nullptr, s);
 }
 
 int stem8pool_h2_launch(const void* plane, const float* wp, const void* wh2, const float* w_inv, const float* gamma, float* pooled, double* stats, int B,
-                        hipStream_t s) {
+                        hipStream_t s, int regs) {
     if (!plane || !wp || !wh2 || !w_inv || !gamma || !pooled || !stats) return fail(SAGEN_ERR_NULL, "stem8pool_h2: null argument");
-    static bool attr_set = false;
-    if (!attr_set) {
-        SAGEN_HIP_CHECK(hipFuncSetAttribute(reinterpret_cast<const void*>(stem8pool_kernel<0, 2>), hipFuncAttributeMaxDynamicSharedMemorySize, S8_LDS));
-        attr_set = true;
-    }
-    const int npatch = B * 7 * 16;
-    hipLaunchKernelGGL((stem8pool_kernel<0, 2>), dim3(2 * std::min(npatch, 256), 1, cur_group().G), dim3(S8_THREADS), S8_LDS, s, reinterpret_cast<const char*>(plane), wp,
-                       reinterpret_cast<const char*>(wh2), gamma, pooled, stats, B, 0L, (const float*)nullptr, w_inv, (float*)nullptr, cur_group());
-    SAGEN_LAUNCH_CHECK();
-    return SAGEN_OK;
+    const char* p = reinterpret_cast<const char*>(plane);
+    const char* w = reinterpret_cast<const char*>(wh2);
+    if (regs) return stem8pool_run<0, 2, true>(p, wp, w, gamma, pooled, stats, B, 0L, nullptr, w_inv, nullptr, s);
+    return stem8pool_run<0, 2, false>(p, wp, w, gamma, pooled, stats, B, 0L, nullptr, w_inv, nullptr, s);
 }
 
 int stem8raw_launch(const void* plane, const float* wp, float* y0, double* stats, int B, hipStream_t s) {
     if (!plane || !wp || !y0 || !stats) return fail(SAGEN_ERR_NULL, "stem8raw: null argument");
-    static bool attr_set = false;
-    if (!attr_set) {
-        SAGEN_HIP_CHECK(hipFuncSetAttribute(reinterpret_cast<const void*>(stem8pool_kernel<1>), hipFuncAttributeMaxDynamicSharedMemorySize, S8_LDS));
-        attr_set = true;
-    }
     const char* planes = reinterpret_cast<const char*>(wp + 64 * 224);
-    const int npatch = B * 7 * 16;
-    hipLaunchKernelGGL(stem8pool_kernel<1>, dim3(2 * std::min(npatch, 256), 1, cur_group().G), dim3(S8_THREADS), S8_LDS, s, reinterpret_cast<const char*>(plane), wp, planes,
-                       (const float*)nullptr, y0, stats, B, 0L, (const float*)nullptr, (const float*)nullptr, (float*)nullptr, cur_group());
-    SAGEN_LAUNCH_CHECK();
-    return SAGEN_OK;
+    return stem8pool_run<1, 0, false>(reinterpret_cast<const char*>(plane), wp, planes, nullptr, y0, stats, B, 0L, nullptr, nullptr, nullptr, s);
 }
 
 int stem8rawpool_launch(const void* plane, const float* wp, const float* gamma, float* y0, float* pooled, double* stats, int B, hipStream_t s) {
     if (!plane || !wp || !gamma || !y0 || !pooled || !stats) return fail(SAGEN_ERR_NULL, "stem8rawpool: null argument");
-    static bool attr_set = false;
-    if (!attr_set) {
-        SAGEN_HIP_CHECK(hipFuncSetAttribute(reinterpret_cast<const void*>(stem8pool_kernel<2>), hipFuncAttributeMaxDynamicSharedMemorySize, S8_LDS));
-        attr_set = true;
-    }
     const char* planes = reinterpret_cast<const char*>(wp + 64 * 224);
-    const int npatch = B * 7 * 16;
-    hipLaunchKernelGGL(stem8pool_kernel<2>, dim3(2 * std::min(npatch, 256), 1, cur_group().G), dim3(S8_THREADS), S8_LDS, s, reinterpret_cast<const char*>(plane), wp, planes,
-                       gamma, pooled, stats, B, 0L, (const float*)nullptr, (const float*)nullptr, y0, cur_group());
-    SAGEN_LAUNCH_CHECK();
-    return SAGEN_OK;
+    return stem8pool_run<2, 0, false>(reinterpret_cast<const char*>(plane), wp, planes, gamma, pooled, stats, B, 0L, nullptr, nullptr, y0, s);
 }
 
 constexpr int S16_PARTS = 1024;
@@ -424,16 +475,8 @@
 int stem16pool_launch(const void* planes, const void* wh2, const float* gamma, float* pooled, double* stats, const float* a_inv, const float* w_inv,
                       int B, hipStream_t s) {
     if (!planes || !wh2 || !gamma || !pooled || !stats || !a_inv || !w_inv) return fail(SAGEN_ERR_NULL, "stem16pool: null argument");
-    static bool attr_set = false;
-    if (!attr_set) {
-        SAGEN_HIP_CHECK(hipFuncSetAttribute(reinterpret_cast<const void*>(stem8pool_kernel<0, 1>), hipFuncAttributeMaxDynamicSharedMemorySize, S8_LDS));
-        attr_set = true;
-    }
-    const int npatch = B * 7 * 16;
-    hipLaunchKernelGGL((stem8pool_kernel<0, 1>), dim3(2 * std::min(npatch, 256), 1, cur_group().G), dim3(S8_THREADS), S8_LDS, s, reinterpret_cast<const char*>(planes),
-                       (const float*)nullptr, reinterpret_cast<const char*>(wh2), gamma, pooled, stats, B, (long)stem8_plane_bytes(B), a_inv, w_inv, (float*)nullptr, cur_group());
-    SAGEN_LAUNCH_CHECK();
-    return SAGEN_OK;
-}
-
-}
+    return stem8pool_run<0, 1, false>(reinterpret_cast<const char*>(planes), nullptr, reinterpret_cast<const char*>(wh2), gamma, pooled, stats, B,
+                                      (long)stem8_plane_bytes(B), a_inv, w_inv, nullptr, s);
+}
+
+}
diff --git a/spatialaudiogen_amd/csrc/stem8_layout.h b/spatialaudiogen_amd/csrc/stem8_layout.h
--- /dev/null
+++ b/spatialaudiogen_amd/csrc/stem8_layout.h
@@ -0,0 +1,26 @@
+#pragma once
+
+namespace sagen {
+
+constexpr int S8L_RW = 15;
+constexpr int S8L_M = 17 * S8L_RW;
+constexpr int S8L_PROWS = 39, S8L_PCH = 18;
+
+constexpr int s8l_pitch(int nplanes) { return nplanes == 1 ? 32 : 22; }
+constexpr int s8l_rot(int nplanes) { return nplanes == 1 ? 15 : 3; }
+constexpr int s8l_plane_bytes(int nplanes) { return S8L_PROWS * s8l_pitch(nplanes) * 16; }
+
+constexpr int s8l_rotated(int nplanes, int chunk, int pair) { return (int)((unsigned)(chunk + s8l_rot(nplanes) * pair) % (unsigned)s8l_pitch(nplanes)); }
+constexpr int s8l_chunk_off(int nplanes, int row, int chunk) { return (row * s8l_pitch(nplanes) + s8l_rotated(nplanes, chunk, row >> 1)) * 16; }
+
+constexpr int s8l_frag_row(int m, int ks) { return 2 * ((m < S8L_M ? m : 0) / S8L_RW) + (ks >> 1); }
+constexpr int s8l_frag_chunk(int m, int ks, int g) { return (m < S8L_M ? m : 0) % S8L_RW + 2 * (ks & 1) + g; }
+constexpr int s8l_frag_off(int nplanes, int m, int ks, int g) {
+    const int mm = m < S8L_M ? m : 0, r = mm / S8L_RW, c = mm - r * S8L_RW;
+    return (2 * r * s8l_pitch(nplanes) + s8l_rotated(nplanes, (c + g + s8l_rot(nplanes) * r) + (2 * (ks & 1) + s8l_rot(nplanes) * (ks >> 2)), 0)) * 16
+           + (ks >> 1) * s8l_pitch(nplanes) * 16;
+}
+
+constexpr int s8l_stage_off(int nplanes, int k) { return s8l_chunk_off(nplanes, k / S8L_PCH, k % S8L_PCH); }
+
+}
```

Result: no change. 3208 (-0.2%).
